# constantingoeldel/alphabeta-rs

Measured on AMD Instinct MI355X. Metric: ABneutral model fits/sec (pedigree x bootstraps x windows), higher is better.
Workload: dtype f64; 1 GPU; C3: synthetic 100-edge/8-generation pedigree (N=105 rows, T=8, K=47 distinct triples), 10 starts + 10000 bootstraps per GPU (bootstraps of one window sharded over the GPUs); rows=105, windows_per_gpu=1, starts=10, bootstraps=10000, plan_device_bytes=9663014, reduction_tree=0x10040, parallelism=bootstraps sharded over 1 GPU(s), one RCCL all-gather of the bootstrap tables

## Files before the change

### alphabeta_rs_amd/__init__.py

```python
from __future__ import annotations

import ctypes as C
import os
from pathlib import Path

import numpy as np

from . import build as _build

PKG = Path(__file__).resolve().parent
LIB_PATH = PKG / "libabneutral_hip.so"
if os.environ.get("ABNEUTRAL_HIP_LIB"):
    LIB_PATH = Path(os.environ["ABNEUTRAL_HIP_LIB"])

ABN_OK = 0
STATUS_NAMES = {
    0: "ABN_OK",
    1: "ABN_ERR_INVALID_ARG",
    2: "ABN_ERR_BAD_PEDIGREE",
    3: "ABN_ERR_NO_DEVICE",
    4: "ABN_ERR_HIP",
    5: "ABN_ERR_NO_FINITE_FIT",
    6: "ABN_ERR_STATE",
}
FIT_CONVERGED, FIT_MAX_ITERS, FIT_NONFINITE, FIT_TARGET = 0, 1, 2, 3
KERNEL_NAMES = {0: "none", 1: "speculative", 2: "resident", 3: "persistent", 4: "stream", 5: "two_pass"}

FIT_INFO_DTYPE = np.dtype(
    [("best_cost", "<f8"), ("iters", "<i4"), ("evals", "<i4"), ("status", "<i4"), ("lanes", "<i4")]
)

EXPORTED_SYMBOLS = [
    "abn_default_options", "abn_device_count", "abn_init", "abn_shutdown", "abn_device_info", "abn_last_error",
    "abn_status_string", "abn_version", "abn_cost_batch", "abn_fit_batch", "abn_gen_start_simplices",
    "abn_gen_boot_simplices", "abn_gen_boot_indices", "abn_ab_neutral_run", "abn_boot_model_run",
    "abn_analyze", "abn_select_best", "abn_bootstrap_rows", "abn_pairwise_divergence", "abn_plan_create", "abn_plan_destroy", "abn_plan_set_windows", "abn_plan_run",
    "abn_plan_run_phase", "abn_plan_sync", "abn_plan_tail_handed", "abn_plan_kernel_ms", "abn_plan_raw_device_ptr",
    "abn_plan_bind_raw", "abn_plan_download", "abn_plan_counters", "abn_plan_device_bytes",
    "abn_plan_set_window_ids", "abn_plan_failed_windows",
    "abn_multi_create", "abn_multi_destroy", "abn_multi_last_error", "abn_multi_set_windows", "abn_multi_run",
    "abn_multi_sync", "abn_multi_shard", "abn_multi_raw_device_ptr", "abn_multi_download", "abn_multi_counters",
    "abn_multi_rccl_available", "abn_reduction_tree", "abn_pairwise_divergence_dev", "abn_multi_set_window_ids",
    "abn_pairwise_divergence_windows", "abn_pairwise_divergence_windows_dev",
    "abn_multi_plan_shard", "abn_plan_last_kernels", "abn_multi_kernel_ms",
    "abn_packed_row_stride", "abn_pack_codes", "abn_unpack_codes", "abn_pairwise_divergence_packed",
    "abn_pairwise_divergence_packed_dev",
    "abn_pairwise_divergence_windows_packed", "abn_pairwise_divergence_windows_packed_dev",
    "abn_analyze_batch", "abn_analyze_batch_dev", "abn_plan_analyze", "abn_multi_analyze",
    "abn_windows_create", "abn_windows_destroy", "abn_windows_info", "abn_windows_stats", "abn_windows_layout",
    "abn_windows_packed", "abn_windows_packed_device_ptr", "abn_windows_pairwise",
    "abn_sites_parse", "abn_sites_destroy", "abn_sites_info", "abn_sites_fetch", "abn_sites_deferred",
    "abn_genes_create", "abn_genes_destroy", "abn_genes_choose", "abn_genes_choose_dev", "abn_windows_create_sites",
]


class Options(C.Structure):
    _fields_ = [
        ("seed", C.c_uint64),
        ("lanes_per_chain", C.c_int32),
        ("strict_order", C.c_int32),
        ("shrink_on_failed_contraction", C.c_int32),
        ("max_iters_start", C.c_int32),
        ("max_iters_boot", C.c_int32),
        ("stream_mode", C.c_int32),
        ("sd_tolerance", C.c_double),
        ("window_groups", C.c_int32),
        ("no_fixed_point_skip", C.c_int32),
    ]


class WindowsParams(C.Structure):
    _fields_ = [
        ("cutoff", C.c_uint32),
        ("step", C.c_uint32),
        ("size", C.c_uint32),
        ("absolute", C.c_int32),
        ("n_upstream", C.c_int32),
        ("n_gene", C.c_int32),
        ("n_downstream", C.c_int32),
    ]


class GeneRule(C.Structure):
    _fields_ = [
        ("cutoff", C.c_uint32),
        ("cutoff_gene_length", C.c_int32),
    ]


class SitesParams(C.Structure):
    _fields_ = [
        ("slab_bytes", C.c_int64),
        ("skip_lines", C.c_int32),
        ("reserved", C.c_int32),
    ]


class AbnError(RuntimeError):
    def __init__(self, status: int, detail: str = ""):
        self.status = status
        super().__init__(f"{STATUS_NAMES.get(status, status)}: {detail}")


_lib = None


def load_library(build_if_missing: bool = False) -> C.CDLL:
    global _lib
    if _lib is not None:
        return _lib
    if not LIB_PATH.exists():
        if build_if_missing:
            _build.build_hip()
        else:
            raise FileNotFoundError(
                f"{LIB_PATH} is missing: build it with `python -m alphabeta_rs_amd.build` "
                "(the ABneutral path has no CPU fallback)"
            )
    L = C.CDLL(str(LIB_PATH))
    dp, u32p, vp = C.POINTER(C.c_double), C.POINTER(C.c_uint32), C.c_void_p
    op = C.POINTER(Options)
    L.abn_default_options.argtypes = [op]
    L.abn_default_options.restype = None
    L.abn_device_count.argtypes = [C.POINTER(C.c_int)]
    L.abn_init.argtypes = [C.c_int, vp, C.POINTER(vp)]
    L.abn_shutdown.argtypes = [vp]
    L.abn_device_info.argtypes = [vp, C.POINTER(C.c_int32)]
    L.abn_last_error.argtypes = [vp]
    L.abn_last_error.restype = C.c_char_p
    L.abn_status_string.argtypes = [C.c_int]
    L.abn_status_string.restype = C.c_char_p
    L.abn_cost_batch.argtypes = [vp, op, dp, C.c_int32, C.c_double, C.c_double, C.c_double, dp, C.c_int64, dp, dp,
                                 u32p, u32p, C.c_int64, dp, dp, dp]
    L.abn_fit_batch.argtypes = [vp, op, dp, C.c_int32, C.c_double, C.c_double, C.c_double, dp, C.c_int64, dp,
                                C.c_int32, dp, vp]
    L.abn_gen_start_simplices.argtypes = [C.c_uint64, C.c_uint32, C.c_int32, C.c_double, dp]
    L.abn_gen_boot_simplices.argtypes = [C.c_uint64, C.c_uint32, C.c_uint32, C.c_int64, dp, dp]
    L.abn_gen_boot_indices.argtypes = [vp, C.c_uint64, C.c_uint32, C.c_uint32, C.c_int64, C.c_int32, u32p]
    L.abn_ab_neutral_run.argtypes = [vp, op, dp, C.c_int32, C.c_double, C.c_double, C.c_double, C.c_int32, dp, dp,
                                     dp, dp, vp, dp]
    L.abn_boot_model_run.argtypes = [vp, op, dp, C.c_int32, dp, dp, dp, C.c_double, C.c_double, C.c_double,
                                     C.c_int32, dp, vp]
    L.abn_analyze.argtypes = [dp, C.c_int64, dp]
    L.abn_analyze_batch.argtypes = [vp, dp, C.c_int32, C.c_int64, dp, C.POINTER(C.c_int32)]
    L.abn_analyze_batch_dev.argtypes = [vp, vp, C.c_int32, C.c_int64, vp, vp, dp]
    L.abn_plan_analyze.argtypes = [vp, dp, C.POINTER(C.c_int32)]
    L.abn_multi_analyze.argtypes = [vp, dp, C.POINTER(C.c_int32)]
    L.abn_select_best.argtypes = [vp, dp, C.c_int32, C.c_double, dp, C.c_int32, C.POINTER(C.c_int32), dp, dp, dp, dp]
    L.abn_bootstrap_rows.argtypes = [vp, dp, C.c_int64, dp]
    L.abn_pairwise_divergence.argtypes = [vp, C.POINTER(C.c_uint8), C.c_int32, C.c_int64, C.POINTER(C.c_uint64),
                                          C.POINTER(C.c_uint64), dp]
    L.abn_pairwise_divergence_dev.argtypes = [vp, vp, C.c_int32, C.c_int64, vp, vp, vp, dp]
    i64p = C.POINTER(C.c_int64)
    L.abn_pairwise_divergence_windows.argtypes = [vp, C.POINTER(C.c_uint8), C.c_int32, C.c_int64, i64p, i64p, C.c_int32,
                                                  C.POINTER(C.c_uint64), C.POINTER(C.c_uint64), dp]
    L.abn_pairwise_divergence_windows_dev.argtypes = [vp, vp, C.c_int32, C.c_int64, i64p, i64p, C.c_int32, vp, vp, vp, dp]
    u8p = C.POINTER(C.c_uint8)
    L.abn_packed_row_stride.argtypes = [C.c_int64]
    L.abn_packed_row_stride.restype = C.c_int64
    L.abn_pack_codes.argtypes = [u8p, C.c_int32, C.c_int64, C.c_int64, u8p, C.c_int64]
    L.abn_unpack_codes.argtypes = [u8p, C.c_int32, C.c_int64, C.c_int64, u8p, C.c_int64]
    L.abn_pairwise_divergence_packed.argtypes = [vp, u8p, C.c_int32, C.c_int64, C.c_int64, C.POINTER(C.c_uint64),
                                                 C.POINTER(C.c_uint64), dp]
    L.abn_pairwise_divergence_packed_dev.argtypes = [vp, vp, C.c_int32, C.c_int64, C.c_int64, vp, vp, vp, dp]
    L.abn_pairwise_divergence_windows_packed.argtypes = [vp, u8p, C.c_int32, C.c_int64, C.c_int64, i64p, i64p, C.c_int32,
                                                         C.POINTER(C.c_uint64), C.POINTER(C.c_uint64), dp]
    L.abn_pairwise_divergence_windows_packed_dev.argtypes = [vp, vp, C.c_int32, C.c_int64, C.c_int64, i64p, i64p,
                                                             C.c_int32, vp, vp, vp, dp]
    L.abn_windows_create.argtypes = [vp, C.POINTER(WindowsParams), C.c_int32, i64p, u32p, u32p, u32p, u8p, u8p, dp,
                                     C.POINTER(vp)]
    L.abn_windows_destroy.argtypes = [vp]
    L.abn_windows_info.argtypes = [vp, C.POINTER(C.c_int32), i64p, i64p]
    L.abn_windows_stats.argtypes = [vp, i64p, dp, dp, i64p]
    L.abn_windows_layout.argtypes = [vp, i64p, i64p, C.POINTER(C.c_int32)]
    L.abn_windows_packed.argtypes = [vp, u8p]
    L.abn_windows_packed_device_ptr.argtypes = [vp, C.POINTER(vp)]
    L.abn_windows_pairwise.argtypes = [vp, C.POINTER(C.c_uint64), C.POINTER(C.c_uint64), dp]
    L.abn_sites_parse.argtypes = [vp, C.c_char_p, C.c_int64, C.POINTER(SitesParams), C.POINTER(vp)]
    L.abn_sites_destroy.argtypes = [vp]
    L.abn_sites_info.argtypes = [vp, i64p, i64p, i64p, dp]
    L.abn_sites_fetch.argtypes = [vp, i64p, C.POINTER(C.c_int32), u32p, u32p, u8p, dp, u8p, u8p, dp]
    L.abn_sites_deferred.argtypes = [vp, i64p, i64p, i64p]
    i32p = C.POINTER(C.c_int32)
    L.abn_genes_create.argtypes = [vp, C.c_int32, i32p, i32p, i64p, u32p, u32p, u8p, C.POINTER(vp)]
    L.abn_genes_destroy.argtypes = [vp]
    L.abn_genes_choose.argtypes = [vp, C.POINTER(GeneRule), C.c_int32, i64p, i32p, u32p, u32p, u8p, u32p, u32p, u8p, dp]
    L.abn_genes_choose_dev.argtypes = [vp, C.POINTER(GeneRule), C.c_int32, i64p, vp, vp, vp, vp, vp, vp, vp, dp]
    L.abn_windows_create_sites.argtypes = [vp, C.POINTER(WindowsParams), vp, C.POINTER(GeneRule), C.c_int32, i64p, i32p,
                                           u32p, u32p, u8p, u8p, dp, C.POINTER(vp)]
    L.abn_plan_create.argtypes = [vp, op, dp, C.c_int32, C.c_int32, C.c_int32, C.c_int32, C.c_uint32, C.c_uint32,
                                  C.POINTER(vp)]
    L.abn_plan_destroy.argtypes = [vp]
    L.abn_plan_set_windows.argtypes = [vp, dp, dp, dp, dp]
    L.abn_plan_run.argtypes = [vp]
    L.abn_plan_run_phase.argtypes = [vp, C.c_int32]
    L.abn_plan_sync.argtypes = [vp]
    L.abn_plan_tail_handed.argtypes = [vp, C.POINTER(C.c_int64)]
    L.abn_plan_kernel_ms.argtypes = [vp, dp]
    L.abn_plan_raw_device_ptr.argtypes = [vp, C.POINTER(vp)]
    L.abn_plan_bind_raw.argtypes = [vp, vp]
    L.abn_plan_download.argtypes = [vp, dp, dp, dp, dp, vp, vp, C.POINTER(C.c_int32)]
    L.abn_plan_counters.argtypes = [vp, C.POINTER(C.c_int64)]
    L.abn_plan_device_bytes.argtypes = [vp, C.POINTER(C.c_int64)]
    L.abn_plan_set_window_ids.argtypes = [vp, u32p]
    L.abn_plan_failed_windows.argtypes = [vp, C.POINTER(C.c_int32)]
    L.abn_plan_last_kernels.argtypes = [vp, C.POINTER(C.c_int32)]
    i32p = C.POINTER(C.c_int32)
    L.abn_multi_create.argtypes = [i32p, C.c_int32, op, dp, C.c_int32, C.c_int32, C.c_int32, C.c_int32, C.POINTER(vp)]
    L.abn_multi_destroy.argtypes = [vp]
    L.abn_multi_last_error.argtypes = [vp]
    L.abn_multi_last_error.restype = C.c_char_p
    L.abn_multi_set_windows.argtypes = [vp, dp, dp, dp, dp]
    L.abn_multi_set_window_ids.argtypes = [vp, u32p]
    L.abn_multi_run.argtypes = [vp]
    L.abn_multi_sync.argtypes = [vp]
    L.abn_multi_shard.argtypes = [vp, C.c_int32, i32p]
    L.abn_multi_plan_shard.argtypes = [C.c_int32, C.c_int32, C.c_int32, C.c_int32, i32p]
    L.abn_multi_raw_device_ptr.argtypes = [vp, C.c_int32, C.POINTER(vp)]
    L.abn_multi_kernel_ms.argtypes = [vp, C.c_int32, dp]
    L.abn_multi_download.argtypes = [vp, dp, dp, dp, dp, vp, vp, i32p]
    L.abn_multi_counters.argtypes = [vp, C.POINTER(C.c_int64)]
    L.abn_multi_rccl_available.argtypes = [C.POINTER(C.c_int)]
    L.abn_reduction_tree.argtypes = [op, dp, C.c_int32, i32p]
    _lib = L
    return L


def _dp(a):
    return None if a is None else a.ctypes.data_as(C.POINTER(C.c_double))


def _u32p(a):
    return None if a is None else a.ctypes.data_as(C.POINTER(C.c_uint32))


def _f64(a, shape=None):
    a = np.ascontiguousarray(a, dtype=np.float64)
    return a if shape is None else a.reshape(shape)


def default_options(**kw) -> Options:
    o = Options()
    load_library().abn_default_options(C.byref(o))
    for k, v in kw.items():
        if not hasattr(o, k):
            raise TypeError(f"unknown option {k}")
        setattr(o, k, v)
    return o


def device_count() -> int:
    n = C.c_int(0)
    load_library().abn_device_count(C.byref(n))
    return n.value


def gen_start_simplices(seed: int, window: int, n_starts: int, max_divergence: float) -> np.ndarray:
    out = np.empty((n_starts, 5, 4))
    rc = load_library().abn_gen_start_simplices(seed, window, n_starts, max_divergence, _dp(out))
    if rc:
        raise AbnError(rc)
    return out


def gen_boot_simplices(seed: int, window: int, b0: int, nb: int, params) -> np.ndarray:
    p = _f64(params, (4,))
    out = np.empty((nb, 5, 4))
    rc = load_library().abn_gen_boot_simplices(seed, window, b0, nb, _dp(p), _dp(out))
    if rc:
        raise AbnError(rc)
    return out


def packed_row_stride(n_sites: int) -> int:
    return int(load_library().abn_packed_row_stride(int(n_sites)))


def pack_codes(codes, row_stride: int | None = None) -> np.ndarray:
    codes = np.ascontiguousarray(codes, dtype=np.uint8)
    n, L = codes.shape
    stride = packed_row_stride(L) if row_stride is None else int(row_stride)
    packed = np.empty((n, max(stride, 0)), dtype=np.uint8)
    u8p = C.POINTER(C.c_uint8)
    rc = load_library().abn_pack_codes(codes.ctypes.data_as(u8p), n, L, L, packed.ctypes.data_as(u8p), stride)
    if rc != 0:
        raise AbnError(rc, "pack_codes: a byte that is not 0, 1, 2 or 0x80 | status, or a bad row stride")
    return packed


def unpack_codes(packed, n_sites: int) -> np.ndarray:
    packed = np.ascontiguousarray(packed, dtype=np.uint8)
    n, stride = packed.shape
    codes = np.empty((n, int(n_sites)), dtype=np.uint8)
    u8p = C.POINTER(C.c_uint8)
    rc = load_library().abn_unpack_codes(packed.ctypes.data_as(u8p), n, int(n_sites), stride, codes.ctypes.data_as(u8p),
                                         int(n_sites))
    if rc != 0:
        raise AbnError(rc, "unpack_codes: bad row stride")
    return codes


def analyze(raw) -> np.ndarray:
    raw = _f64(raw).reshape(-1, 7)
    with np.errstate(all="ignore"):
        bad = np.isnan(raw).any(axis=1) | np.isnan(raw[:, 1] / raw[:, 0])
    if bad.any():
        raise AbnError(5, f"bootstrap {int(np.flatnonzero(bad)[0])} has no finite fit: no analysis of this table")
    out = np.empty(32)
    rc = load_library().abn_analyze(_dp(raw), raw.shape[0], _dp(out))
    if rc:
        raise AbnError(rc)
    return out.reshape(4, 8)


def analyze_batch(ctx: "Context", raw, allow_failed_windows=False):
    raw = _f64(raw)
    if raw.ndim != 3 or raw.shape[2] != 7:
        raise ValueError("raw is (n_windows, n_boot, 7)")
    W, B = raw.shape[0], raw.shape[1]
    out, fb = np.empty((W, 32)), np.full(W, -1, dtype=np.int32)
    rc = ctx._L.abn_analyze_batch(ctx._h, _dp(raw), W, B, _dp(out), fb.ctypes.data_as(C.POINTER(C.c_int32)))
    if not (rc == 5 and allow_failed_windows):
        ctx._check(rc)
    return out, fb


class Context:

    def __init__(self, device: int = 0, stream: int | None = None):
        self._L = load_library()
        h = C.c_void_p()
        if stream is None:
            sp = None
        elif stream == 0:
            sp = C.c_void_p(-1)
        else:
            sp = C.c_void_p(stream)
        rc = self._L.abn_init(device, sp, C.byref(h))
        if rc:
            raise AbnError(rc, "abn_init failed (no HIP device? the ABneutral path has no CPU fallback)")
        self._h = h
        self.device = device

    def close(self):
        if getattr(self, "_h", None):
            self._L.abn_shutdown(self._h)
            self._h = None

    def device_info(self):
        out = (C.c_int32 * 4)()
# ... 157 lines not shown
        return ms.value

    def pairwise_divergence_windows_packed(self, packed, n_sites: int, begin, end):
        packed = np.ascontiguousarray(packed, dtype=np.uint8)
        n, stride = packed.shape
        b, e = np.ascontiguousarray(begin, dtype=np.int64), np.ascontiguousarray(end, dtype=np.int64)
        if b.ndim != 1 or b.shape != e.shape:
            raise ValueError("begin and end are 1-d arrays of one length")
        W, npairs = b.shape[0], n * (n - 1) // 2
        diff, both = np.zeros((W, npairs), dtype=np.uint64), np.zeros((W, npairs), dtype=np.uint64)
        dval = np.zeros((W, npairs))
        i64p = C.POINTER(C.c_int64)
        self._check(self._L.abn_pairwise_divergence_windows_packed(
            self._h, packed.ctypes.data_as(C.POINTER(C.c_uint8)), n, int(n_sites), stride, b.ctypes.data_as(i64p),
            e.ctypes.data_as(i64p), W, diff.ctypes.data_as(C.POINTER(C.c_uint64)),
            both.ctypes.data_as(C.POINTER(C.c_uint64)), _dp(dval)))
        return diff, both, dval

    def pairwise_divergence_windows_packed_dev(self, packed_ptr: int, n_samples: int, n_sites: int, row_stride: int,
                                               begin, end, diff_ptr: int = 0, both_ptr: int = 0,
                                               dvalue_ptr: int = 0) -> float:
        b, e = np.ascontiguousarray(begin, dtype=np.int64), np.ascontiguousarray(end, dtype=np.int64)
        if b.ndim != 1 or b.shape != e.shape:
            raise ValueError("begin and end are 1-d arrays of one length")
        ms = C.c_double(0.0)
        i64p = C.POINTER(C.c_int64)
        self._check(self._L.abn_pairwise_divergence_windows_packed_dev(
            self._h, C.c_void_p(packed_ptr), n_samples, n_sites, row_stride, b.ctypes.data_as(i64p),
            e.ctypes.data_as(i64p), b.shape[0], C.c_void_p(diff_ptr or None), C.c_void_p(both_ptr or None),
            C.c_void_p(dvalue_ptr or None), C.byref(ms)))
        return ms.value

    def analyze_batch_dev(self, raw_ptr: int, n_windows: int, n_boot: int, out_ptr: int, first_bad_ptr: int = 0,
                          allow_failed_windows=False) -> float:
        ms = C.c_double(0.0)
        rc = self._L.abn_analyze_batch_dev(self._h, C.c_void_p(raw_ptr), n_windows, n_boot, C.c_void_p(out_ptr),
                                           C.c_void_p(first_bad_ptr or None), C.byref(ms))
        if not (rc == 5 and allow_failed_windows):
            self._check(rc)
        return ms.value

    def parse_sites(self, text: bytes, *, skip_lines: int = 1, slab_bytes: int = 0):
        text = bytes(text)
        p = SitesParams(slab_bytes, skip_lines, 0)
        h = C.c_void_p()
        self._check(self._L.abn_sites_parse(self._h, text, len(text), C.byref(p), C.byref(h)))
        try:
            n, nd, nl, ms = C.c_int64(), C.c_int64(), C.c_int64(), C.c_double()
            self._check(self._L.abn_sites_info(h, C.byref(n), C.byref(nd), C.byref(nl), C.byref(ms)))
            kinds = {"line": np.int64, "chromosome": np.int32, "start": np.uint32, "end": np.uint32, "strand": np.uint8,
                     "posteriormax": np.float64, "status": np.uint8, "status_flag": np.uint8, "meth_lvl": np.float64}
            sites = {k: np.zeros(n.value, dtype=t) for k, t in kinds.items()}
            self._check(self._L.abn_sites_fetch(h, *(a.ctypes.data_as(t) for a, t in
                                                     zip(sites.values(), self._L.abn_sites_fetch.argtypes[1:]))))
            deferred = {k: np.zeros(nd.value, dtype=np.int64) for k in ("line", "offset", "length")}
            self._check(self._L.abn_sites_deferred(h, *(a.ctypes.data_as(C.POINTER(C.c_int64)) for a in deferred.values())))
            sites["n_lines"], sites["kernel_ms"] = nl.value, ms.value
            return sites, deferred
        finally:
            self._L.abn_sites_destroy(h)

    def choose_genes(self, genes: "Genes", site_offset, chromosome, start, end, strand, *, cutoff,
                     cutoff_gene_length=False):
        off, u = _site_arrays(site_offset, chromosome, start, end, strand)
        S = int(off[-1])
        gs, ge, fl = np.zeros(S, dtype=np.uint32), np.zeros(S, dtype=np.uint32), np.zeros(S, dtype=np.uint8)
        ms = np.zeros(3)
        rule = GeneRule(cutoff, 1 if cutoff_gene_length else 0)
        u8p = C.POINTER(C.c_uint8)
        self._check(self._L.abn_genes_choose(genes._h, C.byref(rule), off.shape[0] - 1, off.ctypes.data_as(C.POINTER(C.c_int64)),
                                             u[0].ctypes.data_as(C.POINTER(C.c_int32)), _u32p(u[1]), _u32p(u[2]),
                                             u[3].ctypes.data_as(u8p), _u32p(gs), _u32p(ge), fl.ctypes.data_as(u8p), _dp(ms)))
        return gs, ge, fl, ms

    def choose_genes_dev(self, genes: "Genes", site_offset, chromosome_ptr: int, start_ptr: int, end_ptr: int,
                         strand_ptr: int, gene_start_ptr: int, gene_end_ptr: int, flags_ptr: int, *, cutoff,
                         cutoff_gene_length=False) -> np.ndarray:
        off = np.ascontiguousarray(site_offset, dtype=np.int64)
        ms = np.zeros(3)
        rule = GeneRule(cutoff, 1 if cutoff_gene_length else 0)
        self._check(self._L.abn_genes_choose_dev(genes._h, C.byref(rule), off.shape[0] - 1,
                                                 off.ctypes.data_as(C.POINTER(C.c_int64)),
                                                 *(C.c_void_p(p or None) for p in (chromosome_ptr, start_ptr, end_ptr,
                                                                                   strand_ptr, gene_start_ptr,
                                                                                   gene_end_ptr, flags_ptr)), _dp(ms)))
        return ms

    def boot_model_run(self, pedigree, model, pred, resid, p0uu, eqp, eqp_weight, n_boot, *,
                       options: Options | None = None):
        ped = _f64(pedigree).reshape(-1, 4)
        n = ped.shape[0]
        raw = np.empty((n_boot, 7))
        info = np.zeros(n_boot, dtype=FIT_INFO_DTYPE)
        self._check(self._L.abn_boot_model_run(self._h, C.byref(options) if options else None, _dp(ped), n,
                                               _dp(_f64(model, (4,))), _dp(_f64(pred, (n,))), _dp(_f64(resid, (n,))),
                                               p0uu, eqp, eqp_weight, n_boot, _dp(raw), info.ctypes.data))
        return raw, info


class Plan:

    def __init__(self, ctx: Context, generations, n_windows, n_starts, n_boot, *, window_offset=0, boot_offset=0,
                 options: Options | None = None):
        self.ctx = ctx
        self._L = ctx._L
        g = _f64(generations).reshape(-1, 3)
        self.N, self.W, self.S, self.B = g.shape[0], n_windows, n_starts, n_boot
        h = C.c_void_p()
        ctx._check(self._L.abn_plan_create(ctx._h, C.byref(options) if options else None, _dp(g), self.N, n_windows,
                                           n_starts, n_boot, window_offset, boot_offset, C.byref(h)))
        self._h = h

    def close(self):
        if getattr(self, "_h", None):
            self._L.abn_plan_destroy(self._h)
            self._h = None

    def __del__(self):
        try:
            self.close()
        except Exception:
            pass

    def set_window_ids(self, ids):
        a = None if ids is None else np.ascontiguousarray(ids, dtype=np.uint32).reshape(self.W)
        self.ctx._check(self._L.abn_plan_set_window_ids(self._h, _u32p(a)))

    def failed_windows(self) -> int:
        n = C.c_int32(0)
        self.ctx._check(self._L.abn_plan_failed_windows(self._h, C.byref(n)))
        return n.value

    def set_windows(self, d_obs, p0uu, eqp=None, eqp_weight=None):
        d = _f64(d_obs, (self.W, self.N))
        p = _f64(p0uu, (self.W,))
        e = None if eqp is None else _f64(eqp, (self.W,))
        ew = None if eqp_weight is None else _f64(eqp_weight, (self.W,))
        self.ctx._check(self._L.abn_plan_set_windows(self._h, _dp(d), _dp(p), _dp(e), _dp(ew)))

    def run(self):
        self.ctx._check(self._L.abn_plan_run(self._h))

    def run_phase(self, phase: int):
        self.ctx._check(self._L.abn_plan_run_phase(self._h, phase))

    def sync(self):
        self.ctx._check(self._L.abn_plan_sync(self._h))

    def tail_handed(self):
        out = (C.c_int64 * 2)()
        self.ctx._check(self._L.abn_plan_tail_handed(self._h, out))
        return int(out[0]), int(out[1])

    def kernel_ms(self):
        ms = np.zeros(3)
        self.ctx._check(self._L.abn_plan_kernel_ms(self._h, _dp(ms)))
        return {"fit_starts": ms[0], "select": ms[1], "fit_boot": ms[2]}

    def raw_device_ptr(self) -> int:
        p = C.c_void_p()
        self.ctx._check(self._L.abn_plan_raw_device_ptr(self._h, C.byref(p)))
        return p.value or 0

    def bind_raw(self, dev_ptr: int):
        self.ctx._check(self._L.abn_plan_bind_raw(self._h, C.c_void_p(dev_ptr)))

    def download(self, want_info=True, allow_failed_windows=False):
        W, N, S, B = self.W, self.N, self.S, self.B
        models, pred, resid = np.empty((W, 4)), np.empty((W, N)), np.empty((W, N))
        raw = np.empty((W, B, 7)) if B else None
        ia = np.zeros((W, S), dtype=FIT_INFO_DTYPE) if (S and want_info) else None
        ib = np.zeros((W, B), dtype=FIT_INFO_DTYPE) if (B and want_info) else None
        bs = np.full(W, -1, dtype=np.int32)
        rc = self._L.abn_plan_download(self._h, _dp(models), _dp(pred), _dp(resid), _dp(raw),
                                       None if ia is None else ia.ctypes.data,
                                       None if ib is None else ib.ctypes.data,
                                       bs.ctypes.data_as(C.POINTER(C.c_int32)))
        if not (rc == 5 and allow_failed_windows):
            self.ctx._check(rc)
        return {"models": models, "pred": pred, "resid": resid, "raw": raw, "info_a": ia, "info_b": ib,
                "best_start": bs}

    def analyze(self, allow_failed_windows=False):
        out, fb = np.empty((self.W, 32)), np.full(self.W, -1, dtype=np.int32)
        rc = self._L.abn_plan_analyze(self._h, _dp(out), fb.ctypes.data_as(C.POINTER(C.c_int32)))
        if not (rc == 5 and allow_failed_windows):
            self.ctx._check(rc)
        return out, fb

    def counters(self):
        out = (C.c_int64 * 5)()
        self.ctx._check(self._L.abn_plan_counters(self._h, out))
        return {"fits": out[0], "evals": out[1], "iters": out[2], "evals_skipped": out[3] + out[4],
                "evals_skipped_starts": out[3], "evals_skipped_boot": out[4]}

    def device_bytes(self) -> int:
        b = C.c_int64()
        self.ctx._check(self._L.abn_plan_device_bytes(self._h, C.byref(b)))
        return b.value

    def last_kernels(self):
        out = (C.c_int32 * 4)()
        self.ctx._check(self._L.abn_plan_last_kernels(self._h, out))
        return {"starts": (KERNEL_NAMES.get(out[0], out[0]), out[1]), "boot": (KERNEL_NAMES.get(out[2], out[2]), out[3])}


def _site_arrays(site_offset, chromosome, start, end, strand):
    off = np.ascontiguousarray(site_offset, dtype=np.int64)
    S = int(off[-1]) if off.shape[0] else 0
    return off, [np.ascontiguousarray(a, dtype=t).reshape(S) for a, t in
                 ((chromosome, np.int32), (start, np.uint32), (end, np.uint32), (strand, np.uint8))]


class Genes:

    def __init__(self, ctx: "Context", lists):
        self.ctx = ctx
        self._L = ctx._L
        lists = list(lists)
        chrom = np.array([l[0] for l in lists], dtype=np.int32)
        kind = np.array([l[1] for l in lists], dtype=np.int32)
        off = np.zeros(len(lists) + 1, dtype=np.int64)
        off[1:] = np.cumsum([len(l[2]) for l in lists])
        cat = lambda k, t: np.ascontiguousarray(np.concatenate([np.asarray(l[k], dtype=t) for l in lists])
                                                if lists else np.zeros(0, dtype=t))
        start, end, strand = cat(2, np.uint32), cat(3, np.uint32), cat(4, np.uint8)
        h = C.c_void_p()
        i32p = C.POINTER(C.c_int32)
        ctx._check(self._L.abn_genes_create(ctx._h, len(lists), chrom.ctypes.data_as(i32p), kind.ctypes.data_as(i32p),
                                            off.ctypes.data_as(C.POINTER(C.c_int64)), _u32p(start), _u32p(end),
                                            strand.ctypes.data_as(C.POINTER(C.c_uint8)), C.byref(h)))
        self._h = h
        self.n_genes = int(off[-1])

    def close(self):
        if getattr(self, "_h", None):
            self._L.abn_genes_destroy(self._h)
            self._h = None

    def __del__(self):
        try:
            self.close()
        except Exception:
            pass


class Windows:

    def __init__(self, ctx: Context, site_offset, pos, gene_start, gene_end, flags, code, level, *, cutoff, step, size,
                 absolute, counts):
        self.ctx = ctx
        self._L = ctx._L
        off = np.ascontiguousarray(site_offset, dtype=np.int64)
        self.n_samples = off.shape[0] - 1
        S = int(off[-1]) if off.shape[0] else 0
        u32 = [np.ascontiguousarray(a, dtype=np.uint32).reshape(S) for a in (pos, gene_start, gene_end)]
        u8 = [np.ascontiguousarray(a, dtype=np.uint8).reshape(S) for a in (flags, code)]
        lvl = _f64(level, (S,))
        p = WindowsParams(cutoff, step, size, 1 if absolute else 0, *map(int, counts))
        h = C.c_void_p()
        u8p = C.POINTER(C.c_uint8)
        ctx._check(self._L.abn_windows_create(ctx._h, C.byref(p), self.n_samples, off.ctypes.data_as(C.POINTER(C.c_int64)),
                                              _u32p(u32[0]), _u32p(u32[1]), _u32p(u32[2]), u8[0].ctypes.data_as(u8p),
                                              u8[1].ctypes.data_as(u8p), _dp(lvl), C.byref(h)))
        self._h = h
        W, stride, ns = C.c_int32(), C.c_int64(), C.c_int64()
        ctx._check(self._L.abn_windows_info(h, C.byref(W), C.byref(stride), C.byref(ns)))
        self.W, self.row_stride, self.n_sites = W.value, stride.value, ns.value

    @classmethod
    def from_sites(cls, ctx: Context, genes: Genes, site_offset, chromosome, start, end, strand, code, level, *, cutoff,
                   cutoff_gene_length=False, step, size, absolute, counts):
        self = cls.__new__(cls)
        self.ctx = ctx
        self._L = ctx._L
        off, u = _site_arrays(site_offset, chromosome, start, end, strand)
        self.n_samples = off.shape[0] - 1
        S = int(off[-1]) if off.shape[0] else 0
        co = np.ascontiguousarray(code, dtype=np.uint8).reshape(S)
        lvl = _f64(level, (S,))
        p = WindowsParams(cutoff, step, size, 1 if absolute else 0, *map(int, counts))
        rule = GeneRule(cutoff, 1 if cutoff_gene_length else 0)
        h = C.c_void_p()
        u8p = C.POINTER(C.c_uint8)
        ctx._check(self._L.abn_windows_create_sites(ctx._h, C.byref(p), genes._h, C.byref(rule), self.n_samples,
                                                    off.ctypes.data_as(C.POINTER(C.c_int64)),
                                                    u[0].ctypes.data_as(C.POINTER(C.c_int32)), _u32p(u[1]), _u32p(u[2]),
                                                    u[3].ctypes.data_as(u8p), co.ctypes.data_as(u8p), _dp(lvl), C.byref(h)))
        self._h = h
        W, stride, ns = C.c_int32(), C.c_int64(), C.c_int64()
        ctx._check(self._L.abn_windows_info(h, C.byref(W), C.byref(stride), C.byref(ns)))
        self.W, self.row_stride, self.n_sites = W.value, stride.value, ns.value
        return self

    def close(self):
        if getattr(self, "_h", None):
            self._L.abn_windows_destroy(self._h)
            self._h = None

    def __del__(self):
        try:
            self.close()
        except Exception:
            pass

    def stats(self):
# ... 147 lines not shown
```

### alphabeta_rs_amd/csrc/abn_api.hip

```cpp
#include <functional>

#include "abn_host.hpp"
#include "abn_device.hpp"
#include "abn_route.hpp"

using namespace abn;

static_assert(sizeof(abn_fit_info) == sizeof(FitInfoDev), "abn_fit_info layout");


static int as_i8(double x) {
  if (x != x) return 0;
  if (x >= 127.0) return 127;
  if (x <= -128.0) return -128;
  return (int)x;
}

struct Topology {
  int N = 0, K = 0, T = 0, TP = 0, KP = 0, chain_stride = 0;
  std::vector<uint32_t> tri;
  std::vector<uint16_t> tid;
};

static int build_topology(const double* rows, int n, int stride, Topology& t) {
// ... 385 lines not shown
  DevBuf<uint32_t> d;
  HIPCHK(c, d.alloc((size_t)nb * (size_t)n_rows));
  int rc = launch_gen_idx(c, d.p, n_rows, (int)nb, 1, seed, window, b0);
  if (rc) return rc;
  HIPCHK(c, hipMemcpyAsync(idx, d.p, d.bytes(), hipMemcpyDeviceToHost, c->stream));
  HIPCHK(c, hipStreamSynchronize(c->stream));
  return ABN_OK;
}

extern "C" int abn_cost_batch(abn_ctx* c, const abn_options* opts, const double* pedigree, int32_t n_rows, double p_uu0,
                              double eqp, double eqp_weight, const double* candidates, int64_t m, const double* pred,
                              const double* resid, const uint32_t* idx, const uint32_t* cand_to_boot,
                              int64_t n_boot_rows, double* cost, double* dt1t2, double* p_uu_inf) {
  if (!c) return ABN_ERR_INVALID_ARG;
  if (!pedigree || n_rows <= 0 || !candidates || m < 0 || !cost) return set_err(c, ABN_ERR_INVALID_ARG, "null/size");
  if (idx && (!pred || !resid || n_boot_rows <= 0)) return set_err(c, ABN_ERR_INVALID_ARG, "bootstrap inputs");
  if (m == 0) return ABN_OK;
  if (const char* oe = options_error(resolve(opts))) return set_err(c, ABN_ERR_INVALID_ARG, oe);
  const abn_options o = resolve_for(opts, n_rows);
  OneShot s(c);
  int rc = s.open(c, pedigree, n_rows, [&]() -> int {
    for (int64_t i = 0; idx && i < m; ++i)
      if ((cand_to_boot ? (int64_t)cand_to_boot[i] : i) >= n_boot_rows)
        return set_err(c, ABN_ERR_INVALID_ARG, "cand_to_boot out of range");
    return ABN_OK;
  });
  if (rc) return rc;
  const size_t N = (size_t)n_rows;
  const std::vector<double> dcol = column3(pedigree, n_rows);
  DevBuf<double> dD, dpred, dresid, dcand, dcost, ddt, dpuu;
  DevBuf<uint32_t> didx, dc2b;
  if ((rc = upload(c, dD, dcol.data(), N)) || (rc = upload(c, dcand, candidates, (size_t)m * 4))) return rc;
  HIPCHK(c, dcost.alloc((size_t)m));
  if (idx) {
    if ((rc = upload(c, dpred, pred, N)) || (rc = upload(c, dresid, resid, N)) ||
        (rc = upload(c, didx, idx, (size_t)n_boot_rows * N)))
      return rc;
    for (size_t q = 0; q < (size_t)n_boot_rows * N; ++q)
      if (idx[q] >= (uint32_t)N) return set_err(c, ABN_ERR_INVALID_ARG, "bootstrap index out of range");
    if (cand_to_boot && (rc = upload(c, dc2b, cand_to_boot, (size_t)m))) return rc;
  }
  if (dt1t2) HIPCHK(c, ddt.alloc((size_t)m * N));
  if (p_uu_inf) HIPCHK(c, dpuu.alloc((size_t)m));

  const PedigreeRoute pr = route_pedigree(n_rows, s.t.K, s.t.T, o.lanes_per_chain, o.strict_order);
  if (pr.cost_refusal) return set_err(c, ABN_ERR_INVALID_ARG, pr.cost_refusal);
  const int ng = kWave / pr.cost_lanes;
  CostArgs a{};
  fill_topology(a, s.t, s.dt);
  a.chain_stride = s.t.chain_stride;
  a.p_uu0 = p_uu0;
  a.eqp = eqp;
  a.eqp_w = eqp_weight;
  a.D = dD.p;
  a.pred = dpred.p;
  a.resid = dresid.p;
  a.idx = didx.p;
  a.cand_to_boot = dc2b.p;
  a.dmode = idx ? 1 : 0;
  a.cand = dcand.p;
  a.M = m;
  a.strict = pr.strict;
  a.tree = pr.cost_tree;
  a.cost = dcost.p;
  a.dt = ddt.p;
  a.puu = dpuu.p;
  const long long blocks = (m + ng - 1) / ng;
  if (blocks > 0x7fffffffLL) return set_err(c, ABN_ERR_INVALID_ARG, "too many candidates");
  LaunchRoute r{};
  r.key = {kFamCost, pr.cost_lanes, 0, false, false, false};
  r.grid = (unsigned)blocks;
  r.block = kWave;
  r.lds = pr.cost_lds;
  rc = launch_route(c, r, a, c->stream);
  if (rc) return rc;
  HIPCHK(c, hipMemcpyAsync(cost, dcost.p, dcost.bytes(), hipMemcpyDeviceToHost, c->stream));
  if (dt1t2) HIPCHK(c, hipMemcpyAsync(dt1t2, ddt.p, ddt.bytes(), hipMemcpyDeviceToHost, c->stream));
  if (p_uu_inf) HIPCHK(c, hipMemcpyAsync(p_uu_inf, dpuu.p, dpuu.bytes(), hipMemcpyDeviceToHost, c->stream));
  HIPCHK(c, hipStreamSynchronize(c->stream));
  return ABN_OK;
}

extern "C" int abn_fit_batch(abn_ctx* c, const abn_options* opts, const double* pedigree, int32_t n_rows, double p_uu0,
                             double eqp, double eqp_weight, const double* simplex0, int64_t f, const double* dobs_rows,
                             int32_t max_iters, double* best, abn_fit_info* info) {
  if (!c) return ABN_ERR_INVALID_ARG;
  if (!pedigree || n_rows <= 0 || !simplex0 || f < 0 || !best || max_iters < 0 || f > 0x7fffffff)
    return set_err(c, ABN_ERR_INVALID_ARG, "null/size");
  if (f == 0) return ABN_OK;
  if (const char* oe = options_error(resolve(opts))) return set_err(c, ABN_ERR_INVALID_ARG, oe);
  const abn_options o = resolve_for(opts, n_rows);
  if (max_iters > (1 << 28)) return set_err(c, ABN_ERR_INVALID_ARG, "max_iters must be in 0 .. 2^28");
  OneShot s(c);
  int rc = s.open(c, pedigree, n_rows);
  if (rc) return rc;
  const size_t N = (size_t)n_rows;
  DevBuf<double> dD, ds0, dbest, dscal;
  DevBuf<FitInfoDev> dinfo;
  const std::vector<double> dcol = dobs_rows ? std::vector<double>() : column3(pedigree, n_rows);
  const double scal[3] = {p_uu0, eqp, eqp_weight};
  if ((rc = upload(c, dD, dobs_rows ? dobs_rows : dcol.data(), dobs_rows ? (size_t)f * N : N)) ||
      (rc = upload(c, ds0, simplex0, (size_t)f * 20)) || (rc = upload(c, dscal, scal, 3)))
    return rc;
  HIPCHK(c, dbest.alloc((size_t)f * 4));
  HIPCHK(c, dinfo.alloc((size_t)f));
  HIPCHK(c, hipMemsetAsync(dinfo.p, 0, dinfo.bytes(), c->stream));

  const PedigreeRoute pr = route_pedigree(n_rows, s.t.K, s.t.T, o.lanes_per_chain, o.strict_order);
  FitArgs a{};
  fill_topology(a, s.t, s.dt);
  fill_options(a, o, pr);
  a.p_uu = dscal.p;
  a.eqp = dscal.p + 1;
  a.eqp_w = dscal.p + 2;
  a.D = dD.p;
  a.simplex0 = ds0.p;
  a.W = dobs_rows ? (int)f : 1;
  a.C = dobs_rows ? 1 : (int)f;
  a.max_iters = max_iters;
  a.best = dbest.p;
  a.info = dinfo.p;
  rc = launch_fit(c, pr, PhaseRoute{false, pr.lanes, false}, a, LaunchOffer{}, c->stream);
  if (rc) return rc;
  HIPCHK(c, hipMemcpyAsync(best, dbest.p, dbest.bytes(), hipMemcpyDeviceToHost, c->stream));
  if (info) HIPCHK(c, hipMemcpyAsync(info, dinfo.p, dinfo.bytes(), hipMemcpyDeviceToHost, c->stream));
  HIPCHK(c, hipStreamSynchronize(c->stream));
  return ABN_OK;
}

enum PlanEvent { kEvFitA, kEvFitAEnd, kEvSelect, kEvSelectEnd, kEvFitB, kEvFitBEnd, kPlanEvents };

struct abn_plan {
  abn_ctx* ctx = nullptr;
  abn_options opt{};
  Topology topo;
  DevTopology dtopo;
  int N = 0, W = 0, S = 0, B = 0;
  uint32_t window_offset = 0, boot_offset = 0;
  PedigreeRoute route{};
  std::vector<uint32_t> wid_host;
  DevBuf<uint32_t> wid;
  bool windows_set = false, phase_a_done = false, ran_a = false, ran_b = false;
  DevBuf<double> D, pred, resid, p_uu, eqp, eqp_w, simplexA, bestA, model, lse, bestB, raw_own;
  DevBuf<FitInfoDev> infoA, infoB;
  DevBuf<int32_t> best_start;
  DevBuf<uint32_t> idx;
  DevBuf<double> dstar;
  DevBuf<double> nm_state;
  DevBuf<int> susp_list;
  DevBuf<unsigned long long> skipped;
  bool twopass_a = false;
  DevBuf<int> slice_buf;
  unsigned slice_cap = 0;
  DevBuf<unsigned> slice_status;
  long long persist_expected[2] = {0, 0};
  long long tail_handed[2] = {0, 0};
  int32_t last_kernels[4] = {0, 0, 0, 0};
  bool stream_b = false;
  double* raw = nullptr;
  hipEvent_t ev[kPlanEvents] = {};
  hipEvent_t ev_fork = nullptr;
  std::vector<hipEvent_t> ev_join;
};

extern "C" int abn_plan_destroy(abn_plan* p) {
  if (!p) return ABN_ERR_INVALID_ARG;
  for (auto& e : p->ev)
    if (e) (void)hipEventDestroy(e);
  if (p->ev_fork) (void)hipEventDestroy(p->ev_fork);
  for (auto e : p->ev_join) (void)hipEventDestroy(e);
  delete p;
  return ABN_OK;
}

extern "C" int abn_plan_create(abn_ctx* c, const abn_options* opts, const double* generations, int32_t n_rows,
                               int32_t n_windows, int32_t n_starts, int32_t n_boot, uint32_t window_offset,
                               uint32_t boot_offset, abn_plan** out) {
  if (!c || !out) return ABN_ERR_INVALID_ARG;
  *out = nullptr;
  if (!generations || n_rows <= 0 || n_windows <= 0 || n_starts < 0 || n_boot < 0)
    return set_err(c, ABN_ERR_INVALID_ARG, "null/size");
  if ((long long)n_windows * std::max(n_starts, n_boot) > 0x7fffffffLL)
    return set_err(c, ABN_ERR_INVALID_ARG, "too many chains");
  {
    const abn_options o = resolve(opts);
    if (const char* oe = options_error(o)) return set_err(c, ABN_ERR_INVALID_ARG, oe);
  }
  HIPCHK(c, hipSetDevice(c->device));
  PoolScope pool_scope(c);
  struct Destroy {
    void operator()(abn_plan* q) const { abn_plan_destroy(q); }
  };
  std::unique_ptr<abn_plan, Destroy> owner(new (std::nothrow) abn_plan());
  abn_plan* p = owner.get();
  if (!p) return ABN_ERR_HIP;
  p->ctx = c;
  p->opt = resolve_for(opts, n_rows);
  p->N = n_rows;
  p->W = n_windows;
  p->S = n_starts;
  p->B = n_boot;
  p->window_offset = window_offset;
  p->boot_offset = boot_offset;
  int rc = build_topology(generations, n_rows, 3, p->topo);
  if (rc) return set_err(c, rc, abn_status_string(rc));
  p->route = route_pedigree(n_rows, p->topo.K, p->topo.T, p->opt.lanes_per_chain, p->opt.strict_order);
  if (p->route.refusal) return set_err(c, ABN_ERR_INVALID_ARG, p->route.refusal);
  auto fail = [&](hipError_t e, const char* what) {
    return set_err(c, ABN_ERR_HIP, std::string(what) + ": " + hipGetErrorString(e));
  };
  rc = upload_topology(c, p->topo, p->dtopo);
  if (rc) return rc;
  const size_t W = (size_t)n_windows, N = (size_t)n_rows, S = (size_t)n_starts, B = (size_t)n_boot;
  hipError_t e;
#define PALLOC(buf, count)                         \
  if ((e = p->buf.alloc(count)) != hipSuccess) return fail(e, "hipMalloc " #buf)
  PALLOC(D, W * N);
  PALLOC(pred, W * N);
  PALLOC(resid, W * N);
  PALLOC(p_uu, W);
  PALLOC(eqp, W);
  PALLOC(eqp_w, W);
  PALLOC(model, W * 4);
  PALLOC(best_start, W);
  PALLOC(simplexA, W * S * 20);
  PALLOC(bestA, W * S * 4);
  PALLOC(infoA, W * S);
  PALLOC(lse, W * S);
  PALLOC(idx, W * B * N);
  PALLOC(bestB, W * B * 4);
  PALLOC(infoB, W * B);
  PALLOC(raw_own, W * B * 7);
  PALLOC(skipped, 2 * kPhaseWords);
  PALLOC(slice_status, 2 * kSliceWords);
  p->twopass_a = plan_two_pass((long long)n_windows * n_starts, p->opt.max_iters_start, p->opt.no_fixed_point_skip,
                               p->opt.shrink_on_failed_contraction, p->opt.strict_order);
  if (p->twopass_a) {
    PALLOC(nm_state, W * S * kStateDoubles);
    PALLOC(susp_list, W * S + 1);
  }
  if (const size_t chains = plan_sliced_chains(p->route, W * std::max(S, B), c->cus, p->opt.window_groups)) {
    if (p->nm_state.n < chains * kStateDoubles) PALLOC(nm_state, chains * kStateDoubles);
    p->slice_cap = (unsigned)(chains * 16 / kParkShards + 4096);
    PALLOC(slice_buf, (size_t)kParkShards * ((size_t)kParkHeaderInts + (size_t)p->slice_cap));
    if (p->susp_list.n < chains + 1) PALLOC(susp_list, chains + 1);
  }
  p->stream_b = n_boot > 0 && p->route.streams && p->opt.stream_mode == 0;
  if (p->stream_b) PALLOC(dstar, W * B * N);
#undef PALLOC
  p->raw = p->raw_own.p;
  for (auto& ev : p->ev)
    if ((e = hipEventCreate(&ev)) != hipSuccess) return fail(e, "hipEventCreate");
  *out = owner.release();
  return ABN_OK;
}

static int plan_upload_model(abn_plan* p, const double* model, const double* pred, const double* resid,
                             const double* p0uu, const double* eqp, const double* eqp_w) {
  abn_ctx* c = p->ctx;
  const size_t W = (size_t)p->W;
  HIPCHK(c, hipMemcpyAsync(p->model.p, model, p->model.bytes(), hipMemcpyHostToDevice, c->stream));
  HIPCHK(c, hipMemcpyAsync(p->pred.p, pred, p->pred.bytes(), hipMemcpyHostToDevice, c->stream));
  HIPCHK(c, hipMemcpyAsync(p->resid.p, resid, p->resid.bytes(), hipMemcpyHostToDevice, c->stream));
  HIPCHK(c, hipMemcpyAsync(p->p_uu.p, p0uu, W * sizeof(double), hipMemcpyHostToDevice, c->stream));
  HIPCHK(c, hipMemcpyAsync(p->eqp.p, eqp, W * sizeof(double), hipMemcpyHostToDevice, c->stream));
  HIPCHK(c, hipMemcpyAsync(p->eqp_w.p, eqp_w, W * sizeof(double), hipMemcpyHostToDevice, c->stream));
  int rc = launch_gen_idx(c, p->idx.p, p->N, p->B, p->W, p->opt.seed, p->window_offset, p->boot_offset, p->wid.p);
  if (rc) return rc;
  HIPCHK(c, hipStreamSynchronize(c->stream));
  p->windows_set = true;
  p->phase_a_done = true;
  return ABN_OK;
}

extern "C" int abn_plan_set_window_ids(abn_plan* p, const uint32_t* ids) {
  if (!p) return ABN_ERR_INVALID_ARG;
  abn_ctx* c = p->ctx;
  if (p->windows_set) return set_err(c, ABN_ERR_STATE, "abn_plan_set_window_ids must precede abn_plan_set_windows");
  HIPCHK(c, hipSetDevice(c->device));
  PoolScope pool_scope(c);
  if (!ids) {
    p->wid_host.clear();
    p->wid.release();
    return ABN_OK;
  }
  p->wid_host.assign(ids, ids + p->W);
  if (int rc = upload(c, p->wid, p->wid_host.data(), (size_t)p->W)) return rc;
  HIPCHK(c, hipStreamSynchronize(c->stream));
  return ABN_OK;
}

extern "C" int abn_plan_set_windows(abn_plan* p, const double* d_obs, const double* p0uu, const double* eqp,
                                    const double* eqp_weight) {
  if (!p) return ABN_ERR_INVALID_ARG;
  abn_ctx* c = p->ctx;
  if (!d_obs || !p0uu) return set_err(c, ABN_ERR_INVALID_ARG, "null window data");
  HIPCHK(c, hipSetDevice(c->device));
  const size_t W = (size_t)p->W, N = (size_t)p->N, S = (size_t)p->S;
  std::vector<double> ones(W, 1.0);
  const double* e1 = eqp ? eqp : p0uu;
  const double* e2 = eqp_weight ? eqp_weight : ones.data();
  HIPCHK(c, hipMemcpyAsync(p->D.p, d_obs, p->D.bytes(), hipMemcpyHostToDevice, c->stream));
  HIPCHK(c, hipMemcpyAsync(p->p_uu.p, p0uu, W * sizeof(double), hipMemcpyHostToDevice, c->stream));
  HIPCHK(c, hipMemcpyAsync(p->eqp.p, e1, W * sizeof(double), hipMemcpyHostToDevice, c->stream));
  HIPCHK(c, hipMemcpyAsync(p->eqp_w.p, e2, W * sizeof(double), hipMemcpyHostToDevice, c->stream));
  std::vector<double> sx(W * S * 20);
  for (size_t w = 0; w < W; ++w) {
    double mx = d_obs[w * N];
    for (size_t i = 1; i < N; ++i) mx = std::max(mx, d_obs[w * N + i]);
    const uint32_t wg = p->wid_host.empty() ? p->window_offset + (uint32_t)w : p->wid_host[w];
    abn_gen_start_simplices(p->opt.seed, wg, p->S, mx, sx.data() + w * S * 20);
  }
  if (!sx.empty())
    HIPCHK(c, hipMemcpyAsync(p->simplexA.p, sx.data(), p->simplexA.bytes(), hipMemcpyHostToDevice, c->stream));
  int rc = launch_gen_idx(c, p->idx.p, p->N, p->B, p->W, p->opt.seed, p->window_offset, p->boot_offset, p->wid.p);
  if (rc) return rc;
  HIPCHK(c, hipStreamSynchronize(c->stream));
  p->windows_set = true;
  p->phase_a_done = false;
  return ABN_OK;
}

struct WindowOffsets {
  size_t w, rows, starts, boots;
};
static WindowOffsets window_offsets(const abn_plan* p, int w0) {
  const size_t o = (size_t)w0;
  return {o, o * (size_t)p->N, o * (size_t)p->S, o * (size_t)p->B};
}

static FitArgs phase_args(const abn_plan* p, int phase, int w0, int wn) {
  const WindowOffsets o = window_offsets(p, w0);
  const size_t chains = phase ? o.boots : o.starts;
  FitArgs a{};
  fill_topology(a, p->topo, p->dtopo);
  fill_options(a, p->opt, p->route);
  a.p_uu = p->p_uu.p + o.w;
  a.eqp = p->eqp.p + o.w;
  a.eqp_w = p->eqp_w.p + o.w;
  a.wstride = 1;
  a.D = p->D.p + o.rows;
  a.pred = p->pred.p + o.rows;
  a.resid = p->resid.p + o.rows;
  a.idx = p->idx.p + o.boots * (size_t)p->N;
  a.model = p->model.p + o.w * 4;
  a.window_offset = p->window_offset + (uint32_t)w0;
  a.boot_offset = p->boot_offset;
  a.wid = p->wid.p ? p->wid.p + o.w : nullptr;
  a.W = wn;
  a.C = phase ? p->B : p->S;
  a.dmode = a.smode = phase;
  a.simplex0 = phase ? nullptr : p->simplexA.p + chains * 20;
  a.max_iters = phase ? p->opt.max_iters_boot : p->opt.max_iters_start;
  a.best = (phase ? p->bestB.p : p->bestA.p) + chains * 4;
  a.info = (phase ? p->infoB.p : p->infoA.p) + chains;
  a.raw = phase ? p->raw + chains * 7 : nullptr;
  return a;
}

static int launch_phase(abn_plan* p, int phase, FitArgs& a, hipStream_t st, bool timed) {
  abn_ctx* c = p->ctx;
  const bool whole = a.W == p->W;
  const char* force = nullptr;
#ifdef ABN_MEASUREMENT_KNOBS
  force = getenv(phase ? "ABN_PHASE_B_KERNEL" : "ABN_PHASE_A_KERNEL");
#endif
  const PhaseRoute ph = route_phase(p->route, phase, (long long)p->W * (phase ? p->B : p->S), c->cus, a.dmode, whole,
                                    p->twopass_a, force);
  LaunchOffer offer;
  offer.queue = whole;
  offer.parking = whole && p->slice_cap > 0;
  a.skipped = p->skipped.p + kPhaseWords * phase + kPhaseSkipped;
  if (whole) {
    a.queue = reinterpret_cast<unsigned*>(p->skipped.p + kPhaseWords * phase + kPhaseQueue);
    a.slice_status = p->slice_status.p + kSliceWords * phase;
  }
  if (offer.parking) {
    a.park_cap = p->slice_cap;
    a.park_ht = reinterpret_cast<unsigned*>(p->slice_buf.p);
    a.parked = p->slice_buf.p + kParkShards * kParkHeaderInts;
    a.state = p->nm_state.p;
    a.susp_list = p->susp_list.p;
  }
  int kind = ABN_KERNEL_NONE, rc;
  if (ph.two_pass) {
    int* cnt = p->susp_list.p + (size_t)p->W * (size_t)p->S;
    HIPCHK(c, hipMemsetAsync(cnt, 0, sizeof(int), st));
    a.state = p->nm_state.p;
    a.susp_list = p->susp_list.p;
    a.susp_count = cnt;
    offer.pass = 1;
    rc = launch_fit(c, p->route, ph, a, offer, st, &kind);
    offer.pass = 2;
    if (!rc) rc = launch_fit(c, p->route, ph, a, offer, st);
  } else {
    rc = launch_fit(c, p->route, ph, a, offer, st, &kind);
  }
  if (rc) return rc;
  if (whole) p->persist_expected[phase] = kind == ABN_KERNEL_PERSISTENT ? (long long)a.W * a.C : 0;
  if (timed) {
    p->last_kernels[2 * phase] = kind;
    p->last_kernels[2 * phase + 1] = ph.lanes;
  }
  return ABN_OK;
}

static int enqueue_phase_a(abn_plan* p, int w0, int wn, hipStream_t st, bool timed) {
  abn_ctx* c = p->ctx;
  FitArgs a = phase_args(p, 0, w0, wn);
  if (timed) HIPCHK(c, hipEventRecord(p->ev[kEvFitA], st));
  if (int rc = launch_phase(p, 0, a, st, timed)) return rc;
  if (timed) HIPCHK(c, hipEventRecord(p->ev[kEvFitAEnd], st));
  const WindowOffsets o = window_offsets(p, w0);
  SelectArgs s{};
  fill_topology(s, p->topo, p->dtopo);
  s.p_uu = a.p_uu;
  s.D = a.D;
  s.models = a.best;
  s.info = a.info;
  s.W = wn;
  s.S = p->S;
  s.lse = p->lse.p + o.starts;
  s.model = p->model.p + o.w * 4;
  s.pred = p->pred.p + o.rows;
  s.resid = p->resid.p + o.rows;
  s.best_start = p->best_start.p + o.w;
  if (timed) HIPCHK(c, hipEventRecord(p->ev[kEvSelect], st));
  if (int rc = launch_select(c, s, p->route.select_lds, st)) return rc;
  if (timed) HIPCHK(c, hipEventRecord(p->ev[kEvSelectEnd], st));
  return ABN_OK;
}

static int enqueue_phase_b(abn_plan* p, int w0, int wn, hipStream_t st, bool timed) {
  abn_ctx* c = p->ctx;
  FitArgs a = phase_args(p, 1, w0, wn);
  if (timed) HIPCHK(c, hipEventRecord(p->ev[kEvFitB], st));
  if (p->stream_b) {
    double* dst = p->dstar.p + window_offsets(p, w0).boots * (size_t)p->N;
    const long long total = (long long)wn * p->B * p->N;
    const unsigned blocks = (unsigned)std::min<long long>((total + 255) / 256, 64LL * c->cus);
    hipLaunchKernelGGL(abn_make_dstar_kernel, dim3(blocks), dim3(256), 0, st, dst, a.pred, a.resid, a.idx, p->N,
                       (long long)p->B * p->N, total);
    HIPCHK(c, hipGetLastError());
    a.dmode = 2;
    a.D = dst;
  }
  if (int rc = launch_phase(p, 1, a, st, timed)) return rc;
  if (timed) HIPCHK(c, hipEventRecord(p->ev[kEvFitBEnd], st));
  return ABN_OK;
}

static int clear_phase_words(abn_plan* p, int first, int n) {
  HIPCHK(p->ctx, hipMemsetAsync(p->skipped.p + kPhaseWords * first, 0, (size_t)n * kPhaseWords * sizeof(unsigned long long),
                                p->ctx->stream));
  return ABN_OK;
}

enum ClearWords { kClearNone, kClearOwnPhase, kClearBothPhases };
static int plan_run_phase(abn_plan* p, int32_t phase, ClearWords clear) {
  abn_ctx* c = p->ctx;
  if (!p->windows_set) return set_err(c, ABN_ERR_STATE, "abn_plan_set_windows has not been called");
  HIPCHK(c, hipSetDevice(c->device));
  if (clear == kClearBothPhases) {
    if (int rc = clear_phase_words(p, 0, 2)) return rc;
  } else if (clear == kClearOwnPhase) {
    if (int rc = clear_phase_words(p, phase == 0 ? 0 : 1, 1)) return rc;
  }
  if (phase == 0) {
    if (p->S <= 0) return set_err(c, ABN_ERR_STATE, "plan has no starts");
    int rc = enqueue_phase_a(p, 0, p->W, c->stream, true);
    if (rc) return rc;
    p->phase_a_done = true;
    p->ran_a = true;
    return ABN_OK;
  }
  if (phase == 1) {
    if (p->B <= 0) return set_err(c, ABN_ERR_STATE, "plan has no bootstraps");
    if (!p->phase_a_done) return set_err(c, ABN_ERR_STATE, "phase A has not run");
    int rc = enqueue_phase_b(p, 0, p->W, c->stream, true);
    if (rc) return rc;
    p->ran_b = true;
    return ABN_OK;
  }
  return set_err(c, ABN_ERR_INVALID_ARG, "phase must be 0 or 1");
}

extern "C" int abn_plan_run_phase(abn_plan* p, int32_t phase) {
  if (!p) return ABN_ERR_INVALID_ARG;
  return plan_run_phase(p, phase, kClearOwnPhase);
}

extern "C" int abn_plan_run(abn_plan* p) {
  if (!p) return ABN_ERR_INVALID_ARG;
  abn_ctx* c = p->ctx;
  if (!p->windows_set) return set_err(c, ABN_ERR_STATE, "abn_plan_set_windows has not been called");
  int groups = p->opt.window_groups > 0 ? p->opt.window_groups : 1;
  groups = std::max(1, std::min(groups, p->W));
  if (groups == 1 || p->S <= 0 || p->B <= 0) {
    int rc = ABN_OK;
    if (p->S > 0) rc = plan_run_phase(p, 0, kClearBothPhases);
    if (rc) return rc;
    if (p->B > 0) rc = plan_run_phase(p, 1, p->S > 0 ? kClearNone : kClearOwnPhase);
    return rc;
  }
  HIPCHK(c, hipSetDevice(c->device));
  while ((int)c->side.size() < groups) {
    hipStream_t st = nullptr;
    HIPCHK(c, hipStreamCreateWithFlags(&st, hipStreamNonBlocking));
    c->side.push_back(st);
  }
  if (!p->ev_fork) HIPCHK(c, hipEventCreateWithFlags(&p->ev_fork, hipEventDisableTiming));
  while ((int)p->ev_join.size() < groups) {
    hipEvent_t e = nullptr;
    HIPCHK(c, hipEventCreateWithFlags(&e, hipEventDisableTiming));
    p->ev_join.push_back(e);
  }
  if (int rc = clear_phase_words(p, 0, 2)) return rc;
  HIPCHK(c, hipEventRecord(p->ev_fork, c->stream));
  for (int g = 0; g < groups; ++g) {
    const int w0 = (int)((long long)p->W * g / groups), w1 = (int)((long long)p->W * (g + 1) / groups);
    hipStream_t st = c->side[(size_t)g];
    HIPCHK(c, hipStreamWaitEvent(st, p->ev_fork, 0));
    int rc = enqueue_phase_a(p, w0, w1 - w0, st, g == 0);
    if (!rc) rc = enqueue_phase_b(p, w0, w1 - w0, st, g == 0);
    if (rc) return rc;
    HIPCHK(c, hipEventRecord(p->ev_join[(size_t)g], st));
  }
  for (int g = 0; g < groups; ++g) HIPCHK(c, hipStreamWaitEvent(c->stream, p->ev_join[(size_t)g], 0));
  p->phase_a_done = true;
  p->ran_a = true;
  p->ran_b = true;
  return ABN_OK;
}

static int verify_persistent(abn_plan* p) {
  abn_ctx* c = p->ctx;
  HIPCHK(c, hipSetDevice(c->device));
  unsigned sl[2][kSliceWords] = {};
  const bool check = p->persist_expected[0] > 0 || p->persist_expected[1] > 0;
  if (check) HIPCHK(c, hipMemcpyAsync(sl, p->slice_status.p, sizeof sl, hipMemcpyDeviceToHost, c->stream));
  HIPCHK(c, hipStreamSynchronize(c->stream));
  for (int ph = 0; ph < 2 && check; ++ph) {
    if (p->persist_expected[ph] <= 0) continue;
    const unsigned* s = sl[ph];
    p->tail_handed[ph] = (long long)s[kSliceHanded];
    if (s[kSliceError] != 0 || (long long)s[kSliceFinished] != p->persist_expected[ph])
      return set_err(c, ABN_ERR_HIP, std::string("persistent fit launch of phase ") + (ph ? "B" : "A") + " finished " +
                                         std::to_string(s[kSliceFinished]) + " of " + std::to_string(p->persist_expected[ph]) +
                                         " chains (error word " + std::to_string(s[kSliceError]) + ", " + std::to_string(s[kSliceHanded]) +
                                         " handed to the speculative kernel, list length " + std::to_string(s[kSliceTailFill]) +
                                         "): results are incomplete");
  }
  return ABN_OK;
}

extern "C" int abn_plan_sync(abn_plan* p) {
  if (!p) return ABN_ERR_INVALID_ARG;
  return verify_persistent(p);
}

extern "C" int abn_plan_tail_handed(abn_plan* p, int64_t* out2) {
  if (!p || !out2) return ABN_ERR_INVALID_ARG;
  const int rc = verify_persistent(p);
  out2[0] = p->persist_expected[0] > 0 ? p->tail_handed[0] : 0;
  out2[1] = p->persist_expected[1] > 0 ? p->tail_handed[1] : 0;
  return rc;
}

extern "C" int abn_plan_kernel_ms(abn_plan* p, double* ms3) {
  if (!p || !ms3) return ABN_ERR_INVALID_ARG;
  abn_ctx* c = p->ctx;
  HIPCHK(c, hipStreamSynchronize(c->stream));
  ms3[0] = ms3[1] = ms3[2] = 0.0;
  float ms = 0.f;
  if (p->ran_a) {
    HIPCHK(c, hipEventElapsedTime(&ms, p->ev[kEvFitA], p->ev[kEvFitAEnd]));
    ms3[0] = ms;
    HIPCHK(c, hipEventElapsedTime(&ms, p->ev[kEvSelect], p->ev[kEvSelectEnd]));
    ms3[1] = ms;
  }
  if (p->ran_b) {
    HIPCHK(c, hipEventElapsedTime(&ms, p->ev[kEvFitB], p->ev[kEvFitBEnd]));
    ms3[2] = ms;
  }
  return ABN_OK;
}

extern "C" int abn_plan_raw_device_ptr(abn_plan* p, void** dev_ptr) {
  if (!p || !dev_ptr) return ABN_ERR_INVALID_ARG;
  *dev_ptr = p->raw;
  return ABN_OK;
}

extern "C" int abn_plan_bind_raw(abn_plan* p, void* dev_ptr) {
  if (!p) return ABN_ERR_INVALID_ARG;
  p->raw = dev_ptr ? (double*)dev_ptr : p->raw_own.p;
  return ABN_OK;
}

extern "C" int abn_plan_download(abn_plan* p, double* models, double* pred, double* resid, double* raw,
                                 abn_fit_info* info_a, abn_fit_info* info_b, int32_t* best_start) {
  if (!p) return ABN_ERR_INVALID_ARG;
  abn_ctx* c = p->ctx;
  HIPCHK(c, hipSetDevice(c->device));
  hipStream_t s = c->stream;
  const size_t W = (size_t)p->W, B = (size_t)p->B;
  if (models) HIPCHK(c, hipMemcpyAsync(models, p->model.p, p->model.bytes(), hipMemcpyDeviceToHost, s));
  if (pred) HIPCHK(c, hipMemcpyAsync(pred, p->pred.p, p->pred.bytes(), hipMemcpyDeviceToHost, s));
  if (resid) HIPCHK(c, hipMemcpyAsync(resid, p->resid.p, p->resid.bytes(), hipMemcpyDeviceToHost, s));
  if (raw && B) HIPCHK(c, hipMemcpyAsync(raw, p->raw, W * B * 7 * sizeof(double), hipMemcpyDeviceToHost, s));
  if (info_a && p->S) HIPCHK(c, hipMemcpyAsync(info_a, p->infoA.p, p->infoA.bytes(), hipMemcpyDeviceToHost, s));
  if (info_b && B) HIPCHK(c, hipMemcpyAsync(info_b, p->infoB.p, p->infoB.bytes(), hipMemcpyDeviceToHost, s));
  std::vector<int32_t> bs;
  if (p->ran_a) {
    bs.resize(W);
    HIPCHK(c, hipMemcpyAsync(bs.data(), p->best_start.p, p->best_start.bytes(), hipMemcpyDeviceToHost, s));
  }
  if (int rc = verify_persistent(p)) return rc;
  if (best_start) {
    if (p->ran_a) std::copy(bs.begin(), bs.end(), best_start);
    else std::fill(best_start, best_start + W, 0);
  }
  for (int32_t b : bs)
    if (b < 0) return set_err(c, ABN_ERR_NO_FINITE_FIT, "a window has no finite start (best_start = -1): its rows are NaN");
  return ABN_OK;
}

extern "C" int abn_plan_analyze(abn_plan* p, double* out, int32_t* first_bad) {
  if (!p) return ABN_ERR_INVALID_ARG;
  abn_ctx* c = p->ctx;
  if (!out) return set_err(c, ABN_ERR_INVALID_ARG, "null out");
  if (!p->ran_b || p->B <= 0) return set_err(c, ABN_ERR_STATE, "phase B has not run: there is no bootstrap table");
  if (int rc = verify_persistent(p)) return rc;
  return analyze_device_table(c, p->raw, p->W, p->B, out, first_bad);
}

extern "C" int abn_plan_failed_windows(abn_plan* p, int32_t* n_failed) {
  if (!p || !n_failed) return ABN_ERR_INVALID_ARG;
  abn_ctx* c = p->ctx;
  *n_failed = 0;
  if (!p->ran_a) return verify_persistent(p);
  HIPCHK(c, hipSetDevice(c->device));
  std::vector<int32_t> bs((size_t)p->W);
  HIPCHK(c, hipMemcpyAsync(bs.data(), p->best_start.p, p->best_start.bytes(), hipMemcpyDeviceToHost, c->stream));
  if (int rc = verify_persistent(p)) return rc;
  for (int32_t b : bs) *n_failed += b < 0 ? 1 : 0;
  return ABN_OK;
}

extern "C" int abn_plan_counters(abn_plan* p, int64_t* out5) {
  if (!p || !out5) return ABN_ERR_INVALID_ARG;
  abn_ctx* c = p->ctx;
  out5[0] = out5[1] = out5[2] = out5[3] = out5[4] = 0;
  std::vector<FitInfoDev> h;
  auto add = [&](const DevBuf<FitInfoDev>& b, int phase) -> int {
    if (!b.n) return ABN_OK;
    h.resize(b.n);
    unsigned long long sk = 0;
    HIPCHK(c, hipMemcpyAsync(h.data(), b.p, b.bytes(), hipMemcpyDeviceToHost, c->stream));
    HIPCHK(c, hipMemcpyAsync(&sk, p->skipped.p + kPhaseWords * phase + kPhaseSkipped, sizeof sk, hipMemcpyDeviceToHost, c->stream));
    HIPCHK(c, hipStreamSynchronize(c->stream));
    for (const auto& f : h) {
      out5[0] += 1;
      out5[1] += f.evals;
      out5[2] += f.iters;
    }
    out5[3 + phase] = (int64_t)sk;
    return ABN_OK;
  };
  int rc = ABN_OK;
  if (p->ran_a) rc = add(p->infoA, 0);
  if (rc) return rc;
  if (p->ran_b) rc = add(p->infoB, 1);
  return rc;
}

#ifdef ABN_STAMPS
static int debug_stamps(abn_plan* p, unsigned long long* out8, bool spec) {
  abn_ctx* c = p->ctx;
  DevBuf<unsigned long long> d;
  HIPCHK(c, d.alloc(8));
  HIPCHK(c, hipMemsetAsync(d.p, 0, 64, c->stream));
  FitArgs a = phase_args(p, 0, 0, p->W);
  a.dbg = d.p;
  int rc = launch_fit(c, p->route, PhaseRoute{spec, p->route.lanes, false}, a, LaunchOffer{}, c->stream);
  if (rc) return rc;
  HIPCHK(c, hipMemcpyAsync(out8, d.p, 64, hipMemcpyDeviceToHost, c->stream));
  HIPCHK(c, hipStreamSynchronize(c->stream));
  return ABN_OK;
}
extern "C" int abn_plan_debug_stamps(abn_plan* p, unsigned long long* out8) { return debug_stamps(p, out8, false); }
extern "C" int abn_plan_debug_stamps_spec(abn_plan* p, unsigned long long* out8) { return debug_stamps(p, out8, true); }
#endif

extern "C" int abn_plan_last_kernels(abn_plan* p, int32_t* out4) {
  if (!p || !out4) return ABN_ERR_INVALID_ARG;
  for (int k = 0; k < 4; ++k) out4[k] = p->last_kernels[k];
  return ABN_OK;
}

extern "C" int abn_plan_device_bytes(abn_plan* p, int64_t* bytes) {
  if (!p || !bytes) return ABN_ERR_INVALID_ARG;
  size_t t = 0;
  t += p->D.bytes() + p->pred.bytes() + p->resid.bytes() + p->p_uu.bytes() + p->eqp.bytes() + p->eqp_w.bytes();
  t += p->simplexA.bytes() + p->bestA.bytes() + p->model.bytes() + p->lse.bytes() + p->bestB.bytes();
  t += p->raw_own.bytes() + p->infoA.bytes() + p->infoB.bytes() + p->best_start.bytes() + p->idx.bytes();
  t += p->dstar.bytes() + p->nm_state.bytes() + p->susp_list.bytes() + p->skipped.bytes() + p->slice_buf.bytes();
  t += p->slice_status.bytes() + p->wid.bytes();
  t += p->dtopo.tri.bytes() + p->dtopo.tid.bytes();
  *bytes = (int64_t)t;
  return ABN_OK;
}

static void split_pedigree(const double* ped, int n, std::vector<double>& gens, std::vector<double>& d) {
  gens.resize((size_t)n * 3);
  d = column3(ped, n);
  for (size_t i = 0; i < (size_t)n; ++i) std::copy(ped + i * 4, ped + i * 4 + 3, gens.begin() + i * 3);
}

extern "C" int abn_ab_neutral_run(abn_ctx* c, const abn_options* opts, const double* pedigree, int32_t n_rows,
                                  double p0uu, double eqp, double eqp_weight, int32_t n_starts, double* model,
                                  double* pred, double* resid, double* all_models, abn_fit_info* info, double* lse) {
  if (!c) return ABN_ERR_INVALID_ARG;
  if (!pedigree || n_rows <= 0 || n_starts <= 0 || !model || !pred || !resid)
    return set_err(c, ABN_ERR_INVALID_ARG, "null/size");
  std::vector<double> gens, d;
  split_pedigree(pedigree, n_rows, gens, d);
  abn_plan* p = nullptr;
  int rc = abn_plan_create(c, opts, gens.data(), n_rows, 1, n_starts, 0, 0, 0, &p);
  if (rc) return rc;
  rc = abn_plan_set_windows(p, d.data(), &p0uu, &eqp, &eqp_weight);
  if (!rc) rc = abn_plan_run_phase(p, 0);
  int32_t best = -1;
  bool no_fit = false;
  if (!rc) {
    rc = abn_plan_download(p, model, pred, resid, nullptr, info, nullptr, &best);
    if (rc == ABN_ERR_NO_FINITE_FIT) {
      no_fit = true;
      rc = ABN_OK;
    }
  }
  if (!rc && all_models) {
    hipError_t e = hipMemcpy(all_models, p->bestA.p, p->bestA.bytes(), hipMemcpyDeviceToHost);
    if (e != hipSuccess) rc = set_err(c, ABN_ERR_HIP, hipGetErrorString(e));
  }
  if (!rc && lse) {
    hipError_t e = hipMemcpy(lse, p->lse.p, p->lse.bytes(), hipMemcpyDeviceToHost);
    if (e != hipSuccess) rc = set_err(c, ABN_ERR_HIP, hipGetErrorString(e));
  }
  abn_plan_destroy(p);
  if (!rc && (no_fit || best < 0)) rc = set_err(c, ABN_ERR_NO_FINITE_FIT, abn_status_string(ABN_ERR_NO_FINITE_FIT));
  return rc;
}

extern "C" int abn_boot_model_run(abn_ctx* c, const abn_options* opts, const double* pedigree, int32_t n_rows,
                                  const double* model, const double* pred, const double* resid, double p0uu,
                                  double eqp, double eqp_weight, int32_t n_boot, double* raw, abn_fit_info* info) {
  if (!c) return ABN_ERR_INVALID_ARG;
  if (!pedigree || n_rows <= 0 || n_boot <= 0 || !model || !pred || !resid || !raw)
    return set_err(c, ABN_ERR_INVALID_ARG, "null/size");
  std::vector<double> gens, d;
  split_pedigree(pedigree, n_rows, gens, d);
  abn_plan* p = nullptr;
  int rc = abn_plan_create(c, opts, gens.data(), n_rows, 1, 0, n_boot, 0, 0, &p);
  if (rc) return rc;
  rc = plan_upload_model(p, model, pred, resid, &p0uu, &eqp, &eqp_weight);
  if (!rc) rc = abn_plan_run_phase(p, 1);
  if (!rc) rc = abn_plan_download(p, nullptr, nullptr, nullptr, raw, nullptr, info, nullptr);
  abn_plan_destroy(p);
  return rc;
}

extern "C" int abn_select_best(abn_ctx* c, const double* pedigree, int32_t n_rows, double p0uu, const double* models,
                               int32_t n_models, int32_t* best_index, double* model, double* pred, double* resid,
                               double* lse) {
  if (!c) return ABN_ERR_INVALID_ARG;
  if (!pedigree || n_rows <= 0 || !models || n_models <= 0 || !best_index)
    return set_err(c, ABN_ERR_INVALID_ARG, "null/size");
  OneShot s(c);
  PedigreeRoute pr{};
  int rc = s.open(c, pedigree, n_rows, [&]() -> int {
    pr = route_pedigree(n_rows, s.t.K, s.t.T, 0, 0);
    return pr.select_refusal ? set_err(c, ABN_ERR_INVALID_ARG, pr.select_refusal) : ABN_OK;
  });
  if (rc) return rc;
  const size_t N = (size_t)n_rows, S = (size_t)n_models;
  const std::vector<double> dcol = column3(pedigree, n_rows);
  DevBuf<double> dD, dm, dlse, dmodel, dpred, dresid, dp;
  DevBuf<FitInfoDev> dinfo;
  DevBuf<int32_t> dbest;
  if ((rc = upload(c, dD, dcol.data(), N)) || (rc = upload(c, dm, models, S * 4)) || (rc = upload(c, dp, &p0uu, 1)))
    return rc;
  HIPCHK(c, dlse.alloc(S));
  HIPCHK(c, dmodel.alloc(4));
  HIPCHK(c, dpred.alloc(N));
  HIPCHK(c, dresid.alloc(N));
  HIPCHK(c, dinfo.alloc(S));
  HIPCHK(c, dbest.alloc(1));
  HIPCHK(c, hipMemsetAsync(dinfo.p, 0, dinfo.bytes(), c->stream));
  SelectArgs a{};
  fill_topology(a, s.t, s.dt);
  a.p_uu = dp.p;
  a.D = dD.p;
  a.models = dm.p;
  a.info = dinfo.p;
  a.W = 1;
  a.S = n_models;
  a.lse = dlse.p;
  a.model = dmodel.p;
  a.pred = dpred.p;
  a.resid = dresid.p;
  a.best_start = dbest.p;
  rc = launch_select(c, a, pr.select_lds, c->stream);
  if (rc) return rc;
  HIPCHK(c, hipMemcpyAsync(best_index, dbest.p, sizeof(int32_t), hipMemcpyDeviceToHost, c->stream));
  if (model) HIPCHK(c, hipMemcpyAsync(model, dmodel.p, dmodel.bytes(), hipMemcpyDeviceToHost, c->stream));
  if (pred) HIPCHK(c, hipMemcpyAsync(pred, dpred.p, dpred.bytes(), hipMemcpyDeviceToHost, c->stream));
  if (resid) HIPCHK(c, hipMemcpyAsync(resid, dresid.p, dresid.bytes(), hipMemcpyDeviceToHost, c->stream));
  if (lse) HIPCHK(c, hipMemcpyAsync(lse, dlse.p, dlse.bytes(), hipMemcpyDeviceToHost, c->stream));
  HIPCHK(c, hipStreamSynchronize(c->stream));
  if (*best_index < 0) return set_err(c, ABN_ERR_NO_FINITE_FIT, abn_status_string(ABN_ERR_NO_FINITE_FIT));
  return ABN_OK;
}

extern "C" int abn_bootstrap_rows(abn_ctx* c, const double* best, int64_t n_boot, double* raw) {
  if (!c) return ABN_ERR_INVALID_ARG;
  if (!best || !raw || n_boot < 0) return set_err(c, ABN_ERR_INVALID_ARG, "null/size");
  if (n_boot == 0) return ABN_OK;
  HIPCHK(c, hipSetDevice(c->device));
  PoolScope pool_scope(c);
  DevBuf<double> db, dr;
  if (int rc = upload(c, db, best, (size_t)n_boot * 4)) return rc;
  HIPCHK(c, dr.alloc((size_t)n_boot * 7));
  const unsigned blocks = (unsigned)std::min<long long>((n_boot + 255) / 256, 4096);
  hipLaunchKernelGGL(abn_rows_kernel, dim3(blocks), dim3(256), 0, c->stream, db.p, (long long)n_boot, dr.p);
  HIPCHK(c, hipGetLastError());
  HIPCHK(c, hipMemcpyAsync(raw, dr.p, dr.bytes(), hipMemcpyDeviceToHost, c->stream));
  HIPCHK(c, hipStreamSynchronize(c->stream));
  return ABN_OK;
}
```

### alphabeta_rs_amd/csrc/abn_aux_kernels.hpp

```cpp
#pragma once
#include "abn_common.hpp"

namespace abn {

struct SelectArgs {
  const uint32_t* tri;
  const uint16_t* tid;
  int N, K, T, TP;
  const double* p_uu;
  const double* D;
  const double* models;
  const FitInfoDev* info;
  int W, S;
  double* lse;
  double* model;
  double* pred;
  double* resid;
  int32_t* best_start;
};

__device__ __forceinline__ void select_fill_dt(const SelectArgs& a, const double* x, double p_uu0, double* pw,
                                               double* dtab, int lane) {
  const double p_mm = 1.0 - p_uu0;
  const double sv0 = p_uu0, sv1 = x[2] * p_mm, sv2 = (1.0 - x[2]) * p_mm;
  if constexpr (kMatrixFma) build_power_table_mx<kWave>(x[0], x[1], a.T, pw, 0, dtab, lane);
  else build_power_table<kWave>(genmatrix(x[0], x[1]), a.T, a.TP, pw, lane);
  __syncthreads();
  for (int t = lane; t < a.K; t += kWave) dtab[t] = triple_dt(a.tri[t], pw, a.TP, sv0, sv1, sv2);
  __syncthreads();
}

__global__ __launch_bounds__(kWave) void abn_select_lse_kernel(const SelectArgs a) {
  extern __shared__ __align__(16) double lds[];
  const int lane = threadIdx.x;
  const int w = blockIdx.x / a.S, sidx = blockIdx.x - w * a.S;
  const int N = a.N;
  double* pw = lds;
  double* dtab = pw + kPw * a.TP;
  double* term = dtab + ((a.K + 1) & ~1);
  const size_t wN = (size_t)w * (size_t)N;
  double x[4];
#pragma unroll
  for (int d = 0; d < 4; ++d) x[d] = a.models[((size_t)w * a.S + sidx) * 4 + d];
  select_fill_dt(a, x, a.p_uu[w], pw, dtab, lane);
  double lsum = 0.0;
  for (int base = 0; base < N; base += kSelChunk) {
    const int cnt = (N - base) < kSelChunk ? (N - base) : kSelChunk;
    for (int i = lane; i < cnt; i += kWave) {
      const double r = a.D[wN + base + i] - x[3] - dtab[a.tid[base + i]];
      term[i] = r * r;
    }
    __syncthreads();
    for (int i = 0; i < cnt; ++i) lsum = lsum + term[i];
    __syncthreads();
  }
  if (lane == 0) a.lse[(size_t)w * a.S + sidx] = lsum;
}

__global__ __launch_bounds__(kWave) void abn_select_kernel(const SelectArgs a) {
  extern __shared__ __align__(16) double lds[];
  const int lane = threadIdx.x;
  const int w = blockIdx.x;
  const int N = a.N;
  double* pw = lds;
  double* dtab = pw + kPw * a.TP;
  const size_t wN = (size_t)w * (size_t)N;

  int best = -1;
  double best_lse = __builtin_inf();
  for (int sidx = lane; sidx < a.S; sidx += kWave) {
    const double lsum = a.lse[(size_t)w * a.S + sidx];
    const bool ok = (lsum == lsum) && (a.info[(size_t)w * a.S + sidx].status != 2);
    if (ok && (best < 0 || lsum < best_lse)) {
      best = sidx;
      best_lse = lsum;
    }
  }
#pragma unroll
  for (int off = kWave / 2; off >= 1; off >>= 1) {
    const int ob = __shfl_xor(best, off, kWave);
    const double ol = __shfl_xor(best_lse, off, kWave);
    if (ob >= 0 && (best < 0 || ol < best_lse || (ol == best_lse && ob < best))) {
      best = ob;
      best_lse = ol;
    }
  }
  if (lane == 0) a.best_start[w] = best;
  if (best < 0) {
    for (int i = lane; i < N; i += kWave) {
      a.pred[wN + i] = __builtin_nan("");
      a.resid[wN + i] = __builtin_nan("");
    }
    if (lane < 4) a.model[4 * w + lane] = __builtin_nan("");
    return;
  }
  double x[4];
#pragma unroll
  for (int d = 0; d < 4; ++d) x[d] = a.models[((size_t)w * a.S + best) * 4 + d];
  select_fill_dt(a, x, a.p_uu[w], pw, dtab, lane);
  for (int i = lane; i < N; i += kWave) {
    const double p = x[3] + dtab[a.tid[i]];
    a.pred[wN + i] = p;
    a.resid[wN + i] = a.D[wN + i] - p;
  }
  if (lane < 4) a.model[4 * w + lane] = x[lane];
}

struct CostArgs {
  const uint32_t* tri;
  const uint16_t* tid;
  int N, K, T, TP;
  int chain_stride;
  double p_uu0, eqp, eqp_w;
  const double* D;
  const double* pred;
  const double* resid;
  const uint32_t* idx;
  const uint32_t* cand_to_boot;
  int dmode;
  const double* cand;
  long long M;
  int strict;
  int tree;
  double* cost;
  double* dt;
  double* puu;
};

template <int G>
__global__ __launch_bounds__(kWave) void abn_cost_kernel(const CostArgs a) {
  constexpr int NG = kWave / G;
  extern __shared__ __align__(16) double lds[];
  const int lane = threadIdx.x;
  const int g = lane / G;
  const int gl = lane - g * G;
  const long long m_raw = (long long)blockIdx.x * NG + g;
  const bool valid = m_raw < a.M;
  const long long m = valid ? m_raw : 0;
  const int N = a.N, K = a.K, TP = a.TP;
  double* pw = lds + (size_t)g * a.chain_stride;
  double* dtab = pw + kPw * TP;
  double* term = lds + (size_t)NG * a.chain_stride;

  const double al = a.cand[4 * m + 0], be = a.cand[4 * m + 1], wt = a.cand[4 * m + 2], ic = a.cand[4 * m + 3];
  const double p_mm = 1.0 - a.p_uu0;
  const uint32_t* idx_row = nullptr;
  if (a.dmode) {
    const size_t b = a.cand_to_boot ? a.cand_to_boot[m] : (size_t)m;
    idx_row = a.idx + b * (size_t)N;
  }
  const double sv0 = a.p_uu0, sv1 = wt * p_mm, sv2 = (1.0 - wt) * p_mm;
  if constexpr (kMatrixFma && G == kWave) build_power_table_mx<G>(al, be, a.T, lds, a.chain_stride, dtab, lane);
  else build_power_table<G>(genmatrix(al, be), a.T, TP, pw, gl);
  __syncthreads();
  for (int t = gl; t < K; t += G) dtab[t] = triple_dt(a.tri[t], pw, TP, sv0, sv1, sv2);
  __syncthreads();
  const double puu = p_uu_est(al, be);
  const double pen = (a.eqp_w * (double)N) * ((puu - a.eqp) * (puu - a.eqp));
  double result;
  if (a.strict) {
    double ssum = 0.0;
    for (int base = 0; base < N; base += kSelChunk) {
      const int cnt = (N - base) < kSelChunk ? (N - base) : kSelChunk;
      for (int i = gl; i < cnt; i += G) {
        const int row = base + i;
        const double d = a.dmode ? a.pred[row] + a.resid[idx_row[row]] : a.D[row];
        const double r = d - ic - dtab[a.tid[row]];
        term[i] = r * r + pen;
      }
      __syncthreads();
      for (int i = 0; i < cnt; ++i) ssum = ssum + term[i];
      __syncthreads();
    }
    result = ssum;
  } else {
    if (a.tree == kTreeCanon) {
      constexpr int NA = kWave / G;
      double av[NA];
#pragma unroll
      for (int j = 0; j < NA; ++j) av[j] = 0.0;
      for (int i0 = gl; i0 < N; i0 += kWave) {
#pragma unroll
        for (int j = 0; j < NA; ++j) {
          const int i = i0 + G * j;
          if (i < N) {
            const double d = a.dmode ? a.pred[i] + a.resid[idx_row[i]] : a.D[i];
            const double r = d - ic - dtab[a.tid[i]];
            av[j] = av[j] + (r * r + pen);
          }
        }
      }
      result = tree64_finish<G>(av);
    } else {
      double acc = 0.0;
      for (int i = gl; i < N; i += G) {
        const double d = a.dmode ? a.pred[i] + a.resid[idx_row[i]] : a.D[i];
        const double r = d - ic - dtab[a.tid[i]];
        acc = acc + (r * r + pen);
      }
      result = group_sum<G>(acc);
    }
  }
  if (valid) {
    if (gl == 0) {
      a.cost[m] = result;
      if (a.puu) a.puu[m] = puu;
    }
    if (a.dt)
      for (int i = gl; i < N; i += G) a.dt[(size_t)m * N + i] = dtab[a.tid[i]];
  }
}

__global__ __launch_bounds__(256) void abn_rows_kernel(const double* best, long long n, double* raw) {
  for (long long t = (long long)blockIdx.x * blockDim.x + threadIdx.x; t < n; t += (long long)gridDim.x * blockDim.x) {
    const double al = best[4 * t + 0], be = best[4 * t + 1];
    double* ro = raw + 7 * t;
    ro[0] = al;
    ro[1] = be;
    ro[2] = best[4 * t + 2];
    ro[3] = best[4 * t + 3];
    ro[4] = est_mm(al, be);
    ro[5] = est_um(al, be);
    ro[6] = p_uu_est(al, be);
  }
}

__global__ __launch_bounds__(256) void abn_make_dstar_kernel(double* dstar, const double* pred, const double* resid,
                                                             const uint32_t* idx, int N, long long rows_per_window,
                                                             long long total) {
  for (long long t = (long long)blockIdx.x * blockDim.x + threadIdx.x; t < total;
       t += (long long)gridDim.x * blockDim.x) {
    const long long w = t / rows_per_window;
    const int i = (int)(t % N);
    const size_t wN = (size_t)w * (size_t)N;
    dstar[t] = pred[wN + i] + resid[wN + idx[t]];
  }
}

__global__ __launch_bounds__(256) void abn_gen_idx_kernel(uint32_t* idx, int N, int B, int W, uint64_t seed,
                                                          uint32_t window_offset, uint32_t boot_offset,
                                                          const uint32_t* wid) {
  const int Q = (N + 3) / 4;
  const long long total = (long long)W * B * Q;
  const uint32_t k0 = (uint32_t)seed, k1 = (uint32_t)(seed >> 32);
  for (long long t = (long long)blockIdx.x * blockDim.x + threadIdx.x; t < total;
       t += (long long)gridDim.x * blockDim.x) {
    const int q = (int)(t % Q);
    const long long wb = t / Q;
    const int b = (int)(wb % B);
    const int w = (int)(wb / B);
    uint32_t r[4];
    philox4x32_10((uint32_t)q, boot_offset + (uint32_t)b, wid ? wid[w] : window_offset + (uint32_t)w, kTagIdx, k0, k1, r);
    uint32_t* row = idx + (size_t)wb * (size_t)N;
#pragma unroll
    for (int e = 0; e < 4; ++e) {
      const int i = 4 * q + e;
      if (i < N) row[i] = index_from(r[e], (uint32_t)N);
    }
// ... 5 lines not shown
```

### alphabeta_rs_amd/csrc/abn_common.hpp

```cpp
#pragma once
#include <type_traits>
#include <hip/hip_runtime.h>
#include <stdint.h>

#include "abn_constants.hpp"
#include "abn_philox.h"

namespace abn {

#ifndef ABN_STREAM_WAVES
#define ABN_STREAM_WAVES 2
#endif
constexpr int kStreamWaves = ABN_STREAM_WAVES;

typedef uint32_t u32x4 __attribute__((ext_vector_type(4), aligned(4)));
typedef uint16_t u16x4 __attribute__((ext_vector_type(4), aligned(2)));
typedef double f64x2 __attribute__((ext_vector_type(2), aligned(8)));
typedef uint32_t u32x4_lds __attribute__((ext_vector_type(4)));
typedef double f64x2_lds __attribute__((ext_vector_type(2)));

constexpr int ST_INIT0 = 0;
constexpr int ST_REFLECT = 5;
constexpr int ST_EXPAND = 6;
constexpr int ST_CONTRACT = 7;
constexpr int ST_SHRINK1 = 8;
constexpr int ST_DONE = 12;
constexpr int kFitSuspended = 4;
constexpr unsigned kSliceErrLostEntry = 1u;

struct FitInfoDev {
  double best_cost;
  int32_t iters;
  int32_t evals;
  int32_t status;
  int32_t lanes;
};

struct FitArgs {
  const uint32_t* tri;
  const uint16_t* tid;
  int N, K, T, TP;
  int chain_stride;
  const double* p_uu;
  const double* eqp;
  const double* eqp_w;
  int wstride;
  int dmode;
  const double* D;
  const double* pred;
  const double* resid;
  const uint32_t* idx;
  int smode;
  const double* simplex0;
  const double* model;
  uint64_t seed;
  uint32_t window_offset, boot_offset;
  const uint32_t* wid;
  int tree;
  int strict;
  int W, C;
  int max_iters;
  int iter_cap;
  int resume;
  double* state;
  int* susp_list;
  int* susp_count;
  int shrink_variant;
  int no_skip;
  unsigned long long* skipped;
  unsigned* queue;
  int quantum;
  unsigned park_cap;
  unsigned* park_ht;
  int* parked;
  unsigned* slice_status;
  int tail_cap;
  int spec_resume;
#ifdef ABN_MEASUREMENT_KNOBS
  int prio_mode;
  int prio_t[3];
  int drop_entry;
#endif
  double sd_tol;
  double gap_tol;
  double* best;
  FitInfoDev* info;
  double* raw;
  unsigned long long* dbg;
};

#ifdef ABN_STAMPS
#define ABN_STAMP(slot)                                                           \
  do {                                                                            \
    __builtin_amdgcn_sched_barrier(0);                                            \
    unsigned long long t__;                                                       \
    asm volatile("s_memtime %0\n\ts_waitcnt lgkmcnt(0)" : "=s"(t__)::"memory"); \
    __builtin_amdgcn_sched_barrier(0);                                            \
    seg[slot] += t__ - tprev;                                                     \
    tprev = t__;                                                                  \
  } while (0)
#else
#define ABN_STAMP(slot) \
  do {                  \
  } while (0)
#endif

__device__ __forceinline__ double fma3(double a, double b, double c) { return __builtin_fma(a, b, c); }

struct Gen {
  double g0, g1, g2, g3, g4, g5, g6, g7, g8;
};
__device__ __forceinline__ Gen genmatrix(double alpha, double beta) {
  Gen G;
  G.g0 = (1.0 - alpha) * (1.0 - alpha);
  G.g1 = 2.0 * (1.0 - alpha) * alpha;
  G.g2 = alpha * alpha;
  G.g3 = 0.25 * ((beta + 1.0 - alpha) * (beta + 1.0 - alpha));
  G.g4 = 0.5 * (beta + 1.0 - alpha) * (alpha + 1.0 - beta);
  G.g5 = 0.25 * ((alpha + 1.0 - beta) * (alpha + 1.0 - beta));
  G.g6 = beta * beta;
  G.g7 = 2.0 * (1.0 - beta) * beta;
  G.g8 = (1.0 - beta) * (1.0 - beta);
  return G;
}

__device__ __forceinline__ double p_uu_est(double alpha, double beta) {
  return (beta * ((1.0 - beta) * (1.0 - beta) - (1.0 - alpha) * (1.0 - alpha) - 1.0)) /
         ((alpha + beta) * ((alpha + beta - 1.0) * (alpha + beta - 1.0) - 2.0));
}
__device__ __forceinline__ double est_mm(double alpha, double beta) {
  return (alpha * ((1.0 - alpha) * (1.0 - alpha) - (1.0 - beta) * (1.0 - beta) - 1.0)) /
         ((alpha + beta) * ((alpha + beta - 1.0) * (alpha + beta - 1.0) - 2.0));
}
__device__ __forceinline__ double est_um(double alpha, double beta) {
  return (4.0 * alpha * beta * (alpha + beta - 2.0)) /
         ((alpha + beta) * ((alpha + beta - 1.0) * (alpha + beta - 1.0) - 2.0));
}

template <int G>
__device__ __forceinline__ double group_sum(double v) {
#pragma unroll
  for (int off = 1; off < G; off <<= 1) v = v + __shfl_xor(v, off, kWave);
  return v;
}

template <int CTRL>
__device__ __forceinline__ double dpp_mov(double v) {
  const int lo = __double2loint(v), hi = __double2hiint(v);
  const int nlo = __builtin_amdgcn_update_dpp(lo, lo, CTRL, 0xF, 0xF, true);
  const int nhi = __builtin_amdgcn_update_dpp(hi, hi, CTRL, 0xF, 0xF, true);
  return __hiloint2double(nhi, nlo);
}
constexpr int kDppQuadXor1 = 0xB1;
constexpr int kDppQuadXor2 = 0x4E;
constexpr int kDppRowHalfMirror = 0x141;
constexpr int kDppRowMirror = 0x140;
constexpr int kDppQuadBcast0 = 0x00, kDppQuadBcast1 = 0x55, kDppQuadBcast2 = 0xAA, kDppQuadBcast3 = 0xFF;

template <int G>
__device__ __forceinline__ void build_power_table(Gen Gm, int T, int TP, double* pw, int gl) {
  (void)TP;
  asm("" : "+v"(Gm.g0), "+v"(Gm.g1), "+v"(Gm.g2));
  asm("" : "+v"(Gm.g3), "+v"(Gm.g4), "+v"(Gm.g5));
  asm("" : "+v"(Gm.g6), "+v"(Gm.g7), "+v"(Gm.g8));
  if constexpr (G == 16 || G == 32) {
    if (gl < 12) {
      const int i = gl >> 2, jr = gl & 3;
      const bool j1 = (jr == 1), j2 = (jr >= 2);
      const bool i1 = (i == 1), i2 = (i == 2);
      const double gc0 = j2 ? Gm.g2 : (j1 ? Gm.g1 : Gm.g0);
      const double gc1 = j2 ? Gm.g5 : (j1 ? Gm.g4 : Gm.g3);
      const double gc2 = j2 ? Gm.g8 : (j1 ? Gm.g7 : Gm.g6);
      const int j = j2 ? 2 : jr;
      double* pe = pw + 3 * i + j;
      double r = (i == j) ? 1.0 : 0.0;
      pe[0] = r;
      if (T >= 1) {
        r = i2 ? gc2 : (i1 ? gc1 : gc0);
        pe[kPw] = r;
        double* pk = pe + 2 * kPw;
        for (int k = 2; k <= T; ++k) {
          const double b0 = dpp_mov<kDppQuadBcast0>(r), b1 = dpp_mov<kDppQuadBcast1>(r);
          const double b2 = dpp_mov<kDppQuadBcast2>(r);
          r = fma3(b2, gc2, fma3(b1, gc1, fma3(b0, gc0, 0.0)));
          pk[0] = r;
          pk += kPw;
        }
      }
    }
  } else if (gl < 3) {
    const bool is1 = (gl == 1), is2 = (gl == 2);
    double r0 = (is1 || is2) ? 0.0 : 1.0, r1 = is1 ? 1.0 : 0.0, r2 = is2 ? 1.0 : 0.0;
    double* prow = pw + 3 * gl;
    prow[0] = r0;
    prow[1] = r1;
    prow[2] = r2;
    if (T >= 1) {
      r0 = is2 ? Gm.g6 : (is1 ? Gm.g3 : Gm.g0);
      r1 = is2 ? Gm.g7 : (is1 ? Gm.g4 : Gm.g1);
      r2 = is2 ? Gm.g8 : (is1 ? Gm.g5 : Gm.g2);
      prow[kPw + 0] = r0;
      prow[kPw + 1] = r1;
      prow[kPw + 2] = r2;
      double* pk = prow + 2 * kPw;
#pragma unroll 2
      for (int k = 2; k <= T; ++k) {
        const double n0 = fma3(r2, Gm.g6, fma3(r1, Gm.g3, fma3(r0, Gm.g0, 0.0)));
        const double n1 = fma3(r2, Gm.g7, fma3(r1, Gm.g4, fma3(r0, Gm.g1, 0.0)));
        const double n2 = fma3(r2, Gm.g8, fma3(r1, Gm.g5, fma3(r0, Gm.g2, 0.0)));
        r0 = n0;
        r1 = n1;
        r2 = n2;
        pk[0] = r0;
        pk[1] = r1;
        pk[2] = r2;
        pk += kPw;
      }
    }
  }
}

__device__ __forceinline__ double lane_fetch(double v, int src_lane) {
  const int lo = __builtin_amdgcn_ds_bpermute(src_lane << 2, __double2loint(v));
  const int hi = __builtin_amdgcn_ds_bpermute(src_lane << 2, __double2hiint(v));
  return __hiloint2double(hi, lo);
}

#ifdef ABN_NO_MATRIX_FMA
constexpr bool kMatrixFma = false;
#else
// ... 272 lines not shown
```

### alphabeta_rs_amd/csrc/abn_constants.hpp

```cpp
#pragma once

namespace abn {

constexpr int kWave = 64;
constexpr int kPw = 10;
static_assert(kPw % 2 == 0 && kPw >= 9, "load_matrix reads 16-byte aligned pairs");
constexpr int kStreamVec = 4;
#ifndef ABN_STREAM_BLOCKS
#define ABN_STREAM_BLOCKS 6
#endif
constexpr int kStreamBlocks = ABN_STREAM_BLOCKS;
constexpr int kStrictRowsPerLane = 8;

constexpr int kParkHead = 0, kParkTail = 64, kParkAvail = 128, kParkHeaderInts = 192;
constexpr int kParkShards = 64;

constexpr int kStateSimplex = 0;
constexpr int kStateCosts = 20;
constexpr int kStateBest = 25;
constexpr int kStateBestCost = 29;
constexpr int kStateIterEvals = 30;
constexpr int kStateHaveBest = 31;
constexpr int kStateDoubles = 32;
constexpr int kStateIntIter = 0, kStateIntEvals = 1, kStateIntHaveBest = 2, kStateIntZero = 3;
static_assert(kStateSimplex == 0 && kStateCosts == kStateSimplex + 5 * 4 && kStateBest == kStateCosts + 5 &&
                  kStateBestCost == kStateBest + 4 && kStateIterEvals == kStateBestCost + 1 &&
                  kStateHaveBest == kStateIterEvals + 1 && kStateDoubles == kStateHaveBest + 1,
              "the regions of the parked state tile 0 .. kStateDoubles - 1 exactly");
static_assert(2 * (kStateDoubles - kStateIterEvals) == kStateIntZero + 1, "the int view covers words 30 and 31");

constexpr int kSliceError = 0;
constexpr int kSliceFinished = 1;
constexpr int kSliceHanded = 2;
constexpr int kSliceTailFill = 3;
constexpr int kSliceWords = 4;
constexpr int kPhaseSkipped = 0;
constexpr int kPhaseQueue = 1;
constexpr int kPhaseWords = 2;

constexpr double kGapTolFactor = 64.0;

constexpr int kTreeCanon = 0x10040;

constexpr int kSelChunk = 512;

constexpr int kSpecOutcomes = 10;
constexpr int kSpecTabDoubles = kSpecOutcomes * 12;
constexpr int kSpecPreDoubles = kSpecOutcomes * 3 * 12;
constexpr int kSpecCommDoubles = 8 + 2 * kSpecTabDoubles + 16 + 2 * kSpecPreDoubles + 16;

}
```

### alphabeta_rs_amd/csrc/abn_fit_refill.hpp

```cpp
#pragma once
#include "abn_common.hpp"
#include "abn_fit_kernel.hpp"

namespace abn {

constexpr int ST_IDLE = 13;

#ifndef ABN_REFILL_MIN_WAVES
#define ABN_REFILL_MIN_WAVES 3
#endif
template <int G, int RMAX>
__global__ __launch_bounds__(kWave, ABN_REFILL_MIN_WAVES) void abn_fit_refill_kernel(const FitArgs a) {
  static_assert(RMAX > 0, "resident mode only");
  constexpr int NG = kWave / G;
  constexpr int RR = RMAX;
  extern __shared__ __align__(16) double lds[];

  const int lane = threadIdx.x;
  const int g = lane / G;
  const int gl = lane - g * G;
  const int dim = gl & 3;
  const unsigned total = (unsigned)((long long)a.W * a.C);
  const int N = a.N, K = a.K, TP = a.TP;

  double* pw = lds + (size_t)g * a.chain_stride;
  double* dtab = pw + kPw * TP;
  double* wconst = dtab + ((K + 1) & ~1);
  double* dobs = wconst + 4;
  uint32_t* tri_s = reinterpret_cast<uint32_t*>(dobs + ((N + 1) & ~1));

  unsigned* const pht = a.quantum > 0 ? a.park_ht + (blockIdx.x & (kParkShards - 1)) * kParkHeaderInts : nullptr;
  int* const pk = a.quantum > 0 ? a.parked + (size_t)(blockIdx.x & (kParkShards - 1)) * a.park_cap : nullptr;
  const bool canon = a.tree == kTreeCanon;
  uint32_t tidp[(RR + 1) / 2];
  for (int t = gl; t < K; t += G) tri_s[t] = a.tri[t];
#pragma unroll
  for (int q = 0; q < (RR + 1) / 2; ++q) tidp[q] = 0u;
#pragma unroll
  for (int q = 0; q < RR; ++q) {
    const int i = gl + G * q;
    if (i < N) tidp[q / 2] |= (uint32_t)a.tid[i] << (16 * (q & 1));
  }

  unsigned chain = blockIdx.x * NG + g;
  double vx[5], c[5];
  int st = ST_IDLE;
  int iter = 0, evals = 0;
  double xc = 0.0, x0 = 0.0, xr = 0.0, bx = __builtin_nan("");
  double fr = 0.0, best_cost = __builtin_inf();
  bool have_best = false;
  int fin_status = 2;
  int q_start = 0;
  bool fresh_done = false;
  bool wave_fd = false;
  bool tail_mode = false;
  bool tail_park = false;
  unsigned wstep = 0;
#pragma unroll
  for (int k = 0; k < 5; ++k) {
    vx[k] = 0.0;
    c[k] = 0.0;
  }

  auto setup_chain = [&]() {
    const int w = (int)(chain / (unsigned)a.C);
    const int j = (int)(chain - (unsigned)w * (unsigned)a.C);
    const int wi = w * a.wstride;
    const size_t wN = (size_t)w * (size_t)N;
    if (gl == 0) {
      const double p_uu0 = a.p_uu[wi];
      wconst[0] = p_uu0;
      wconst[1] = 1.0 - p_uu0;
      wconst[2] = a.eqp[wi];
      wconst[3] = a.eqp_w[wi] * (double)N;
    }
    const uint32_t* idx_row = (a.dmode == 1) ? a.idx + (size_t)chain * (size_t)N : nullptr;
    const size_t dN = (a.dmode == 2) ? (size_t)chain * (size_t)N : wN;
#pragma unroll
    for (int q = 0; q < RR; ++q) {
      const int i = gl + G * q;
      if (i < N)
        dobs[i] = (a.dmode == 1) ? a.pred[wN + i] + a.resid[wN + idx_row[i]] : a.D[dN + i];
    }
    if (a.smode == 0) {
      const double* s0 = a.simplex0 + (size_t)chain * 20;
#pragma unroll
      for (int k = 0; k < 5; ++k) vx[k] = s0[4 * k + dim];
    } else {
      const uint32_t k0 = (uint32_t)a.seed, k1 = (uint32_t)(a.seed >> 32);
      const uint32_t wg = a.wid ? a.wid[w] : a.window_offset + (uint32_t)w, bg = a.boot_offset + (uint32_t)j;
      vx[0] = a.model[4 * w + dim];
#pragma unroll
      for (int v = 1; v < 5; ++v) {
        uint32_t r[4];
        philox4x32_10((uint32_t)(v - 1) * 2u + (uint32_t)(dim >> 1), bg, wg, kTagJitter, k0, k1, r);
        const uint32_t r0 = r[0], r1 = r[1], r2 = r[2], r3 = r[3];
        const bool odd = (dim & 1) != 0;
        vx[v] = vary_one(vx[0], odd ? r2 : r0, odd ? r3 : r1);
      }
    }
    iter = 0;
    evals = 0;
    bx = __builtin_nan("");
    best_cost = __builtin_inf();
    have_best = false;
    fin_status = 2;
    fr = 0.0;
    q_start = a.quantum > 0 ? -(int)((chain * 2654435761u >> 16) % (unsigned)a.quantum) : 0;
    st = ST_INIT0;
  };
  auto resume_chain = [&]() {
    const int w = (int)(chain / (unsigned)a.C);
    const int wi = w * a.wstride;
    const size_t wN = (size_t)w * (size_t)N;
    if (gl == 0) {
      const double p_uu0 = a.p_uu[wi];
      wconst[0] = p_uu0;
      wconst[1] = 1.0 - p_uu0;
      wconst[2] = a.eqp[wi];
      wconst[3] = a.eqp_w[wi] * (double)N;
    }
    const uint32_t* idx_row = (a.dmode == 1) ? a.idx + (size_t)chain * (size_t)N : nullptr;
    const size_t dN = (a.dmode == 2) ? (size_t)chain * (size_t)N : wN;
#pragma unroll
    for (int q = 0; q < RR; ++q) {
      const int i = gl + G * q;
      if (i < N)
        dobs[i] = (a.dmode == 1) ? a.pred[wN + i] + a.resid[wN + idx_row[i]] : a.D[dN + i];
    }
    double* sp = a.state + (size_t)chain * kStateDoubles;
    auto ld = [&](int i) { return __hip_atomic_load(sp + i, __ATOMIC_RELAXED, __HIP_MEMORY_SCOPE_AGENT); };
#pragma unroll
    for (int k = 0; k < 5; ++k) {
      vx[k] = ld(kStateSimplex + 4 * k + dim);
      c[k] = ld(kStateCosts + k);
    }
    bx = ld(kStateBest + dim);
    best_cost = ld(kStateBestCost);
    const long long ie = __double_as_longlong(ld(kStateIterEvals));
    iter = (int)(ie & 0xffffffffll);
    evals = (int)(ie >> 32);
    have_best = __double_as_longlong(ld(kStateHaveBest)) != 0;
    fin_status = 2;
    fr = 0.0;
    double acc = vx[0];
    acc = acc + vx[1];
    acc = acc + vx[2];
    acc = acc + vx[3];
    x0 = acc * (1.0 / 4.0);
    xr = x0 + (x0 - vx[4]) * 1.0;
    xc = xr;
    q_start = evals;
    st = ST_REFLECT;
  };
  if (chain < total) setup_chain();
  __syncthreads();

  auto eval = [&](double xd) -> double {
    const double al = dpp_mov<kDppQuadBcast0>(xd), be = dpp_mov<kDppQuadBcast1>(xd);
    const double wt = dpp_mov<kDppQuadBcast2>(xd), ic = dpp_mov<kDppQuadBcast3>(xd);
    const double p_mm = wconst[1];
    const double sv0 = wconst[0], sv1 = wt * p_mm, sv2 = (1.0 - wt) * p_mm;
    const double puu = p_uu_est(al, be);
    const double dq = puu - wconst[2];
    const double pen = wconst[3] * (dq * dq);
    uint32_t tr = tri_s[gl < K ? gl : 0];
    if constexpr (kMatrixFma && G == kWave) build_power_table_mx<G>(al, be, a.T, lds, a.chain_stride, dtab, lane);
    else build_power_table<G>(genmatrix(al, be), a.T, TP, pw, gl);
    __syncthreads();
#pragma unroll 1
    for (int t = gl; t < K; t += G) {
      const uint32_t trn = tri_s[t + G < K ? t + G : 0];
      dtab[t] = triple_dt(tr, pw, TP, sv0, sv1, sv2);
      tr = trn;
    }
    __syncthreads();
    double acc = 0.0;
    constexpr int RC = RR < 8 ? RR : 8;
    constexpr int NA = kWave / G;
    double av[NA];
#pragma unroll
    for (int j = 0; j < NA; ++j) av[j] = 0.0;
#pragma unroll
    for (int q0 = 0; q0 < RR; q0 += RC) {
      double dv[RC], tv[RC], x[RC];
#pragma unroll
      for (int q = 0; q < RC; ++q) {
        const int i = gl + G * (q0 + q);
        dv[q] = dobs[i < N ? i : N - 1];
        tv[q] = dtab[(tidp[(q0 + q) / 2] >> (16 * ((q0 + q) & 1))) & 0xffffu];
      }
#pragma unroll
      for (int q = 0; q < RC; ++q) {
        const double r = dv[q] - ic - tv[q];
        const double term = r * r + pen;
        x[q] = ((gl + G * (q0 + q)) < N) ? term : 0.0;
      }
      if (canon) {
#pragma unroll
        for (int q = 0; q < RC; ++q) av[(q0 + q) % NA] = av[(q0 + q) % NA] + x[q];
      } else {
#pragma unroll
        for (int q = 0; q < RC; ++q) acc = acc + x[q];
      }
    }
    acc = canon ? tree64_finish<G>(av) : group_sum_dpp<G>(acc);
    __syncthreads();
    return acc;
  };

  auto begin_iteration = [&](bool count_iter) {
    const double c_best = c[0];
    if (c_best < best_cost || (__builtin_isinf(c_best) && __builtin_isinf(best_cost) &&
                               (__builtin_signbit(c_best) == __builtin_signbit(best_cost)))) {
      bx = vx[0];
      best_cost = c_best;
      have_best = true;
    }
    if (count_iter) ++iter;
    bool converged = false;
    if (!((c[4] - c[0]) > a.gap_tol)) {
      double sum = 0.0;
#pragma unroll
      for (int k = 0; k < 5; ++k) sum = sum + c[k];
      const double c0 = sum / 5.0;
      double ss = 0.0;
#pragma unroll
      for (int k = 0; k < 5; ++k) ss = ss + (c[k] - c0) * (c[k] - c0);
      const double sd = __builtin_sqrt(1.0 / (5.0 - 1.0) * ss);
      converged = sd < a.sd_tol;
    }
    int status = -1;
    if (converged) status = 0;
    else if (iter >= a.max_iters) status = 1;
    else if (best_cost <= -__builtin_inf()) status = 3;
    bool suspend = false;
    if (a.quantum > 0 && status < 0 && evals - q_start >= a.quantum) {
      int verdict = 0;
      if (gl == 0) {
        const unsigned fq = __hip_atomic_load(a.queue, __ATOMIC_RELAXED, __HIP_MEMORY_SCOPE_AGENT);
        const int av = __hip_atomic_load(reinterpret_cast<int*>(pht) + kParkAvail, __ATOMIC_RELAXED,
                                         __HIP_MEMORY_SCOPE_AGENT);
        const unsigned tl = __hip_atomic_load(pht + kParkTail, __ATOMIC_RELAXED, __HIP_MEMORY_SCOPE_AGENT);
        verdict = ((gridDim.x * NG + fq < total || av > 0) && tl + gridDim.x * NG / kParkShards + NG < a.park_cap) ? 1 : 0;
      }
      suspend = __builtin_amdgcn_ds_bpermute(4 * (g * G), verdict) != 0;
      q_start = evals;
    }
    tail_park = false;
    if (tail_mode && status < 0 && !suspend) {
      suspend = true;
      tail_park = true;
    }
    const bool done = status >= 0 || suspend;
    fin_status = (status >= 0) ? (have_best ? status : 2) : (suspend ? kFitSuspended : fin_status);
    double acc = vx[0];
    acc = acc + vx[1];
    acc = acc + vx[2];
    acc = acc + vx[3];
    x0 = acc * (1.0 / 4.0);
    xr = x0 + (x0 - vx[4]) * 1.0;
    xc = xr;
    st = done ? ST_DONE : ST_REFLECT;
  };

#ifdef ABN_MEASUREMENT_KNOBS
  int prio_cur = 0;
#endif
  while (__ballot(st != ST_IDLE) != 0ull) {
#ifdef ABN_MEASUREMENT_KNOBS
    if (a.prio_mode != 0) {
      const int e = st != ST_IDLE ? evals : 0;
      int m = 0;
#pragma unroll
      for (int j = 0; j < NG; ++j) {
        const int ej = __builtin_amdgcn_readlane(e, j * G);
        m = ej > m ? ej : m;
      }
      int lvl = (m >= a.prio_t[0] ? 1 : 0) + (m >= a.prio_t[1] ? 1 : 0) + (m >= a.prio_t[2] ? 1 : 0);
      if (a.prio_mode == 2) lvl = 3 - lvl;
      if (lvl != prio_cur) {
        prio_cur = lvl;
        if (lvl == 0) __builtin_amdgcn_s_setprio(0);
        else if (lvl == 1) __builtin_amdgcn_s_setprio(1);
        else if (lvl == 2) __builtin_amdgcn_s_setprio(2);
        else __builtin_amdgcn_s_setprio(3);
      }
    }
#endif
    if (a.tail_cap > 0 && wave_fd && !tail_mode && (++wstep & 63u) == 0u) {
      int t = 0;
      if (lane == 0) {
        const unsigned fq = __hip_atomic_load(a.queue, __ATOMIC_RELAXED, __HIP_MEMORY_SCOPE_AGENT);
        const int av = __hip_atomic_load(reinterpret_cast<int*>(pht) + kParkAvail, __ATOMIC_RELAXED, __HIP_MEMORY_SCOPE_AGENT);
        const unsigned fin = __hip_atomic_load(a.slice_status + kSliceFinished, __ATOMIC_RELAXED, __HIP_MEMORY_SCOPE_AGENT);
        t = (gridDim.x * NG + fq >= total && av <= 0 && total - fin <= (unsigned)a.tail_cap) ? 1 : 0;
      }
      tail_mode = __builtin_amdgcn_readfirstlane(t) != 0;
    }
    const bool in_init = st < ST_REFLECT;
    const double f = eval(in_init ? vx[0] : xc);
    const bool is_ref = st == ST_REFLECT, is_exp = st == ST_EXPAND, is_con = st == ST_CONTRACT;
    const bool active = is_ref || is_exp || is_con;
    const bool acc_r = is_ref && (f < c[3]) && (f >= c[0]);
    const bool go_exp = is_ref && !acc_r && (f < c[0]);
    const bool go_con = is_ref && !acc_r && !go_exp && (f >= c[3]);
    const bool nan_ref = is_ref && !acc_r && !go_exp && !go_con;
    const bool keep_r = is_exp && !(f < fr);
    const bool acc_c = is_con && (f < c[4]);
    const bool rej_c = is_con && !acc_c;
    const bool do_insert = acc_r || is_exp || acc_c;
    const bool start_shrink = nan_ref || (rej_c && a.shrink_variant != 0);
    const bool do_begin = do_insert || (rej_c && a.shrink_variant == 0);
    evals += active ? 1 : 0;
    if (rej_c && a.shrink_variant == 0 && a.no_skip == 0) {
      const int rest = a.max_iters - iter - 1;
      evals += 2 * rest;
      iter += rest;
      if (a.skipped && gl == 0 && rest > 0) atomicAdd(a.skipped, 2ull * (unsigned long long)rest);
    }
    const double xi = keep_r ? xr : xc;
    const double fi = keep_r ? fr : f;
    fr = is_ref ? f : fr;
    const double x_e = x0 + (xr - x0) * 2.0;
    const double x_c = x0 + (vx[4] - x0) * 0.5;
    xc = go_exp ? x_e : (go_con ? x_c : xc);
    st = go_exp ? ST_EXPAND : (go_con ? ST_CONTRACT : st);
    if (do_insert) {
      c[4] = fi;
      vx[4] = xi;
      insert_tail<4>(c, vx);
    }
    if (do_begin) begin_iteration(true);
    if (in_init) {
      const double tv = vx[0];
#pragma unroll
      for (int q = 0; q < 4; ++q) {
        c[q] = c[q + 1];
        vx[q] = vx[q + 1];
      }
      c[4] = f;
      vx[4] = tv;
      st = st + 1;
      if (st == ST_REFLECT) {
        evals = 5;
        sort5(c, vx);
        begin_iteration(false);
      }
    }
    if (__ballot(start_shrink) != 0ull) {
#pragma unroll 1
      for (int k = 1; k < 5; ++k) {
        const double nv = vx[0] + (vx[1] - vx[0]) * 0.5;
        const double fk = eval(start_shrink ? nv : xc);
        if (start_shrink) {
          ++evals;
#pragma unroll
          for (int q = 1; q < 4; ++q) {
            c[q] = c[q + 1];
            vx[q] = vx[q + 1];
          }
          c[4] = fk;
          vx[4] = nv;
        }
      }
      if (start_shrink) {
        sort5(c, vx);
        begin_iteration(true);
      }
    }
    if (__ballot(st == ST_DONE) != 0ull) {
      const bool fin = st == ST_DONE;
      const double b0 = dpp_mov<kDppQuadBcast0>(bx), b1 = dpp_mov<kDppQuadBcast1>(bx);
      unsigned nxt = 0xffffffffu;
      const bool parking = fin && fin_status == kFitSuspended;
      if (parking) {
        double* sp = a.state + (size_t)chain * kStateDoubles;
        auto sd = [&](int i, double v) { __hip_atomic_store(sp + i, v, __ATOMIC_RELAXED, __HIP_MEMORY_SCOPE_AGENT); };
        if (gl < 4) {
#pragma unroll
          for (int k = 0; k < 5; ++k) sd(kStateSimplex + 4 * k + gl, vx[k]);
          sd(kStateBest + gl, bx);
        }
        if (gl == 0) {
#pragma unroll
          for (int k = 0; k < 5; ++k) sd(kStateCosts + k, c[k]);
          sd(kStateBestCost, best_cost);
          sd(kStateIterEvals, __longlong_as_double((long long)(unsigned)iter | ((long long)evals << 32)));
          sd(kStateHaveBest, __longlong_as_double(have_best ? 1ll : 0ll));
        }
      } else if (fin) {
        if (gl < 4) a.best[(size_t)chain * 4 + gl] = bx;
        if (gl == 0) {
          if (a.slice_status) atomicAdd(a.slice_status + kSliceFinished, 1u);
          FitInfoDev fo;
          fo.best_cost = best_cost;
          fo.iters = iter;
          fo.evals = evals;
          fo.status = fin_status;
          fo.lanes = a.tree;
          a.info[chain] = fo;
        }
        if (a.raw) {
          double* ro = a.raw + (size_t)chain * 7;
          if (gl < 4) ro[gl] = bx;
          if (gl == 4) ro[4] = est_mm(b0, b1);
          if (gl == 5) ro[5] = est_um(b0, b1);
          if (gl == 6) ro[6] = p_uu_est(b0, b1);
        }
      }
      if (a.quantum > 0) {
        if (__ballot(parking) != 0ull) asm volatile("s_waitcnt vmcnt(0) ; abn: parked state written through" ::: "memory");
        if (parking && tail_park && gl == 0) {
          a.susp_list[atomicAdd(a.susp_count, 1)] = (int)chain;
          atomicAdd(a.slice_status + kSliceHanded, 1u);
        }
        if (parking && !tail_park && gl == 0) {
          const unsigned pos = atomicAdd(pht + kParkTail, 1u);
#ifdef ABN_MEASUREMENT_KNOBS
          if (!(a.drop_entry != 0 && pos == 0 && (blockIdx.x & (kParkShards - 1)) == 0))
#endif
          __hip_atomic_store(pk + pos, (int)chain, __ATOMIC_RELAXED, __HIP_MEMORY_SCOPE_AGENT);
          atomicAdd(reinterpret_cast<int*>(pht) + kParkAvail, 1);
        }
      }
      bool take_parked = false;
      if (fin && gl == 0) {
        if (!fresh_done) {
          const unsigned f = gridDim.x * NG + atomicAdd(a.queue, 1u);
          if (f < total) nxt = f;
          else fresh_done = true;
        }
        if (nxt == 0xffffffffu && a.quantum > 0) {
          int* avail = reinterpret_cast<int*>(pht) + kParkAvail;
          bool claimed = false;
          for (int tries = 0; tries < 1024 && !claimed; ++tries) {
            if (atomicSub(avail, 1) > 0) {
              claimed = true;
            } else {
              atomicAdd(avail, 1);
              if (__hip_atomic_load(avail, __ATOMIC_RELAXED, __HIP_MEMORY_SCOPE_AGENT) <= 0) break;
              __builtin_amdgcn_s_sleep(1);
            }
          }
          if (claimed) {
            const unsigned h = atomicAdd(pht + kParkHead, 1u);
            int cpk;
            unsigned spins = 0;
            while ((cpk = __hip_atomic_load(pk + h, __ATOMIC_RELAXED, __HIP_MEMORY_SCOPE_AGENT)) < 0 && spins < (1u << 24)) {
              __builtin_amdgcn_s_sleep(1);
              ++spins;
            }
            if (cpk >= 0) {
              nxt = (unsigned)cpk;
// ... 26 lines not shown
```

### alphabeta_rs_amd/csrc/abn_fit_spec.hpp

```cpp
#pragma once
#include "abn_common.hpp"

namespace abn {

__device__ __forceinline__ void wave_lds_fence() {
  __builtin_amdgcn_fence(__ATOMIC_RELEASE, "workgroup");
  __builtin_amdgcn_wave_barrier();
  __builtin_amdgcn_fence(__ATOMIC_ACQUIRE, "workgroup");
}

template <int RMAX, bool STRICT = false, bool RESUME = false>
__global__ __launch_bounds__(4 * kWave, RMAX <= 2 ? 4 : 3) void abn_fit_spec_kernel(const FitArgs a) {
  static_assert(!RESUME || !STRICT, "the persistent kernel (whose tail this resumes) has no strict-order form");
  constexpr int G = kWave;
  extern __shared__ __align__(16) double lds[];
  const int wv = __builtin_amdgcn_readfirstlane((int)(threadIdx.x >> 6));
  const int gl = threadIdx.x & 63;
  const int dim = gl & 3;
  const bool keeper = wv == 3;
  long long chain = blockIdx.x;
  if constexpr (RESUME) {
    if ((int)blockIdx.x >= __hip_atomic_load(a.susp_count, __ATOMIC_RELAXED, __HIP_MEMORY_SCOPE_AGENT)) return;
    chain = __hip_atomic_load(a.susp_list + blockIdx.x, __ATOMIC_RELAXED, __HIP_MEMORY_SCOPE_AGENT);
  }
  [[maybe_unused]] auto parked = [&](int i) __attribute__((always_inline)) {
    return __hip_atomic_load(a.state + (size_t)chain * kStateDoubles + i, __ATOMIC_RELAXED, __HIP_MEMORY_SCOPE_AGENT);
  };
  const int w = (int)(chain / a.C);
  const int N = a.N, K = a.K, TP = a.TP;

  double* pw = lds + (size_t)(keeper ? 0 : wv) * a.chain_stride;
  double* dtab = pw + kPw * TP;
  double* wconst = dtab + ((K + 1) & ~1);
  double* dobs = wconst + 4;
  double* xch = lds + (size_t)3 * a.chain_stride;
  double* tab = xch + 8;
  double* pts = tab + 2 * kSpecTabDoubles;
  double* gtab = pts + 16;

  const int wi = w * a.wstride;
  const size_t wN = (size_t)w * (size_t)N;
  uint32_t triv[RMAX], tidp[(RMAX + 1) / 2];
#pragma unroll
  for (int q = 0; q < (RMAX + 1) / 2; ++q) tidp[q] = 0u;
#pragma unroll
  for (int q = 0; q < RMAX; ++q) triv[q] = 0u;
  double vx[5] = {0.0, 0.0, 0.0, 0.0, 0.0};
  if (!keeper) {
    if (gl == 0) {
      const double p_uu0 = a.p_uu[wi];
      wconst[0] = p_uu0;
      wconst[1] = 1.0 - p_uu0;
      wconst[2] = a.eqp[wi];
      wconst[3] = a.eqp_w[wi] * (double)N;
    }
    const uint32_t* idx_row = (a.dmode == 1) ? a.idx + (size_t)chain * (size_t)N : nullptr;
#pragma unroll
    for (int q = 0; q < RMAX; ++q) {
      const int i = gl + G * q;
      triv[q] = (i < K) ? a.tri[i] : 0u;
      if (i < N) {
        tidp[q / 2] |= (uint32_t)a.tid[i] << (16 * (q & 1));
        dobs[i] = (a.dmode == 1) ? a.pred[wN + i] + a.resid[wN + idx_row[i]]
                                 : a.D[wN + i];
      }
    }
  } else {
    if constexpr (RESUME) {
#pragma unroll
      for (int k = 0; k < 5; ++k) vx[k] = parked(kStateSimplex + 4 * k + dim);
    } else if (a.smode == 0) {
      const double* s0 = a.simplex0 + (size_t)chain * 20;
#pragma unroll
      for (int k = 0; k < 5; ++k) vx[k] = s0[4 * k + dim];
    } else {
      const int j = (int)(chain - (long long)w * a.C);
      const uint32_t k0 = (uint32_t)a.seed, k1 = (uint32_t)(a.seed >> 32);
      const uint32_t wg = a.wid ? a.wid[w] : a.window_offset + (uint32_t)w, bg = a.boot_offset + (uint32_t)j;
      vx[0] = a.model[4 * w + dim];
#pragma unroll
      for (int v = 1; v < 5; ++v) {
        uint32_t r[4];
        philox4x32_10((uint32_t)(v - 1) * 2u + (uint32_t)(dim >> 1), bg, wg, kTagJitter, k0, k1, r);
        const uint32_t r0 = r[0], r1 = r[1], r2 = r[2], r3 = r[3];
        const bool odd = (dim & 1) != 0;
        vx[v] = vary_one(vx[0], odd ? r2 : r0, odd ? r3 : r1);
      }
    }
    if (gl < 4) {
#pragma unroll
      for (int k = 0; k < 5; ++k) tab[4 * k + dim] = vx[k];
    }
    if (gl == 4) xch[3] = xch[7] = 0.0;
  }
  __syncthreads();

#ifdef ABN_STAMPS
  unsigned long long seg[8] = {0, 0, 0, 0, 0, 0, 0, 0}, tprev = 0;
  asm volatile("s_memtime %0\n\ts_waitcnt lgkmcnt(0)" : "=s"(tprev)::"memory");
#endif
  double preA = 0.0, preB = 0.0, prePen = 0.0;
  const int mx_x = gl & 3, mx_y = gl >> 4;
  const bool mx_in = (mx_x < 3) && (mx_y < 3) && (((gl >> 2) & 3) == 0);
  const int preA_idx = mx_in ? 3 * mx_y + mx_x : 10, preB_idx = mx_in ? 3 * mx_x + mx_y : 10;
  auto eval = [&](double al, double be, double wt, double ic, bool pre) __attribute__((always_inline)) -> double {
    ABN_STAMP(6);
    const double p_mm = wconst[1];
    const double sv0 = wconst[0], sv1 = wt * p_mm, sv2 = (1.0 - wt) * p_mm;
    double pen;
    if (kMatrixFma && pre) {
      pen = prePen;
      ABN_STAMP(0);
      build_power_table_mx_pre(preA, preB, a.T, pw, dtab, gl);
    } else {
      const double puu = p_uu_est(al, be);
      const double dq = puu - wconst[2];
      pen = wconst[3] * (dq * dq);
      ABN_STAMP(0);
      if constexpr (kMatrixFma) build_power_table_mx<G>(al, be, a.T, pw, 0, dtab, gl);
      else build_power_table<G>(genmatrix(al, be), a.T, TP, pw, gl);
    }
    wave_lds_fence();
    ABN_STAMP(1);
#pragma unroll
    for (int q = 0; q < RMAX; ++q) {
      const int t = gl + G * q;
      if (t < K) dtab[t] = triple_dt(triv[q], pw, TP, sv0, sv1, sv2);
      __builtin_amdgcn_sched_barrier(0);
    }
    wave_lds_fence();
    ABN_STAMP(2);
    double acc = 0.0;
    double dv[RMAX], tv[RMAX];
#pragma unroll
    for (int q = 0; q < RMAX; ++q) {
      const bool in = (gl + G * q) < N;
      dv[q] = in ? dobs[gl + G * q] : 0.0;
      tv[q] = in ? dtab[(tidp[q / 2] >> (16 * (q & 1))) & 0xffffu] : 0.0;
    }
    if constexpr (STRICT) {
      if (RMAX == 1 && N <= 16) {
        const double r = dv[0] - ic - tv[0];
        acc = serial_sum_lanes16(gl < N ? r * r + pen : 0.0, N);
      } else {
        double* term = dobs + ((N + 1) & ~1);
#pragma unroll
        for (int q = 0; q < RMAX; ++q) {
          if ((gl + G * q) < N) {
            const double r = dv[q] - ic - tv[q];
            term[gl + G * q] = r * r + pen;
          }
        }
        wave_lds_fence();
        acc = serial_sum_lds(term, N, 0.0);
      }
    } else {
#pragma unroll
      for (int q = 0; q < RMAX; ++q) {
        if ((gl + G * q) < N) {
          const double r = dv[q] - ic - tv[q];
          acc = acc + (r * r + pen);
        }
      }
      const double one[1] = {acc};
      acc = tree64_finish<G>(one);
    }
    wave_lds_fence();
    ABN_STAMP(3);
    return acc;
  };

  double* ctl = gtab + 2 * kSpecPreDoubles;

  if (!keeper) {
// ... 44 lines not shown
      phase ^= 1;
      const uint32_t lt = (uint32_t)__builtin_amdgcn_fcmp(X, Y, 4 );
      const uint32_t ge = (uint32_t)__builtin_amdgcn_fcmp(X, Y, 3 );
      ABN_STAMP(4);
#ifdef ABN_STAMPS
      ++seg[7];
#endif
      if (lt & 0x400u) break;
      cb ^= 1;
      const int o_r = 4 - __builtin_ctz(~lt | 0x10u), o_c = 9 - __builtin_ctz((~lt >> 4) | 0x10u);
      const uint32_t is_r = lt & (ge >> 3) & 1u;
      const uint32_t is_e = (lt >> 3) & 1u;
      const uint32_t is_c = ge & 1u;
      const int o_e = (lt & 0x200u) ? 4 : o_r;
      const int o = is_r ? o_r : (is_e ? o_e : o_c);
      if ((is_r | is_e | (is_c & (lt >> 8))) & 1u) {
        fetch(o);
        par ^= 1;
        ABN_STAMP(5);
      } else if (is_c && a.shrink_variant == 0) {
        par ^= 1;
      } else {
        __syncthreads();
        put(eval_point(pts + 4 * wv));
        put(eval_point(pts + 12));
        done = pickup();
      }
    }
#ifdef ABN_STAMPS
    if (a.dbg && chain == 0 && wv == 0 && gl == 0) {
      for (int q = 0; q < 8; ++q) a.dbg[q] = seg[q];
      a.dbg[7] = seg[7];
    }
#endif
    return;
  }

  int phase = 0, cb = 0, par = 0;
  double c[5], best_cost = __builtin_inf();
  bool have_best = false;
  int iter = 0;
  auto ctl_begin = [&](bool count_iter, bool& improved) __attribute__((always_inline)) -> int {
    const double c_best = c[0];
    improved = c_best < best_cost || (__builtin_isinf(c_best) && __builtin_isinf(best_cost) &&
                                      (__builtin_signbit(c_best) == __builtin_signbit(best_cost)));
    best_cost = improved ? c_best : best_cost;
    have_best = have_best || improved;
    if (count_iter) ++iter;
    bool converged = false;
    if (!((c[4] - c[0]) > a.gap_tol)) {
      double sum = 0.0;
#pragma unroll
      for (int k = 0; k < 5; ++k) sum = sum + c[k];
      const double c0 = sum / 5.0;
      double ss = 0.0;
#pragma unroll
      for (int k = 0; k < 5; ++k) ss = ss + (c[k] - c0) * (c[k] - c0);
      const double sd = __builtin_sqrt(1.0 / (5.0 - 1.0) * ss);
      converged = sd < a.sd_tol;
    }
    int status = -1;
    if (converged) status = 0;
    else if (iter >= a.max_iters) status = 1;
    else if (best_cost <= -__builtin_inf()) status = 3;
    return status;
  };
  double xr = 0.0, x_e = 0.0, x_c = 0.0, bx = __builtin_nan("");
  int evals = 0;
  const int oq = gl >> 2;
  const int o_kind = oq < 4 ? 0 : (oq == 4 ? 1 : 2);
  const int o_rank = oq < 4 ? oq : (oq == 4 ? 0 : oq - 5);
  auto emit_pre = [&](double r_, double e_, double c_, int parity) __attribute__((always_inline)) {
    const double ar = dpp_mov<kDppQuadBcast0>(r_), br = dpp_mov<kDppQuadBcast1>(r_);
    const double ae = dpp_mov<kDppQuadBcast0>(e_), be = dpp_mov<kDppQuadBcast1>(e_);
    const double ac = dpp_mov<kDppQuadBcast0>(c_), bc = dpp_mov<kDppQuadBcast1>(c_);
    const double al_t = dim == 0 ? ar : (dim == 1 ? ae : ac);
    const double be_t = dim == 0 ? br : (dim == 1 ? be : bc);
    const Gen Gt = genmatrix(al_t, be_t);
    const double puu = p_uu_est(al_t, be_t);
    const double dq = puu - wconst[2];
    const double pen = wconst[3] * (dq * dq);
    if (oq < kSpecOutcomes && dim < 3) {
      double* g = gtab + parity * kSpecPreDoubles + (oq * 3 + dim) * 12;
      g[0] = Gt.g0;
      g[1] = Gt.g1;
      g[2] = Gt.g2;
      g[3] = Gt.g3;
      g[4] = Gt.g4;
      g[5] = Gt.g5;
      g[6] = Gt.g6;
      g[7] = Gt.g7;
      g[8] = Gt.g8;
      g[9] = pen;
      g[10] = 0.0;
    }
  };
  auto ctl_write = [&](int status_now) __attribute__((always_inline)) {
    if (gl < 5) ctl[8 * cb + gl] = gl == 0 ? c[0] : (gl == 1 ? c[1] : (gl == 2 ? c[2] : (gl == 3 ? c[3] : c[4])));
    if (gl == 5) ctl[8 * cb + 5] = status_now >= 0 ? 1.0 : 0.0;
  };
  auto take = [&](double& f0, double& f1, double& f2) __attribute__((always_inline)) {
    const double* buf = xch + 4 * phase;
    __syncthreads();
    f0 = buf[0];
    f1 = buf[1];
    f2 = buf[2];
    phase ^= 1;
  };
  bool improved;
  int status = -1;
  double f1, f2;
  auto publish = [&]() __attribute__((always_inline)) -> bool {
    ctl_write(status);
    if (status < 0) {
      double acc = vx[0];
      acc = acc + vx[1];
      acc = acc + vx[2];
      acc = acc + vx[3];
      const double x0 = acc * (1.0 / 4.0);
      xr = x0 + (x0 - vx[4]) * 1.0;
      x_e = x0 + (xr - x0) * 2.0;
      x_c = x0 + (vx[4] - x0) * 0.5;
      if (gl < 4) {
        double* t = tab + par * kSpecTabDoubles;
        t[dim] = xr;
        t[4 + dim] = x_e;
        t[8 + dim] = x_c;
      }
      if constexpr (kMatrixFma) emit_pre(xr, x_e, x_c, par);
    }
    __syncthreads();
    par ^= 1;
    return status >= 0;
  };

  if constexpr (RESUME) {
#pragma unroll
    for (int k = 0; k < 5; ++k) c[k] = parked(kStateCosts + k);
    bx = parked(kStateBest + dim);
    best_cost = parked(kStateBestCost);
    const long long ie = __double_as_longlong(parked(kStateIterEvals));
    iter = (int)(ie & 0xffffffffll);
    evals = (int)(ie >> 32);
    have_best = __double_as_longlong(parked(kStateHaveBest)) != 0;
  } else {
    take(c[0], c[1], c[2]);
    take(c[3], c[4], f2);
    evals = 5;
    sort5(c, vx);
    status = ctl_begin(false, improved);
    if (improved) bx = vx[0];
  }
  bool done = publish();

  while (!done) {
    {
      const double A = o_kind == 0 ? xr : (o_kind == 1 ? x_e : x_c);
      const double e0 = o_rank == 0 ? A : vx[0];
      const double e1 = o_rank == 1 ? A : (o_rank < 1 ? vx[0] : vx[1]);
      const double e2 = o_rank == 2 ? A : (o_rank < 2 ? vx[1] : vx[2]);
      const double e3 = o_rank == 3 ? A : (o_rank < 3 ? vx[2] : vx[3]);
      const double xw = o_rank == 4 ? A : vx[3];
      double acc = e0;
      acc = acc + e1;
      acc = acc + e2;
      acc = acc + e3;
      const double x0 = acc * (1.0 / 4.0);
      const double nr = x0 + (x0 - xw) * 1.0;
      const double ne = x0 + (nr - x0) * 2.0;
      const double nc = x0 + (xw - x0) * 0.5;
      if (oq < kSpecOutcomes) {
        double* t = tab + par * kSpecTabDoubles + oq * 12;
        t[dim] = nr;
        t[4 + dim] = ne;
        t[8 + dim] = nc;
      }
      if constexpr (kMatrixFma) emit_pre(nr, ne, nc, par);
    }
    double fr, fe, fc;
    take(fr, fe, fc);
    cb ^= 1;
    int kind, which = 0;
    double fi = fr;
    int spent;
    if (fr < c[3] && fr >= c[0]) {
      kind = 0;
      spent = 1;
    } else if (fr < c[0]) {
      kind = 0;
      spent = 2;
      const bool take_e = fe < fr;
      which = take_e ? 1 : 0;
      fi = take_e ? fe : fr;
    } else if (fr >= c[3]) {
      spent = 2;
      if (fc < c[4]) {
        kind = 0;
        which = 2;
        fi = fc;
      } else {
        kind = a.shrink_variant ? 2 : 1;
      }
    } else {
      kind = 2;
      spent = 1;
    }
    evals += spent;
    if (kind == 0) {
      const bool b3 = fi < c[3], b2 = b3 && (fi < c[2]), b1 = b2 && (fi < c[1]), b0 = b1 && (fi < c[0]);
      const int p = 4 - ((b3 ? 1 : 0) + (b2 ? 1 : 0) + (b1 ? 1 : 0) + (b0 ? 1 : 0));
      const int o = which == 0 ? p : (which == 1 ? 4 : 5 + p);
      const double* t = tab + par * kSpecTabDoubles + o * 12;
      c[4] = fi;
      vx[4] = which == 0 ? xr : (which == 1 ? x_e : x_c);
      insert_tail<4>(c, vx);
      status = ctl_begin(true, improved);
      if (improved) bx = vx[0];
      ctl_write(status);
      xr = t[dim];
      x_e = t[4 + dim];
      x_c = t[8 + dim];
      par ^= 1;
    } else if (kind == 1) {
      if (a.no_skip == 0) {
        const int rest = a.max_iters - iter - 1;
        evals += 2 * rest;
        iter += rest;
        if (a.skipped && gl == 0 && rest > 0) atomicAdd(a.skipped, 2ull * (unsigned long long)rest);
      }
      status = ctl_begin(true, improved);
      ctl_write(status);
      par ^= 1;
    } else {
#pragma unroll
      for (int k = 1; k < 5; ++k) {
        vx[k] = vx[0] + (vx[k] - vx[0]) * 0.5;
        if (gl < 4) pts[4 * (k - 1) + dim] = vx[k];
      }
      __syncthreads();
      take(c[1], c[2], c[3]);
      take(c[4], f1, f2);
      evals += 4;
      sort5(c, vx);
      status = ctl_begin(true, improved);
      if (improved) bx = vx[0];
      done = publish();
      continue;
    }
    if (status >= 0) {
      __syncthreads();
      break;
    }
  }

  const double b0 = dpp_mov<kDppQuadBcast0>(bx), b1 = dpp_mov<kDppQuadBcast1>(bx);
  if (gl < 4) a.best[(size_t)chain * 4 + gl] = bx;
  if (gl == 0) {
#ifdef ABN_DIAG_RESUME_COUNT
    if constexpr (RESUME) atomicAdd(a.slice_status + kSliceFinished, 0x10000u);
#else
    if constexpr (RESUME) atomicAdd(a.slice_status + kSliceFinished, 1u);
#endif
    FitInfoDev fo;
    fo.best_cost = best_cost;
    fo.iters = iter;
    fo.evals = evals;
    fo.status = have_best ? status : 2;
    fo.lanes = a.tree;
    a.info[chain] = fo;
  }
  if (a.raw) {
    double* ro = a.raw + (size_t)chain * 7;
    if (gl < 4) ro[gl] = bx;
    if (gl == 4) ro[4] = est_mm(b0, b1);
    if (gl == 5) ro[5] = est_um(b0, b1);
    if (gl == 6) ro[6] = p_uu_est(b0, b1);
  }
}

}
```

### alphabeta_rs_amd/csrc/abn_route.hpp

```cpp
#pragma once
#include <algorithm>
#include <cstddef>
#include <cstring>

#include "../../include/abneutral.h"
#include "abn_constants.hpp"

namespace abn {

constexpr size_t kDefaultDynLds = 64 * 1024;
constexpr size_t kMaxDynLds = 160 * 1024;
constexpr size_t lds_limit(int lanes) { return lanes == kWave ? kMaxDynLds : kDefaultDynLds; }
constexpr size_t kLdsResidentMax = 40 * 1024;
#ifndef ABN_PERSIST_WAVES_PER_CU
#define ABN_PERSIST_WAVES_PER_CU 12
#endif
constexpr long long kPersistWavesPerCu = ABN_PERSIST_WAVES_PER_CU;
#ifndef ABN_PERSIST_WAVES_SMALL_PER_CU
#define ABN_PERSIST_WAVES_SMALL_PER_CU 8
#endif
constexpr long long kPersistWavesSmallPerCu = ABN_PERSIST_WAVES_SMALL_PER_CU;
constexpr long long persist_waves(int cus) { return kPersistWavesPerCu * cus; }
constexpr long long persist_waves_small(int cus) { return kPersistWavesSmallPerCu * cus; }
constexpr long long persist_waves_for(int cus, long long blocks) {
// ... 83 lines not shown
inline PedigreeRoute route_pedigree(int n, int k, int t, int requested, int strict) {
  PedigreeRoute p{};
  p.n = n;
  p.k = k;
  p.tp = t + 1;
  p.kp = (k + 1) & ~1;
  p.chain_stride = scratch_stride(p.tp, p.kp);
  p.requested = requested;
  p.strict = strict ? 1 : 0;
  p.lanes = pick_lanes(n, requested, p.chain_stride);
  p.streams = resident_rows(n, k, p.chain_stride, p.lanes, p.strict) == 0;
  p.tree = p.strict ? 1 : (requested != 0 || p.streams) ? p.lanes : kTreeCanon;
  p.reported_tree = (!p.strict && p.streams) ? (p.lanes | ((kStreamVec - 1) << 8)) : p.tree;
  p.wide_ok = (!p.strict && p.tree != kTreeCanon) ? p.tree == kWave
                                                   : resident_rows(n, k, p.chain_stride, kWave, p.strict) != 0;
  const int r64 = pick_rmax(n, kWave);
  p.spec_rows = r64 == 1 || r64 == 2 || r64 == 4 ? r64 : 8;
  p.spec_ok = r64 != 0 && r64 <= 8 && p.wide_ok && spec_lds(p.chain_stride, n, p.strict) <= kLdsResidentMax;
  p.cost_lanes = p.strict ? kWave : p.lanes;
  p.cost_tree = p.strict ? kWave : p.tree;
  p.cost_lds = ((size_t)(kWave / p.cost_lanes) * p.chain_stride + (p.strict ? kSelChunk : 0)) * sizeof(double);
  p.select_lds = select_lds(p.tp, p.kp);
  if ((size_t)(kWave / p.lanes) * stream_stride(p.chain_stride, p.lanes, p.strict) * sizeof(double) > lds_limit(p.lanes) ||
      ((size_t)p.chain_stride + kSelChunk) * sizeof(double) > kMaxDynLds)
    p.refusal = kLdsRefusal;
  if (p.cost_lds > lds_limit(p.cost_lanes)) p.cost_refusal = "pedigree needs more LDS than supported";
  if (p.select_lds > kMaxDynLds) p.select_refusal = "pedigree needs more LDS than supported";
  return p;
}

constexpr long long spec_max_chains(int cus, int n_rows, int phase) {
  const long long mx = kPhaseASpecPerCu * cus;
  const bool small = pick_rmax(n_rows, kWave) <= 2;
  if (phase == 0) return small ? mx * 4 : mx * 2;
  return small ? mx * 3 / 2 : mx * 3 / 4;
}
constexpr bool plan_two_pass(long long start_chains, int max_iters_start, int no_fixed_point_skip, int shrink, int strict) {
  return start_chains > kTwoPassChains && max_iters_start > kPhaseACap && no_fixed_point_skip != 0 && shrink == 0 && !strict;
}

struct PhaseRoute {
  bool spec;
  int lanes;
  bool two_pass;
};

inline PhaseRoute route_phase(const PedigreeRoute& p, int phase, long long plan_chains, int cus, int dmode, bool whole,
                              bool two_pass, const char* force = nullptr) {
  const bool can_wide = p.requested == 0 && dmode != 2 && p.wide_ok;
  const bool can_spec = can_wide && p.spec_ok;
  PhaseRoute r{false, p.lanes, false};
  r.spec = can_spec && plan_chains <= spec_max_chains(cus, p.n, phase);
  if (!r.spec && can_wide && plan_chains <= (phase == 0 ? kPhaseAWidePerCu * cus : (3LL * cus / 4) * p.lanes)) r.lanes = kWave;
  if (force && !strcmp(force, "spec")) r.spec = can_spec;
  if (force && !strcmp(force, "wide")) r = {false, can_wide ? kWave : p.lanes, false};
  if (force && !strcmp(force, "packed")) r = {false, p.lanes, false};
  if (r.spec) r.lanes = kWave;
  r.two_pass = !r.spec && phase == 0 && whole && two_pass;
  return r;
}

struct LaunchOffer {
  bool queue = false;
  bool parking = false;
  int pass = 0;
};

struct LaunchRoute {
  int status;
  const char* error;
  int kind;
  KernelKey key;
  unsigned grid, block;
  size_t lds;
  int chain_stride;
  int tree;
  int quantum;
  int tail_cap;
};

constexpr bool persistent_by_size(int lanes, long long chains, int cus) {
  const int ng = kWave / lanes;
  return ng > 1 && (chains + ng - 1) / ng > persist_waves_small(cus);
}
constexpr size_t plan_sliced_chains(const PedigreeRoute& p, size_t chains, int cus, int window_groups) {
  return kQuantum > 0 && persistent_by_size(p.lanes, (long long)chains, cus) && chains * kStateDoubles * sizeof(double) <= kSliceStateMax &&
                 chains < (1u << 27) && window_groups <= 1
             ? chains : 0;
}
constexpr int tail_cap_for(const PedigreeRoute& p, long long blocks, int cus) {
  if (p.tree != kTreeCanon || !p.spec_ok) return 0;
  return (int)((pick_rmax(p.n, kWave) <= 2 ? (blocks == persist_waves(cus) ? 8LL : 4LL) : 2LL) * cus);
}

inline LaunchRoute refuse(const char* why) {
  LaunchRoute r{};
  r.status = ABN_ERR_INVALID_ARG;
  r.error = why;
  return r;
}

inline LaunchRoute route_spec(const PedigreeRoute& p, long long chains, bool resume) {
  LaunchRoute r{};
  if (chains <= 0) return r;
  if (!p.spec_ok) return refuse("internal: the speculative kernel does not apply to this pedigree");
  r.kind = ABN_KERNEL_SPECULATIVE;
  r.key = {kFamSpec, kWave, p.spec_rows, false, p.strict != 0, resume};
  r.grid = (unsigned)chains;
  r.block = 4 * kWave;
  r.chain_stride = p.chain_stride + spec_extra(p.n, p.strict);
  r.lds = spec_lds(p.chain_stride, p.n, p.strict);
  r.tree = p.strict ? 1 : kTreeCanon;
  return r;
}
inline LaunchRoute route_tail_resume(const PedigreeRoute& p, int tail_cap) { return route_spec(p, tail_cap, true); }

inline LaunchRoute route_launch(const PedigreeRoute& p, const PhaseRoute& ph, long long chains, int cus, const LaunchOffer& o) {
  if (ph.spec) return route_spec(p, chains, false);
  LaunchRoute r{};
  if (chains <= 0) return r;
  const int lanes = ph.lanes, ng = kWave / lanes;
  if (p.strict && o.pass != 0) return refuse("internal: strict order has no two-pass variant");
  r.tree = p.strict ? 1 : p.tree == kTreeCanon ? kTreeCanon : lanes;
  int rows = resident_rows(p.n, p.k, p.chain_stride, lanes, p.strict);
  if (rows > 0) {
    r.chain_stride = p.chain_stride + resident_extra(p.n, p.k, p.strict);
  } else {
    if (r.tree == kTreeCanon) return refuse("internal: the canonical tree needs an LDS-resident pedigree");
    r.chain_stride = stream_stride(p.chain_stride, lanes, p.strict);
    rows = (!p.strict && p.n < 2 * kStreamBlocks * kStreamVec * lanes) ? -1 : 0;
  }
  r.lds = (size_t)ng * (size_t)r.chain_stride * sizeof(double);
  if (r.lds > lds_limit(lanes)) return refuse(kLdsRefusal);
  long long blocks = (chains + ng - 1) / ng;
  if (blocks > 0x7fffffffLL || chains > 0x7fffffffLL) return refuse("too many chains for one launch");
  r.block = kWave;
  if (o.queue && !p.strict && rows > 0 && o.pass == 0 && persistent_by_size(lanes, chains, cus)) {
    blocks = persist_waves_for(cus, blocks);
    r.kind = ABN_KERNEL_PERSISTENT;
    r.key = {kFamRefill, lanes, rows, false, false, false};
    if (o.parking && kQuantum > 0) {
      const long long q = (5LL * kQuantum * chains / (blocks * ng) / 8 + 63) & ~63LL;
      r.quantum = (int)std::min<long long>(4LL * kQuantum, std::max<long long>(kQuantum, q));
      r.tail_cap = tail_cap_for(p, blocks, cus);
    }
  } else {
    r.kind = o.pass != 0 ? ABN_KERNEL_TWO_PASS : rows <= 0 ? ABN_KERNEL_STREAM : ABN_KERNEL_RESIDENT;
    r.key = {kFamFit, lanes, rows, o.pass != 0, p.strict != 0, false};
  }
  r.grid = (unsigned)blocks;
  return r;
}

}
```

### include/abneutral.h

```cpp
#ifndef ABNEUTRAL_H
#define ABNEUTRAL_H

#include <stdint.h>

#ifdef __cplusplus
extern "C" {
#endif

#define ABN_VERSION_MAJOR 0
#define ABN_VERSION_MINOR 1

typedef enum abn_status {
  ABN_OK = 0,
  ABN_ERR_INVALID_ARG = 1,
  ABN_ERR_BAD_PEDIGREE = 2,
  ABN_ERR_NO_DEVICE = 3,
  ABN_ERR_HIP = 4,
  ABN_ERR_NO_FINITE_FIT = 5,
  ABN_ERR_STATE = 6
} abn_status;

#define ABN_FIT_CONVERGED 0
#define ABN_FIT_MAX_ITERS 1
#define ABN_FIT_NONFINITE 2
// ... 20 lines not shown
  int32_t iters;
  int32_t evals;
  int32_t status;
  int32_t lanes;
} abn_fit_info;

void abn_default_options(abn_options* opts);
int abn_device_count(int* count);
#define ABN_STREAM_DEFAULT ((void*)(intptr_t)-1)
int abn_init(int device_ordinal, void* stream, abn_ctx** ctx);
int abn_shutdown(abn_ctx* ctx);
int abn_device_info(const abn_ctx* ctx, int32_t* out4);
const char* abn_last_error(const abn_ctx* ctx);
const char* abn_status_string(int status);
int abn_version(void);

int abn_reduction_tree(const abn_options* opts, const double* generations, int32_t n_rows, int32_t* tree);

int abn_cost_batch(abn_ctx* ctx, const abn_options* opts, const double* pedigree, int32_t n_rows,
                   double p_uu0, double eqp, double eqp_weight, const double* candidates, int64_t m,
                   const double* pred, const double* resid, const uint32_t* idx,
                   const uint32_t* cand_to_boot, int64_t n_boot_rows, double* cost, double* dt1t2,
                   double* p_uu_inf);

int abn_fit_batch(abn_ctx* ctx, const abn_options* opts, const double* pedigree, int32_t n_rows,
                  double p_uu0, double eqp, double eqp_weight, const double* simplex0, int64_t f,
                  const double* dobs_rows, int32_t max_iters, double* best, abn_fit_info* info);

int abn_gen_start_simplices(uint64_t seed, uint32_t window, int32_t n_starts, double max_divergence,
                            double* simplex0);
int abn_gen_boot_simplices(uint64_t seed, uint32_t window, uint32_t b0, int64_t nb,
                           const double params[4], double* simplex0);
int abn_gen_boot_indices(abn_ctx* ctx, uint64_t seed, uint32_t window, uint32_t b0, int64_t nb,
                         int32_t n_rows, uint32_t* idx);

int abn_ab_neutral_run(abn_ctx* ctx, const abn_options* opts, const double* pedigree, int32_t n_rows,
                       double p0uu, double eqp, double eqp_weight, int32_t n_starts, double* model,
                       double* pred, double* resid, double* all_models, abn_fit_info* info,
                       double* lse);

int abn_select_best(abn_ctx* ctx, const double* pedigree, int32_t n_rows, double p0uu, const double* models,
                    int32_t n_models, int32_t* best_index, double* model, double* pred, double* resid,
                    double* lse);

int abn_bootstrap_rows(abn_ctx* ctx, const double* best, int64_t n_boot, double* raw);

int abn_boot_model_run(abn_ctx* ctx, const abn_options* opts, const double* pedigree, int32_t n_rows,
                       const double* model, const double* pred, const double* resid, double p0uu,
                       double eqp, double eqp_weight, int32_t n_boot, double* raw,
                       abn_fit_info* info);

int abn_analyze(const double* raw, int64_t n_boot, double* out32);

int abn_analyze_batch(abn_ctx* ctx, const double* raw, int32_t n_windows, int64_t n_boot, double* out,
                      int32_t* first_bad);
int abn_analyze_batch_dev(abn_ctx* ctx, const void* dev_raw, int32_t n_windows, int64_t n_boot, void* dev_out,
                          void* dev_first_bad, double* kernel_ms);

int abn_pairwise_divergence(abn_ctx* ctx, const uint8_t* codes, int32_t n_samples, int64_t n_sites,
                            uint64_t* diff, uint64_t* both, double* dvalue);
int abn_pairwise_divergence_dev(abn_ctx* ctx, const void* dev_codes, int32_t n_samples, int64_t n_sites,
                                void* dev_diff, void* dev_both, void* dev_dvalue, double* kernel_ms);
int abn_pairwise_divergence_windows(abn_ctx* ctx, const uint8_t* codes, int32_t n_samples, int64_t row_stride,
                                    const int64_t* site_begin, const int64_t* site_end, int32_t n_windows,
                                    uint64_t* diff, uint64_t* both, double* dvalue);
int abn_pairwise_divergence_windows_dev(abn_ctx* ctx, const void* dev_codes, int32_t n_samples, int64_t row_stride,
                                        const int64_t* site_begin, const int64_t* site_end, int32_t n_windows,
                                        void* dev_diff, void* dev_both, void* dev_dvalue, double* kernel_ms);

int64_t abn_packed_row_stride(int64_t n_sites);
int abn_pack_codes(const uint8_t* codes, int32_t n_samples, int64_t n_sites, int64_t src_row_stride, uint8_t* packed,
                   int64_t row_stride_bytes);
int abn_unpack_codes(const uint8_t* packed, int32_t n_samples, int64_t n_sites, int64_t row_stride_bytes, uint8_t* codes,
                     int64_t dst_row_stride);
int abn_pairwise_divergence_packed(abn_ctx* ctx, const uint8_t* packed, int32_t n_samples, int64_t n_sites,
                                   int64_t row_stride_bytes, uint64_t* diff, uint64_t* both, double* dvalue);
int abn_pairwise_divergence_packed_dev(abn_ctx* ctx, const void* dev_packed, int32_t n_samples, int64_t n_sites,
                                       int64_t row_stride_bytes, void* dev_diff, void* dev_both, void* dev_dvalue,
                                       double* kernel_ms);

int abn_pairwise_divergence_windows_packed(abn_ctx* ctx, const uint8_t* packed, int32_t n_samples, int64_t n_sites,
                                           int64_t row_stride_bytes, const int64_t* site_begin, const int64_t* site_end,
                                           int32_t n_windows, uint64_t* diff, uint64_t* both, double* dvalue);
int abn_pairwise_divergence_windows_packed_dev(abn_ctx* ctx, const void* dev_packed, int32_t n_samples, int64_t n_sites,
                                               int64_t row_stride_bytes, const int64_t* site_begin,
                                               const int64_t* site_end, int32_t n_windows, void* dev_diff,
                                               void* dev_both, void* dev_dvalue, double* kernel_ms);

typedef struct abn_windows abn_windows;
typedef struct abn_windows_params {
  uint32_t cutoff;
  uint32_t step;
  uint32_t size;
  int32_t absolute;
  int32_t n_upstream;
  int32_t n_gene;
  int32_t n_downstream;
} abn_windows_params;
int abn_windows_create(abn_ctx* ctx, const abn_windows_params* params, int32_t n_samples, const int64_t* site_offset,
                       const uint32_t* pos, const uint32_t* gene_start, const uint32_t* gene_end, const uint8_t* flags,
                       const uint8_t* code, const double* level, abn_windows** out);
int abn_windows_destroy(abn_windows* h);
int abn_windows_info(const abn_windows* h, int32_t* n_windows, int64_t* row_stride, int64_t* n_sites);
int abn_windows_stats(const abn_windows* h, int64_t* count, double* level_sum, double* level_sum_kept, int64_t* kept);
int abn_windows_layout(const abn_windows* h, int64_t* begin, int64_t* end, int32_t* ragged);
int abn_windows_packed(abn_windows* h, uint8_t* host_out);
int abn_windows_packed_device_ptr(abn_windows* h, void** dev_ptr);
int abn_windows_pairwise(abn_windows* h, uint64_t* diff, uint64_t* both, double* dvalue);

typedef struct abn_genes abn_genes;
typedef struct abn_gene_rule {
  uint32_t cutoff;
  int32_t cutoff_gene_length;
} abn_gene_rule;
int abn_genes_create(abn_ctx* ctx, int32_t n_lists, const int32_t* list_chromosome, const int32_t* list_kind,
                     const int64_t* list_offset, const uint32_t* gene_start, const uint32_t* gene_end,
                     const uint8_t* gene_strand, abn_genes** out);
int abn_genes_destroy(abn_genes* h);
int abn_genes_choose(abn_genes* h, const abn_gene_rule* rule, int32_t n_samples, const int64_t* site_offset,
                     const int32_t* chromosome, const uint32_t* start, const uint32_t* end, const uint8_t* strand,
                     uint32_t* gene_start, uint32_t* gene_end, uint8_t* flags, double* kernel_ms);
int abn_genes_choose_dev(abn_genes* h, const abn_gene_rule* rule, int32_t n_samples, const int64_t* site_offset,
                         const void* dev_chromosome, const void* dev_start, const void* dev_end, const void* dev_strand,
                         void* dev_gene_start, void* dev_gene_end, void* dev_flags, double* kernel_ms);
int abn_windows_create_sites(abn_ctx* ctx, const abn_windows_params* params, abn_genes* genes, const abn_gene_rule* rule,
                             int32_t n_samples, const int64_t* site_offset, const int32_t* chromosome,
                             const uint32_t* start, const uint32_t* end, const uint8_t* strand, const uint8_t* code,
                             const double* level, abn_windows** out);

typedef struct abn_sites abn_sites;
typedef struct abn_sites_params {
  int64_t slab_bytes;
  int32_t skip_lines;
  int32_t reserved;
} abn_sites_params;
int abn_sites_parse(abn_ctx* ctx, const char* text, int64_t n_bytes, const abn_sites_params* params, abn_sites** out);
int abn_sites_destroy(abn_sites* h);
int abn_sites_info(const abn_sites* h, int64_t* n_sites, int64_t* n_deferred, int64_t* n_lines, double* kernel_ms);
int abn_sites_fetch(const abn_sites* h, int64_t* line, int32_t* chromosome, uint32_t* start, uint32_t* end,
                    uint8_t* strand, double* posteriormax, uint8_t* status, uint8_t* status_flag, double* meth_lvl);
int abn_sites_deferred(const abn_sites* h, int64_t* line, int64_t* offset, int64_t* length);

int abn_plan_create(abn_ctx* ctx, const abn_options* opts, const double* generations ,
                    int32_t n_rows, int32_t n_windows, int32_t n_starts, int32_t n_boot,
                    uint32_t window_offset, uint32_t boot_offset, abn_plan** plan);
int abn_plan_destroy(abn_plan* plan);
int abn_plan_set_window_ids(abn_plan* plan, const uint32_t* ids);
int abn_plan_set_windows(abn_plan* plan, const double* d_obs, const double* p0uu, const double* eqp,
                         const double* eqp_weight);
int abn_plan_run(abn_plan* plan);
int abn_plan_run_phase(abn_plan* plan, int32_t phase );
int abn_plan_sync(abn_plan* plan);
int abn_plan_tail_handed(abn_plan* plan, int64_t* out2);
int abn_plan_kernel_ms(abn_plan* plan, double* ms3);
int abn_plan_raw_device_ptr(abn_plan* plan, void** dev_ptr);
int abn_plan_bind_raw(abn_plan* plan, void* dev_ptr);
int abn_plan_download(abn_plan* plan, double* models, double* pred, double* resid, double* raw,
                      abn_fit_info* info_a, abn_fit_info* info_b, int32_t* best_start);
int abn_plan_analyze(abn_plan* plan, double* out, int32_t* first_bad);
int abn_plan_failed_windows(abn_plan* plan, int32_t* n_failed);
int abn_plan_counters(abn_plan* plan, int64_t* out5);
int abn_plan_device_bytes(abn_plan* plan, int64_t* bytes);
#define ABN_KERNEL_NONE 0
#define ABN_KERNEL_SPECULATIVE 1
#define ABN_KERNEL_RESIDENT 2
#define ABN_KERNEL_PERSISTENT 3
#define ABN_KERNEL_STREAM 4
#define ABN_KERNEL_TWO_PASS 5
int abn_plan_last_kernels(abn_plan* plan, int32_t* out4);

typedef struct abn_multi abn_multi;
int abn_multi_create(const int32_t* devices, int32_t n_devices, const abn_options* opts,
                     const double* generations , int32_t n_rows, int32_t n_windows, int32_t n_starts,
                     int32_t n_boot, abn_multi** out);
int abn_multi_destroy(abn_multi* m);
const char* abn_multi_last_error(const abn_multi* m);
int abn_multi_set_window_ids(abn_multi* m, const uint32_t* ids);
int abn_multi_set_windows(abn_multi* m, const double* d_obs, const double* p0uu, const double* eqp,
                          const double* eqp_weight);
int abn_multi_run(abn_multi* m);
int abn_multi_sync(abn_multi* m);
int abn_multi_shard(abn_multi* m, int32_t device_index, int32_t* out4);
int abn_multi_plan_shard(int32_t n_windows, int32_t n_boot, int32_t n_devices, int32_t device_index, int32_t* out4);
int abn_multi_kernel_ms(abn_multi* m, int32_t device_index, double* ms3);
int abn_multi_raw_device_ptr(abn_multi* m, int32_t device_index, void** dev_ptr);
int abn_multi_download(abn_multi* m, double* models, double* pred, double* resid, double* raw,
                       abn_fit_info* info_a, abn_fit_info* info_b, int32_t* best_start);
int abn_multi_analyze(abn_multi* m, double* out, int32_t* first_bad);
int abn_multi_counters(abn_multi* m, int64_t* out5);
int abn_multi_rccl_available(int* ok);

#ifdef __cplusplus
}
#endif
#endif
```

Measured before the change: 3.084 million fits/s.

## Start bootstrap fits speculatively once a quorum of starts converges

Phase A start fits now count their completions. Once a quorum (about 80% of the starts) has converged, the remaining starts are parked and resumed on a side stream, and bootstrap phase B launches at once using the model selected from the quorum. A compare kernel checks whether the final best start differs. If it does, a guard word tells the running phase B to abort and phase B is redone with the corrected model. The intent is to overlap the straggling start fits with bootstrap work, at the cost of extra kernels, polling overhead and a possible full redo.

New measurement: 3.251 million fits/s, median of 6. 1.05x the previous value.

```diff
diff --git a/alphabeta_rs_amd/__init__.py b/alphabeta_rs_amd/__init__.py
--- a/alphabeta_rs_amd/__init__.py
+++ b/alphabeta_rs_amd/__init__.py
@@ -35,7 +35,7 @@
     "abn_status_string", "abn_version", "abn_cost_batch", "abn_fit_batch", "abn_gen_start_simplices",
     "abn_gen_boot_simplices", "abn_gen_boot_indices", "abn_ab_neutral_run", "abn_boot_model_run",
     "abn_analyze", "abn_select_best", "abn_bootstrap_rows", "abn_pairwise_divergence", "abn_plan_create", "abn_plan_destroy", "abn_plan_set_windows", "abn_plan_run",
-    "abn_plan_run_phase", "abn_plan_sync", "abn_plan_tail_handed", "abn_plan_kernel_ms", "abn_plan_raw_device_ptr",
+    "abn_plan_run_phase", "abn_plan_sync", "abn_plan_tail_handed", "abn_plan_set_early_bootstraps", "abn_plan_early_bootstraps", "abn_plan_kernel_ms", "abn_plan_raw_device_ptr",
     "abn_plan_bind_raw", "abn_plan_download", "abn_plan_counters", "abn_plan_device_bytes",
     "abn_plan_set_window_ids", "abn_plan_failed_windows",
     "abn_multi_create", "abn_multi_destroy", "abn_multi_last_error", "abn_multi_set_windows", "abn_multi_run",
@@ -196,6 +196,8 @@
     L.abn_plan_run_phase.argtypes = [vp, C.c_int32]
     L.abn_plan_sync.argtypes = [vp]
     L.abn_plan_tail_handed.argtypes = [vp, C.POINTER(C.c_int64)]
+    L.abn_plan_set_early_bootstraps.argtypes = [vp, C.c_int32]
+    L.abn_plan_early_bootstraps.argtypes = [vp, C.POINTER(C.c_int32)]
     L.abn_plan_kernel_ms.argtypes = [vp, dp]
     L.abn_plan_raw_device_ptr.argtypes = [vp, C.POINTER(vp)]
     L.abn_plan_bind_raw.argtypes = [vp, vp]
@@ -659,6 +661,14 @@
         self.ctx._check(self._L.abn_plan_tail_handed(self._h, out))
         return int(out[0]), int(out[1])
 
+    def set_early_bootstraps(self, mode: int):
+        self.ctx._check(self._L.abn_plan_set_early_bootstraps(self._h, mode))
+
+    def early_bootstraps(self):
+        out = (C.c_int32 * 4)()
+        self.ctx._check(self._L.abn_plan_early_bootstraps(self._h, out))
+        return {"eligible": bool(out[0]), "quorum": int(out[1]), "parked": int(out[2]), "miss": bool(out[3])}
+
     def kernel_ms(self):
         ms = np.zeros(3)
         self.ctx._check(self._L.abn_plan_kernel_ms(self._h, _dp(ms)))
diff --git a/alphabeta_rs_amd/csrc/abn_api.hip b/alphabeta_rs_amd/csrc/abn_api.hip
--- a/alphabeta_rs_amd/csrc/abn_api.hip
+++ b/alphabeta_rs_amd/csrc/abn_api.hip
@@ -561,7 +561,6 @@
   bool twopass_a = false;
   DevBuf<int> slice_buf;
   unsigned slice_cap = 0;
-  DevBuf<unsigned> slice_status;
   long long persist_expected[2] = {0, 0};
   long long tail_handed[2] = {0, 0};
   int32_t last_kernels[4] = {0, 0, 0, 0};
@@ -570,7 +569,28 @@
   hipEvent_t ev[kPlanEvents] = {};
   hipEvent_t ev_fork = nullptr;
   std::vector<hipEvent_t> ev_join;
+  EarlyRoute early{};
+  int early_mode = 1;
+  bool early_ran = false;
+  int32_t early_parked = 0, early_miss = 0;
+  DevBuf<double> early_state;
+  DevBuf<int> early_list;
+  DevBuf<double> sel_model, sel_pred, sel_resid;
+  DevBuf<int32_t> sel_best;
 };
+
+constexpr size_t kPlanWords64 = (size_t)kPhaseSlots * kPhaseWords + ((size_t)kEarlyWords + (size_t)kPhaseSlots * kSliceWords + 1) / 2;
+static unsigned* early_words(const abn_plan* p) { return reinterpret_cast<unsigned*>(p->skipped.p + kPhaseSlots * kPhaseWords); }
+static unsigned* slice_words(const abn_plan* p, int slot) { return early_words(p) + kEarlyWords + kSliceWords * slot; }
+struct PlanWordsHost {
+  unsigned long long phase[kPhaseSlots][kPhaseWords];
+  unsigned early[kEarlyWords];
+  unsigned slice[kPhaseSlots][kSliceWords];
+};
+static_assert(sizeof(PlanWordsHost) <= kPlanWords64 * sizeof(unsigned long long) && sizeof(PlanWordsHost) % 8 == 0 &&
+                  offsetof(PlanWordsHost, early) == kPhaseSlots * kPhaseWords * sizeof(unsigned long long) &&
+                  offsetof(PlanWordsHost, slice) == offsetof(PlanWordsHost, early) + kEarlyWords * sizeof(unsigned),
+              "PlanWordsHost mirrors the plan's words");
 
 extern "C" int abn_plan_destroy(abn_plan* p) {
   if (!p) return ABN_ERR_INVALID_ARG;
@@ -640,8 +660,7 @@
   PALLOC(bestB, W * B * 4);
   PALLOC(infoB, W * B);
   PALLOC(raw_own, W * B * 7);
-  PALLOC(skipped, 2 * kPhaseWords);
-  PALLOC(slice_status, 2 * kSliceWords);
+  PALLOC(skipped, kPlanWords64);
   p->twopass_a = plan_two_pass((long long)n_windows * n_starts, p->opt.max_iters_start, p->opt.no_fixed_point_skip,
                                p->opt.shrink_on_failed_contraction, p->opt.strict_order);
   if (p->twopass_a) {
@@ -656,6 +675,20 @@
   }
   p->stream_b = n_boot > 0 && p->route.streams && p->opt.stream_mode == 0;
   if (p->stream_b) PALLOC(dstar, W * B * N);
+  p->early = route_early_bootstraps(p->route, n_windows, n_starts, n_boot, c->cus, p->opt.window_groups, p->twopass_a,
+                                    p->slice_cap > 0);
+  if (p->stream_b) p->early = EarlyRoute{false, 0};
+#ifdef ABN_MEASUREMENT_KNOBS
+  if (getenv("ABN_PHASE_A_KERNEL") || getenv("ABN_PHASE_B_KERNEL")) p->early = EarlyRoute{false, 0};
+#endif
+  if (p->early.eligible) {
+    PALLOC(early_state, S * kStateDoubles);
+    PALLOC(early_list, S);
+    PALLOC(sel_model, W * 4);
+    PALLOC(sel_pred, W * N);
+    PALLOC(sel_resid, W * N);
+    PALLOC(sel_best, W);
+  }
 #undef PALLOC
   p->raw = p->raw_own.p;
   for (auto& ev : p->ev)
@@ -767,8 +800,9 @@
   return a;
 }
 
-static int launch_phase(abn_plan* p, int phase, FitArgs& a, hipStream_t st, bool timed) {
-  abn_ctx* c = p->ctx;
+static int launch_phase(abn_plan* p, int phase, FitArgs& a, hipStream_t st, bool timed, int slot = -1) {
+  abn_ctx* c = p->ctx;
+  if (slot < 0) slot = phase;
   const bool whole = a.W == p->W;
   const char* force = nullptr;
 #ifdef ABN_MEASUREMENT_KNOBS
@@ -779,10 +813,10 @@
   LaunchOffer offer;
   offer.queue = whole;
   offer.parking = whole && p->slice_cap > 0;
-  a.skipped = p->skipped.p + kPhaseWords * phase + kPhaseSkipped;
+  a.skipped = p->skipped.p + kPhaseWords * slot + kPhaseSkipped;
   if (whole) {
-    a.queue = reinterpret_cast<unsigned*>(p->skipped.p + kPhaseWords * phase + kPhaseQueue);
-    a.slice_status = p->slice_status.p + kSliceWords * phase;
+    a.queue = reinterpret_cast<unsigned*>(p->skipped.p + kPhaseWords * slot + kPhaseQueue);
+    a.slice_status = slice_words(p, slot);
   }
   if (offer.parking) {
     a.park_cap = p->slice_cap;
@@ -790,6 +824,11 @@
     a.parked = p->slice_buf.p + kParkShards * kParkHeaderInts;
     a.state = p->nm_state.p;
     a.susp_list = p->susp_list.p;
+  }
+  if (a.quorum_words) {
+    a.state = p->early_state.p;
+    a.susp_list = p->early_list.p;
+    a.susp_count = reinterpret_cast<int*>(early_words(p) + kEarlyParked);
   }
   int kind = ABN_KERNEL_NONE, rc;
   if (ph.two_pass) {
@@ -814,19 +853,14 @@
   return ABN_OK;
 }
 
-static int enqueue_phase_a(abn_plan* p, int w0, int wn, hipStream_t st, bool timed) {
-  abn_ctx* c = p->ctx;
-  FitArgs a = phase_args(p, 0, w0, wn);
-  if (timed) HIPCHK(c, hipEventRecord(p->ev[kEvFitA], st));
-  if (int rc = launch_phase(p, 0, a, st, timed)) return rc;
-  if (timed) HIPCHK(c, hipEventRecord(p->ev[kEvFitAEnd], st));
+static SelectArgs select_args(const abn_plan* p, int w0, int wn) {
   const WindowOffsets o = window_offsets(p, w0);
   SelectArgs s{};
   fill_topology(s, p->topo, p->dtopo);
-  s.p_uu = a.p_uu;
-  s.D = a.D;
-  s.models = a.best;
-  s.info = a.info;
+  s.p_uu = p->p_uu.p + o.w;
+  s.D = p->D.p + o.rows;
+  s.models = p->bestA.p + o.starts * 4;
+  s.info = p->infoA.p + o.starts;
   s.W = wn;
   s.S = p->S;
   s.lse = p->lse.p + o.starts;
@@ -834,15 +868,36 @@
   s.pred = p->pred.p + o.rows;
   s.resid = p->resid.p + o.rows;
   s.best_start = p->best_start.p + o.w;
+  return s;
+}
+
+static int enqueue_phase_a(abn_plan* p, int w0, int wn, hipStream_t st, bool timed, bool early = false) {
+  abn_ctx* c = p->ctx;
+  FitArgs a = phase_args(p, 0, w0, wn);
+  if (early) {
+    a.quorum_words = early_words(p) + kEarlyCount;
+    a.quorum = p->early.quorum;
+  }
+  if (timed) HIPCHK(c, hipEventRecord(p->ev[kEvFitA], st));
+  if (int rc = launch_phase(p, 0, a, st, timed)) return rc;
+  if (timed) HIPCHK(c, hipEventRecord(p->ev[kEvFitAEnd], st));
+  const SelectArgs s = select_args(p, w0, wn);
   if (timed) HIPCHK(c, hipEventRecord(p->ev[kEvSelect], st));
   if (int rc = launch_select(c, s, p->route.select_lds, st)) return rc;
   if (timed) HIPCHK(c, hipEventRecord(p->ev[kEvSelectEnd], st));
   return ABN_OK;
 }
 
-static int enqueue_phase_b(abn_plan* p, int w0, int wn, hipStream_t st, bool timed) {
+struct PhaseGuard {
+  const unsigned* word = nullptr;
+  int stop = 0, poll = 0, slot = -1;
+};
+static int enqueue_phase_b(abn_plan* p, int w0, int wn, hipStream_t st, bool timed, const PhaseGuard& guard = PhaseGuard{}) {
   abn_ctx* c = p->ctx;
   FitArgs a = phase_args(p, 1, w0, wn);
+  a.guard = guard.word;
+  a.guard_stop = guard.stop;
+  a.guard_poll = guard.poll;
   if (timed) HIPCHK(c, hipEventRecord(p->ev[kEvFitB], st));
   if (p->stream_b) {
     double* dst = p->dstar.p + window_offsets(p, w0).boots * (size_t)p->N;
@@ -854,14 +909,14 @@
     a.dmode = 2;
     a.D = dst;
   }
-  if (int rc = launch_phase(p, 1, a, st, timed)) return rc;
+  if (int rc = launch_phase(p, 1, a, st, timed, guard.slot)) return rc;
   if (timed) HIPCHK(c, hipEventRecord(p->ev[kEvFitBEnd], st));
   return ABN_OK;
 }
 
 static int clear_phase_words(abn_plan* p, int first, int n) {
-  HIPCHK(p->ctx, hipMemsetAsync(p->skipped.p + kPhaseWords * first, 0, (size_t)n * kPhaseWords * sizeof(unsigned long long),
-                                p->ctx->stream));
+  const size_t words = n == 2 ? kPlanWords64 : (size_t)n * kPhaseWords;
+  HIPCHK(p->ctx, hipMemsetAsync(p->skipped.p + kPhaseWords * first, 0, words * sizeof(unsigned long long), p->ctx->stream));
   return ABN_OK;
 }
 
@@ -889,6 +944,7 @@
     int rc = enqueue_phase_b(p, 0, p->W, c->stream, true);
     if (rc) return rc;
     p->ran_b = true;
+    p->early_ran = false;
     return ABN_OK;
   }
   return set_err(c, ABN_ERR_INVALID_ARG, "phase must be 0 or 1");
@@ -899,10 +955,92 @@
   return plan_run_phase(p, phase, kClearOwnPhase);
 }
 
+static int ensure_fork_join(abn_plan* p, int streams) {
+  abn_ctx* c = p->ctx;
+  while ((int)c->side.size() < streams) {
+    hipStream_t st = nullptr;
+    HIPCHK(c, hipStreamCreateWithFlags(&st, hipStreamNonBlocking));
+    c->side.push_back(st);
+  }
+  if (!p->ev_fork) HIPCHK(c, hipEventCreateWithFlags(&p->ev_fork, hipEventDisableTiming));
+  while ((int)p->ev_join.size() < streams) {
+    hipEvent_t e = nullptr;
+    HIPCHK(c, hipEventCreateWithFlags(&e, hipEventDisableTiming));
+    p->ev_join.push_back(e);
+  }
+  return ABN_OK;
+}
+
+constexpr int kGuardPoll = 16;
+
+static int plan_run_early(abn_plan* p) {
+  abn_ctx* c = p->ctx;
+  HIPCHK(c, hipSetDevice(c->device));
+  if (int rc = ensure_fork_join(p, 1)) return rc;
+  hipStream_t side = c->side[0];
+  unsigned* ew = early_words(p);
+  if (int rc = clear_phase_words(p, 0, 2)) return rc;
+  if (int rc = enqueue_phase_a(p, 0, p->W, c->stream, true, true)) return rc;
+  HIPCHK(c, hipEventRecord(p->ev_fork, c->stream));
+  HIPCHK(c, hipStreamWaitEvent(side, p->ev_fork, 0));
+  {
+    FitArgs a = phase_args(p, 0, 0, p->W);
+    const LaunchRoute t = route_tail_resume(p->route, p->S - p->early.quorum);
+    if (t.status) return set_err(c, t.status, t.error);
+    a.chain_stride = t.chain_stride;
+    a.tree = t.tree;
+    a.spec_resume = 1;
+    a.state = p->early_state.p;
+    a.susp_list = p->early_list.p;
+    a.susp_count = reinterpret_cast<int*>(ew + kEarlyParked);
+    a.slice_status = ew + kEarlySink;
+    a.skipped = p->skipped.p + kPhaseSkipped;
+    if (int rc = launch_route(c, t, a, side)) return rc;
+  }
+  const SelectArgs to = select_args(p, 0, p->W);
+  SelectArgs all = to;
+  all.model = p->sel_model.p;
+  all.pred = p->sel_pred.p;
+  all.resid = p->sel_resid.p;
+  all.best_start = p->sel_best.p;
+  if (int rc = launch_select(c, all, p->route.select_lds, side)) return rc;
+  hipLaunchKernelGGL(abn_early_compare_kernel, dim3(1), dim3(kWave), 0, side, to.best_start, all.best_start, p->W, ew + kEarlyMiss);
+  HIPCHK(c, hipGetLastError());
+  HIPCHK(c, hipEventRecord(p->ev_join[0], side));
+  PhaseGuard g;
+  g.word = ew + kEarlyMiss;
+  g.stop = 1;
+  g.poll = kGuardPoll;
+  if (int rc = enqueue_phase_b(p, 0, p->W, c->stream, true, g)) return rc;
+  HIPCHK(c, hipStreamWaitEvent(c->stream, p->ev_join[0], 0));
+  hipLaunchKernelGGL(abn_early_adopt_kernel, dim3(1), dim3(256), 0, c->stream, all, to);
+  HIPCHK(c, hipGetLastError());
+  g.stop = 0;
+  g.poll = 0;
+  g.slot = kSlotRedo;
+  if (int rc = enqueue_phase_b(p, 0, p->W, c->stream, false, g)) return rc;
+  HIPCHK(c, hipEventRecord(p->ev[kEvFitBEnd], c->stream));
+  p->phase_a_done = true;
+  p->ran_a = true;
+  p->ran_b = true;
+  p->early_ran = true;
+  return ABN_OK;
+}
+
+static bool early_applies(const abn_plan* p) { return p->early.eligible && p->early_mode != 0; }
+
+extern "C" int abn_plan_set_early_bootstraps(abn_plan* p, int32_t mode) {
+  if (!p) return ABN_ERR_INVALID_ARG;
+  if (mode != 0 && mode != 1) return set_err(p->ctx, ABN_ERR_INVALID_ARG, "early bootstraps: mode must be 0 (off) or 1 (auto)");
+  p->early_mode = mode;
+  return ABN_OK;
+}
+
 extern "C" int abn_plan_run(abn_plan* p) {
   if (!p) return ABN_ERR_INVALID_ARG;
   abn_ctx* c = p->ctx;
   if (!p->windows_set) return set_err(c, ABN_ERR_STATE, "abn_plan_set_windows has not been called");
+  if (early_applies(p)) return plan_run_early(p);
   int groups = p->opt.window_groups > 0 ? p->opt.window_groups : 1;
   groups = std::max(1, std::min(groups, p->W));
   if (groups == 1 || p->S <= 0 || p->B <= 0) {
@@ -913,17 +1051,7 @@
     return rc;
   }
   HIPCHK(c, hipSetDevice(c->device));
-  while ((int)c->side.size() < groups) {
-    hipStream_t st = nullptr;
-    HIPCHK(c, hipStreamCreateWithFlags(&st, hipStreamNonBlocking));
-    c->side.push_back(st);
-  }
-  if (!p->ev_fork) HIPCHK(c, hipEventCreateWithFlags(&p->ev_fork, hipEventDisableTiming));
-  while ((int)p->ev_join.size() < groups) {
-    hipEvent_t e = nullptr;
-    HIPCHK(c, hipEventCreateWithFlags(&e, hipEventDisableTiming));
-    p->ev_join.push_back(e);
-  }
+  if (int rc = ensure_fork_join(p, groups)) return rc;
   if (int rc = clear_phase_words(p, 0, 2)) return rc;
   HIPCHK(c, hipEventRecord(p->ev_fork, c->stream));
   for (int g = 0; g < groups; ++g) {
@@ -939,19 +1067,24 @@
   p->phase_a_done = true;
   p->ran_a = true;
   p->ran_b = true;
+  p->early_ran = false;
   return ABN_OK;
 }
 
 static int verify_persistent(abn_plan* p) {
   abn_ctx* c = p->ctx;
   HIPCHK(c, hipSetDevice(c->device));
-  unsigned sl[2][kSliceWords] = {};
+  PlanWordsHost h{};
   const bool check = p->persist_expected[0] > 0 || p->persist_expected[1] > 0;
-  if (check) HIPCHK(c, hipMemcpyAsync(sl, p->slice_status.p, sizeof sl, hipMemcpyDeviceToHost, c->stream));
+  if (check || p->early_ran) HIPCHK(c, hipMemcpyAsync(&h, p->skipped.p, sizeof h, hipMemcpyDeviceToHost, c->stream));
   HIPCHK(c, hipStreamSynchronize(c->stream));
+  if (p->early_ran) {
+    p->early_parked = (int32_t)h.early[kEarlyParked];
+    p->early_miss = h.early[kEarlyMiss] != 0 ? 1 : 0;
+  }
   for (int ph = 0; ph < 2 && check; ++ph) {
     if (p->persist_expected[ph] <= 0) continue;
-    const unsigned* s = sl[ph];
+    const unsigned* s = h.slice[ph == 1 && p->early_ran && p->early_miss ? kSlotRedo : ph];
     p->tail_handed[ph] = (long long)s[kSliceHanded];
     if (s[kSliceError] != 0 || (long long)s[kSliceFinished] != p->persist_expected[ph])
       return set_err(c, ABN_ERR_HIP, std::string("persistent fit launch of phase ") + (ph ? "B" : "A") + " finished " +
@@ -973,6 +1106,16 @@
   const int rc = verify_persistent(p);
   out2[0] = p->persist_expected[0] > 0 ? p->tail_handed[0] : 0;
   out2[1] = p->persist_expected[1] > 0 ? p->tail_handed[1] : 0;
+  return rc;
+}
+
+extern "C" int abn_plan_early_bootstraps(abn_plan* p, int32_t* out4) {
+  if (!p || !out4) return ABN_ERR_INVALID_ARG;
+  const int rc = verify_persistent(p);
+  out4[0] = p->early.eligible ? 1 : 0;
+  out4[1] = p->early.eligible ? p->early.quorum : 0;
+  out4[2] = p->early_ran ? p->early_parked : 0;
+  out4[3] = p->early_ran ? p->early_miss : 0;
   return rc;
 }
 
@@ -1065,16 +1208,17 @@
   auto add = [&](const DevBuf<FitInfoDev>& b, int phase) -> int {
     if (!b.n) return ABN_OK;
     h.resize(b.n);
-    unsigned long long sk = 0;
+    PlanWordsHost wd{};
     HIPCHK(c, hipMemcpyAsync(h.data(), b.p, b.bytes(), hipMemcpyDeviceToHost, c->stream));
-    HIPCHK(c, hipMemcpyAsync(&sk, p->skipped.p + kPhaseWords * phase + kPhaseSkipped, sizeof sk, hipMemcpyDeviceToHost, c->stream));
+    HIPCHK(c, hipMemcpyAsync(&wd, p->skipped.p, sizeof wd, hipMemcpyDeviceToHost, c->stream));
     HIPCHK(c, hipStreamSynchronize(c->stream));
     for (const auto& f : h) {
       out5[0] += 1;
       out5[1] += f.evals;
       out5[2] += f.iters;
     }
-    out5[3 + phase] = (int64_t)sk;
+    const int slot = phase == 1 && p->early_ran && wd.early[kEarlyMiss] != 0 ? kSlotRedo : phase;
+    out5[3 + phase] = (int64_t)wd.phase[slot][kPhaseSkipped];
     return ABN_OK;
   };
   int rc = ABN_OK;
@@ -1115,7 +1259,8 @@
   t += p->simplexA.bytes() + p->bestA.bytes() + p->model.bytes() + p->lse.bytes() + p->bestB.bytes();
   t += p->raw_own.bytes() + p->infoA.bytes() + p->infoB.bytes() + p->best_start.bytes() + p->idx.bytes();
   t += p->dstar.bytes() + p->nm_state.bytes() + p->susp_list.bytes() + p->skipped.bytes() + p->slice_buf.bytes();
-  t += p->slice_status.bytes() + p->wid.bytes();
+  t += p->wid.bytes() + p->early_state.bytes() + p->early_list.bytes() + p->sel_model.bytes() + p->sel_pred.bytes();
+  t += p->sel_resid.bytes() + p->sel_best.bytes();
   t += p->dtopo.tri.bytes() + p->dtopo.tid.bytes();
   *bytes = (int64_t)t;
   return ABN_OK;
diff --git a/alphabeta_rs_amd/csrc/abn_aux_kernels.hpp b/alphabeta_rs_amd/csrc/abn_aux_kernels.hpp
--- a/alphabeta_rs_amd/csrc/abn_aux_kernels.hpp
+++ b/alphabeta_rs_amd/csrc/abn_aux_kernels.hpp
@@ -104,6 +104,22 @@
     a.resid[wN + i] = a.D[wN + i] - p;
   }
   if (lane < 4) a.model[4 * w + lane] = x[lane];
+}
+
+__global__ __launch_bounds__(kWave) void abn_early_compare_kernel(const int32_t* early, const int32_t* all, int W, unsigned* miss) {
+  for (int w = threadIdx.x; w < W; w += kWave)
+    if (early[w] != all[w]) __hip_atomic_store(miss, 1u, __ATOMIC_RELAXED, __HIP_MEMORY_SCOPE_AGENT);
+}
+__global__ __launch_bounds__(256) void abn_early_adopt_kernel(const SelectArgs from, const SelectArgs to) {
+  const long long rows = (long long)to.W * to.N, n = rows > 4LL * to.W ? rows : 4LL * to.W;
+  for (long long i = (long long)blockIdx.x * blockDim.x + threadIdx.x; i < n; i += (long long)gridDim.x * blockDim.x) {
+    if (i < rows) {
+      to.pred[i] = from.pred[i];
+      to.resid[i] = from.resid[i];
+    }
+    if (i < 4LL * to.W) to.model[i] = from.model[i];
+    if (i < to.W) to.best_start[i] = from.best_start[i];
+  }
 }
 
 struct CostArgs {
diff --git a/alphabeta_rs_amd/csrc/abn_common.hpp b/alphabeta_rs_amd/csrc/abn_common.hpp
--- a/alphabeta_rs_amd/csrc/abn_common.hpp
+++ b/alphabeta_rs_amd/csrc/abn_common.hpp
@@ -76,6 +76,11 @@
   unsigned* slice_status;
   int tail_cap;
   int spec_resume;
+  unsigned* quorum_words;
+  int quorum;
+  const unsigned* guard;
+  int guard_stop;
+  int guard_poll;
 #ifdef ABN_MEASUREMENT_KNOBS
   int prio_mode;
   int prio_t[3];
diff --git a/alphabeta_rs_amd/csrc/abn_constants.hpp b/alphabeta_rs_amd/csrc/abn_constants.hpp
--- a/alphabeta_rs_amd/csrc/abn_constants.hpp
+++ b/alphabeta_rs_amd/csrc/abn_constants.hpp
@@ -37,6 +37,14 @@
 constexpr int kPhaseSkipped = 0;
 constexpr int kPhaseQueue = 1;
 constexpr int kPhaseWords = 2;
+constexpr int kPhaseSlots = 3, kSlotRedo = 2;
+constexpr int kEarlyCount = 0;
+constexpr int kEarlyFlag = 1;
+constexpr int kEarlyParked = 2;
+constexpr int kEarlyMiss = 3;
+constexpr int kEarlySink = 4;
+constexpr int kEarlyWords = kEarlySink + kSliceWords;
+static_assert(kEarlyFlag == kEarlyCount + 1, "FitArgs::quorum_words: the flag follows the counter");
 
 constexpr double kGapTolFactor = 64.0;
 
diff --git a/alphabeta_rs_amd/csrc/abn_fit_refill.hpp b/alphabeta_rs_amd/csrc/abn_fit_refill.hpp
--- a/alphabeta_rs_amd/csrc/abn_fit_refill.hpp
+++ b/alphabeta_rs_amd/csrc/abn_fit_refill.hpp
@@ -16,6 +16,10 @@
   constexpr int RR = RMAX;
   extern __shared__ __align__(16) double lds[];
 
+  auto guard_says_stop = [&]() {
+    return (__hip_atomic_load(a.guard, __ATOMIC_RELAXED, __HIP_MEMORY_SCOPE_AGENT) != 0u) == (a.guard_stop != 0);
+  };
+  if (a.guard && guard_says_stop()) return;
   const int lane = threadIdx.x;
   const int g = lane / G;
   const int gl = lane - g * G;
@@ -56,6 +60,7 @@
   bool tail_mode = false;
   bool tail_park = false;
   unsigned wstep = 0;
+  unsigned gstep = 0;
 #pragma unroll
   for (int k = 0; k < 5; ++k) {
     vx[k] = 0.0;
@@ -298,8 +303,12 @@
       }
       tail_mode = __builtin_amdgcn_readfirstlane(t) != 0;
     }
+    const bool guard_due = a.guard_poll > 0 && (++gstep & (unsigned)(a.guard_poll - 1)) == 0u;
+    int guard_stop_now = 0;
+    if (guard_due && lane == 0) guard_stop_now = guard_says_stop() ? 1 : 0;
     const bool in_init = st < ST_REFLECT;
     const double f = eval(in_init ? vx[0] : xc);
+    if (guard_due && __builtin_amdgcn_readfirstlane(guard_stop_now) != 0) break;
     const bool is_ref = st == ST_REFLECT, is_exp = st == ST_EXPAND, is_con = st == ST_CONTRACT;
     const bool active = is_ref || is_exp || is_con;
     const bool acc_r = is_ref && (f < c[3]) && (f >= c[0]);
diff --git a/alphabeta_rs_amd/csrc/abn_fit_spec.hpp b/alphabeta_rs_amd/csrc/abn_fit_spec.hpp
--- a/alphabeta_rs_amd/csrc/abn_fit_spec.hpp
+++ b/alphabeta_rs_amd/csrc/abn_fit_spec.hpp
@@ -20,6 +20,7 @@
   const bool keeper = wv == 3;
   long long chain = blockIdx.x;
   if constexpr (RESUME) {
+    if (a.guard && ((__hip_atomic_load(a.guard, __ATOMIC_RELAXED, __HIP_MEMORY_SCOPE_AGENT) != 0u) == (a.guard_stop != 0))) return;
     if ((int)blockIdx.x >= __hip_atomic_load(a.susp_count, __ATOMIC_RELAXED, __HIP_MEMORY_SCOPE_AGENT)) return;
     chain = __hip_atomic_load(a.susp_list + blockIdx.x, __ATOMIC_RELAXED, __HIP_MEMORY_SCOPE_AGENT);
   }
@@ -370,8 +371,16 @@
     if (improved) bx = vx[0];
   }
   bool done = publish();
+  constexpr bool QUORUM = !RESUME && !STRICT;
+  [[maybe_unused]] unsigned quorum_flag = 0u;
+  auto park_on_quorum = [&]() __attribute__((always_inline)) {
+    if constexpr (QUORUM)
+      if (status < 0 && quorum_flag != 0u) status = kFitSuspended;
+  };
 
   while (!done) {
+    if constexpr (QUORUM)
+      if (a.quorum_words) quorum_flag = __hip_atomic_load(a.quorum_words + kEarlyFlag, __ATOMIC_RELAXED, __HIP_MEMORY_SCOPE_AGENT);
     {
       const double A = o_kind == 0 ? xr : (o_kind == 1 ? x_e : x_c);
       const double e0 = o_rank == 0 ? A : vx[0];
@@ -434,6 +443,7 @@
       insert_tail<4>(c, vx);
       status = ctl_begin(true, improved);
       if (improved) bx = vx[0];
+      park_on_quorum();
       ctl_write(status);
       xr = t[dim];
       x_e = t[4 + dim];
@@ -447,6 +457,7 @@
         if (a.skipped && gl == 0 && rest > 0) atomicAdd(a.skipped, 2ull * (unsigned long long)rest);
       }
       status = ctl_begin(true, improved);
+      park_on_quorum();
       ctl_write(status);
       par ^= 1;
     } else {
@@ -462,6 +473,7 @@
       sort5(c, vx);
       status = ctl_begin(true, improved);
       if (improved) bx = vx[0];
+      park_on_quorum();
       done = publish();
       continue;
     }
@@ -471,9 +483,46 @@
     }
   }
 
+  if constexpr (QUORUM) {
+    if (status == kFitSuspended) {
+      double* sp = a.state + (size_t)chain * kStateDoubles;
+      auto sd = [&](int i, double v) __attribute__((always_inline)) {
+        __hip_atomic_store(sp + i, v, __ATOMIC_RELAXED, __HIP_MEMORY_SCOPE_AGENT);
+      };
+      if (gl < 4) {
+#pragma unroll
+        for (int k = 0; k < 5; ++k) sd(kStateSimplex + 4 * k + gl, vx[k]);
+        sd(kStateBest + gl, bx);
+        a.best[(size_t)chain * 4 + gl] = __builtin_nan("");
+      }
+      if (gl == 0) {
+#pragma unroll
+        for (int k = 0; k < 5; ++k) sd(kStateCosts + k, c[k]);
+        sd(kStateBestCost, best_cost);
+        sd(kStateIterEvals, __longlong_as_double((long long)(unsigned)iter | ((long long)evals << 32)));
+        sd(kStateHaveBest, __longlong_as_double(have_best ? 1ll : 0ll));
+        a.susp_list[atomicAdd(a.susp_count, 1)] = (int)chain;
+        FitInfoDev fo;
+        fo.best_cost = best_cost;
+        fo.iters = iter;
+        fo.evals = evals;
+        fo.status = kFitSuspended;
+        fo.lanes = a.tree;
+        a.info[chain] = fo;
+      }
+      return;
+    }
+  }
   const double b0 = dpp_mov<kDppQuadBcast0>(bx), b1 = dpp_mov<kDppQuadBcast1>(bx);
   if (gl < 4) a.best[(size_t)chain * 4 + gl] = bx;
   if (gl == 0) {
+    if constexpr (QUORUM) {
+      if (a.quorum_words) {
+        unsigned* q = a.quorum_words;
+        if (atomicAdd(q + kEarlyCount, 1u) + 1u >= (unsigned)a.quorum)
+          __hip_atomic_store(q + kEarlyFlag, 1u, __ATOMIC_RELAXED, __HIP_MEMORY_SCOPE_AGENT);
+      }
+    }
 #ifdef ABN_DIAG_RESUME_COUNT
     if constexpr (RESUME) atomicAdd(a.slice_status + kSliceFinished, 0x10000u);
 #else
diff --git a/alphabeta_rs_amd/csrc/abn_route.hpp b/alphabeta_rs_amd/csrc/abn_route.hpp
--- a/alphabeta_rs_amd/csrc/abn_route.hpp
+++ b/alphabeta_rs_amd/csrc/abn_route.hpp
@@ -259,4 +259,25 @@
   return r;
 }
 
-}
+struct EarlyRoute {
+  bool eligible;
+  int quorum;
+};
+inline EarlyRoute route_early_bootstraps(const PedigreeRoute& p, int n_windows, int n_starts, int n_boot, int cus,
+                                         int window_groups, bool two_pass, bool parking) {
+  EarlyRoute e{false, 0};
+  if (n_windows != 1 || n_starts < 5 || n_boot <= 0 || p.strict || window_groups > 1) return e;
+  const PhaseRoute pa = route_phase(p, 0, n_starts, cus, 0, true, two_pass);
+  if (!pa.spec || n_starts > (pick_rmax(p.n, kWave) <= 2 ? 4LL : 3LL) * cus) return e;
+  const PhaseRoute pb = route_phase(p, 1, n_boot, cus, 1, true, two_pass);
+  LaunchOffer offer;
+  offer.queue = true;
+  offer.parking = parking;
+  const LaunchRoute lb = route_launch(p, pb, n_boot, cus, offer);
+  if (lb.status != ABN_OK || lb.kind != ABN_KERNEL_PERSISTENT) return e;
+  e.eligible = true;
+  e.quorum = n_starts - std::max(1, n_starts / 5);
+  return e;
+}
+
+}
diff --git a/include/abneutral.h b/include/abneutral.h
--- a/include/abneutral.h
+++ b/include/abneutral.h
@@ -196,6 +196,8 @@
 int abn_plan_run_phase(abn_plan* plan, int32_t phase );
 int abn_plan_sync(abn_plan* plan);
 int abn_plan_tail_handed(abn_plan* plan, int64_t* out2);
+int abn_plan_set_early_bootstraps(abn_plan* plan, int32_t mode);
+int abn_plan_early_bootstraps(abn_plan* plan, int32_t* out4);
 int abn_plan_kernel_ms(abn_plan* plan, double* ms3);
 int abn_plan_raw_device_ptr(abn_plan* plan, void** dev_ptr);
 int abn_plan_bind_raw(abn_plan* plan, void* dev_ptr);
```
